# qope/SIPP

Hardware: AMD Instinct MI355X
Metric: SIPP proof-gen wall-clock + pairings-aggregated/sec, n=128 (the 3 STARK sub-proofs, hardened G1/G2 AIRs; outer plonky2 proof not included) (higher is better)
Workload: dtype u64; 1 GPU; n=128 SIPP instance per GPU: G1ExpStark 127 IO (N=2^16, W+P+Q=1176), G2ExpStark 127 IO (N=2^16, 2314), Fq12ExpStark 14 IO (N=2^13, 7970); IO records on host -> 3 flat proofs on host, the 3 sub-proofs on 3 concurrent HIP streams; parallelism=1 independent SIPP instance(s), one per GPU, no collective

## Files before the change

__graft_entry__.py:

```python
import os
import sys

ROOT = os.path.dirname(os.path.abspath(__file__))
if ROOT not in sys.path:
    sys.path.insert(0, ROOT)


def build():
    from sipp_amd import build as b
    so = b.build()
    assert os.path.exists(so), so
    from tests import _oracle
    _oracle.build()
    import sipp_amd
    sipp_amd.lib()
    import subprocess
    subprocess.check_call(["make", "-C", os.path.join(ROOT, "tests", "host"), "-s"])
    subprocess.check_call(["make", "-C", os.path.join(ROOT, "tests", "probe"), "-s"])


def smoke():
    import numpy as np
    import torch
    assert torch.cuda.is_available(), "smoke() needs a GPU"
    import sipp_amd
    from tests import _oracle

    ios = np.load(os.path.join(ROOT, "tests", "golden", "sipp_n4_ios.npz"))["g1"]
    ctx = sipp_amd.Ctx(device=0, workspace_bytes=4 << 30)
    proof = ctx.prove(0, ios)
    ctx.close()
    ref = _oracle.stark_prove(0, ios)
    assert len(proof) == len(ref) and (proof == ref).all(), "GPU proof differs from the CPU oracle's"
    assert sipp_amd.stark_verify(proof) == 0, "the library's own verifier (sipp_stark_verify) rejects the GPU proof"
    assert _oracle.stark_verify(proof) == 0, "oracle verifier rejects the GPU proof"
    print("smoke ok: G1ExpStark proof (%d words) identical to the oracle's, accepted by the library's verifier and the oracle's" % len(proof))


if __name__ == "__main__":
    build()
    if len(sys.argv) > 1 and sys.argv[1] == "smoke":
        smoke()
```

include/sipp_hip.h:

```cpp
#ifndef SIPP_HIP_H
#define SIPP_HIP_H

#include <stddef.h>
#include <stdint.h>

#ifdef __cplusplus
extern "C" {
#endif

typedef struct sipp_ctx sipp_ctx;

typedef enum {
    SIPP_OK = 0,
    SIPP_E_BADARG = -1,
    SIPP_E_HIP = -2,
    SIPP_E_NOMEM = -3,
    SIPP_E_BUFSZ = -4,
    SIPP_E_SUBGROUP = -5,
    SIPP_E_QUOTIENT = -6,
    SIPP_E_UNSUPPORTED = -7,
    SIPP_E_WITNESS = -8,
    SIPP_E_VERIFY = -9
} sipp_status;

typedef struct {
    uint32_t rate_bits;
    uint32_t cap_height;
    uint32_t pow_bits;
    uint32_t arity_bits;
    uint32_t final_poly_bits;
    uint32_t num_queries;
    uint32_t num_challenges;
    uint32_t pow_rule;
    uint32_t fs_rule;
    uint32_t lookup_rule;
} sipp_stark_config;
#define SIPP_POW_DUPLEX 0
#define SIPP_POW_HASH 1
#define SIPP_FS_STATEMENT 0
#define SIPP_FS_UPSTREAM 1
#define SIPP_LOOKUP_INDEPENDENT 0
#define SIPP_LOOKUP_SHARED 1

void sipp_default_config(sipp_stark_config *cfg);

typedef enum { SIPP_G1_EXP = 0, SIPP_G2_EXP = 1, SIPP_FQ12_EXP = 2,
               SIPP_MAP_G2 = 3 ,
               SIPP_G1_EXP_HARDENED = 4, SIPP_G2_EXP_HARDENED = 5,
               SIPP_PAIRING = 6  } sipp_kind;

#define SIPP_G1_IO_WORDS 56
#define SIPP_G2_IO_WORDS 104
#define SIPP_FQ12_IO_WORDS 296
#define SIPP_MAP_G2_IO_WORDS 48
#define SIPP_PAIRING_IO_WORDS 144

int sipp_ctx_create(sipp_ctx **out, int device, const sipp_stark_config *cfg, size_t workspace_bytes);
#define SIPP_ABI_VERSION 3u
uint32_t sipp_abi_version(void);
int sipp_ctx_create_checked(sipp_ctx **out, int device, const sipp_stark_config *cfg, size_t cfg_size, uint32_t abi_version,
                            size_t workspace_bytes);
#define SIPP_ROUTE_OPENINGS_UNGROUPED 1u
#define SIPP_ROUTE_LDE_COLUMN_WIDE 2u
#define SIPP_ROUTE_WITNESS_NO_GRAPH 4u
int sipp_ctx_set_kernel_routes(sipp_ctx *ctx, uint32_t routes);
void sipp_ctx_destroy(sipp_ctx *ctx);
int sipp_ctx_set_stream_priority(sipp_ctx *ctx, int level);
int sipp_ctx_set_hardened(sipp_ctx *ctx, int on);
const char *sipp_last_error(const sipp_ctx *ctx);
int sipp_sync(sipp_ctx *ctx);
void *sipp_stream(sipp_ctx *ctx);

int sipp_g1_exp_prove(sipp_ctx *ctx, const uint32_t *ios, size_t num_io, uint64_t *proof_out, size_t proof_cap,
                      size_t *proof_len);
int sipp_g2_exp_prove(sipp_ctx *ctx, const uint32_t *ios, size_t num_io, uint64_t *proof_out, size_t proof_cap,
                      size_t *proof_len);
int sipp_fq12_exp_prove(sipp_ctx *ctx, const uint32_t *ios, size_t num_io, uint64_t *proof_out, size_t proof_cap,
                        size_t *proof_len);
int sipp_prove(sipp_ctx *ctx, int kind, const uint32_t *ios, size_t num_io, uint64_t *proof_out, size_t proof_cap,
               size_t *proof_len);
int sipp_prove_async(sipp_ctx *ctx, int kind, const uint32_t *ios, size_t num_io, uint64_t *proof_out,
                     size_t proof_cap);
int sipp_wait(sipp_ctx *ctx, size_t *proof_len);
int sipp_instance_prove(sipp_ctx *const ctxs[3], const uint32_t *const ios[3], const size_t num_io[3],
                        uint64_t *const proof_out[3], const size_t proof_cap[3], size_t proof_len[3]);
int sipp_instances_prove(sipp_ctx *const *ctxs, size_t in_flight, size_t count, const uint32_t *const *ios,
                         const size_t *num_io, uint64_t *const *proof_out, const size_t *proof_cap, size_t *proof_len,
                         int *status);
int sipp_io_shard(size_t num_io, uint32_t world, uint32_t rank, size_t *first, size_t *count);
int sipp_exp_outputs(sipp_ctx *ctx, int kind, uint32_t *ios, size_t num_io);
size_t sipp_proof_size(const sipp_ctx *ctx, int kind, size_t num_io);
size_t sipp_workspace_bytes(int kind, size_t num_io);
size_t sipp_workspace_bytes_cfg(int kind, size_t num_io, const sipp_stark_config *cfg);
int sipp_device_memory(int device, size_t *free_bytes, size_t *total_bytes);
int sipp_stark_shape(const sipp_ctx *ctx, int kind, size_t num_io, uint32_t *log_rows, uint32_t *main_cols,
                     uint32_t *perm_cols, uint32_t *quotient_cols);

int sipp_map_to_g2_prove(sipp_ctx *ctx, const uint32_t *ios, size_t num_io, uint64_t *proof_out, size_t proof_cap,
                         size_t *proof_len);
int sipp_pairing_prove(sipp_ctx *ctx, const uint32_t *ios, size_t num_io, uint64_t *proof_out, size_t proof_cap,
                       size_t *proof_len);
int sipp_stark_verify(const uint64_t *proof, size_t len, const sipp_stark_config *cfg, int *reason);

int sipp_map_to_g2(sipp_ctx *ctx, const uint32_t *msgs, size_t n, uint32_t *map_ios, uint32_t *g2_ios, uint32_t *cleared);

int sipp_inner_product(sipp_ctx *ctx, const uint32_t *g1, const uint32_t *g2, size_t n, uint32_t *out);
int sipp_inner_products(sipp_ctx *ctx, const uint32_t *g1, const uint32_t *g2, size_t n, size_t count, uint32_t *out);

size_t sipp_native_proof_words(size_t n);
int sipp_prove_native(sipp_ctx *ctx, const uint32_t *A, const uint32_t *B, size_t n, uint32_t *proof);
int sipp_verify_native(sipp_ctx *ctx, const uint32_t *A, const uint32_t *B, size_t n, const uint32_t *proof,
                       uint32_t *statement, uint32_t *g1_ios, uint32_t *g2_ios, uint32_t *fq12_ios, int *accepted);

#define SIPP_SALT_SIZE 4
#define SIPP_FRI_MAX_ROUNDS 32
typedef struct {
    uint32_t rate_bits, cap_height, pow_bits, num_queries, pow_rule;
    uint32_t hiding;
    uint32_t n_rounds;
    uint32_t arity_bits[SIPP_FRI_MAX_ROUNDS];
} sipp_fri_params;
void sipp_fri_const_arity(sipp_fri_params *p, uint32_t arity_bits, uint32_t final_poly_bits, uint32_t degree_bits);
typedef struct {
    const uint64_t *d_coeffs;
    const uint64_t *d_lde;
    const uint64_t *d_tree;
    uint32_t n_polys, n_salt;
} sipp_oracle;
int sipp_commit_batch_ex(sipp_ctx *ctx, const uint64_t *d_in, int from_coeffs, uint64_t *d_coeffs, uint64_t *d_lde,
                         uint64_t *d_tree, size_t ncols, uint32_t log_n, uint32_t rate_bits, uint32_t cap_height,
                         const uint64_t *d_salt, uint32_t n_salt, uint64_t *cap_out);
typedef struct { uint32_t oracle, col_begin, col_end; } sipp_poly_range;
typedef struct {
    uint64_t point[2];
    uint32_t n_ranges;
    const sipp_poly_range *ranges;
} sipp_fri_batch;
typedef struct {
    uint64_t state[12];
    uint64_t in_buf[8];
    uint64_t n_in;
    uint64_t out_buf[8];
    uint64_t n_out;
} sipp_challenger;
size_t sipp_fri_proof_size(const sipp_oracle *oracles, size_t n_oracles, const sipp_fri_batch *batches, size_t n_batches,
                           uint32_t log_n, const sipp_fri_params *p);
int sipp_fri_prove_openings(sipp_ctx *ctx, const sipp_oracle *oracles, size_t n_oracles, const sipp_fri_batch *batches,
// ... 125 lines not shown
```

sipp_amd/csrc/api.hip:

```cpp
#include <algorithm>
#include <string>

#include "ctx.hpp"
#include "host_poseidon.hpp"

int sipp_poseidon_init_constants(sipp_ctx* ctx);

extern "C" {

void sipp_default_config(sipp_stark_config* cfg) {
    if (!cfg) return;
    cfg->rate_bits = 1;
    cfg->cap_height = 4;
    cfg->pow_bits = 16;
    cfg->arity_bits = 4;
    cfg->final_poly_bits = 5;
    cfg->num_queries = 84;
    cfg->num_challenges = 2;
    cfg->pow_rule = SIPP_POW_DUPLEX;
    cfg->fs_rule = SIPP_FS_STATEMENT;
    cfg->lookup_rule = SIPP_LOOKUP_INDEPENDENT;
}

static hipError_t create_ctx_stream(int device, int level, hipStream_t* out) {
    int lo = 0, hi = 0;
    (void)hipDeviceGetStreamPriorityRange(&lo, &hi);
    static const int dedicated = [] { const char* e = getenv("SIPP_DEDICATED_QUEUES"); return e ? atoi(e) : 1; }();
    if (level <= 0 && dedicated) {
        hipDeviceProp_t prop;
        if (hipGetDeviceProperties(&prop, device) == hipSuccess && prop.multiProcessorCount > 0 && prop.multiProcessorCount <= 1024) {
            uint32_t mask[32];
            const uint32_t words = ((uint32_t)prop.multiProcessorCount + 31) / 32;
            for (uint32_t i = 0; i < words; i++) {
                const uint32_t left = (uint32_t)prop.multiProcessorCount - 32 * i;
                mask[i] = left >= 32 ? 0xffffffffu : (1u << left) - 1;
            }
            if (hipExtStreamCreateWithCUMask(out, words, mask) == hipSuccess) return hipSuccess;
            (void)hipGetLastError();
        }
    }
    return hipStreamCreateWithPriority(out, hipStreamNonBlocking, level > 0 ? hi : level < 0 ? lo : 0);
}

int sipp_ctx_create(sipp_ctx** out, int device, const sipp_stark_config* cfg, size_t workspace_bytes) {
    if (!out) return SIPP_E_BADARG;
    *out = nullptr;
    int ndev = 0;
    if (hipGetDeviceCount(&ndev) != hipSuccess || ndev <= 0 || device < 0 || device >= ndev) return SIPP_E_HIP;
    sipp_ctx* ctx = new sipp_ctx();
    ctx->device = device;
    if (cfg)
        ctx->cfg = *cfg;
    else
        sipp_default_config(&ctx->cfg);
    if (ctx->cfg.rate_bits < 1 || ctx->cfg.rate_bits > 3 || ctx->cfg.num_challenges != 2 || ctx->cfg.arity_bits < 1 ||
        ctx->cfg.arity_bits > 4 || ctx->cfg.cap_height > 8 || ctx->cfg.pow_bits > 32 || ctx->cfg.pow_rule > SIPP_POW_HASH ||
        ctx->cfg.fs_rule > SIPP_FS_UPSTREAM || ctx->cfg.lookup_rule > SIPP_LOOKUP_SHARED || ctx->cfg.num_queries == 0 || ctx->cfg.num_queries > 1024 || ctx->cfg.final_poly_bits > 12) {
        delete ctx;
        return SIPP_E_UNSUPPORTED;
    }
    auto bail = [&](int rc) {
        hipError_t last = hipGetLastError();
        fprintf(stderr, "sipp_ctx_create(device %d, workspace %zu bytes) failed with status %d (last HIP error: %s)\n", device,
                workspace_bytes, rc, hipGetErrorString(last));
        sipp_ctx_destroy(ctx);
        return rc;
    };
    if (hipSetDevice(device) != hipSuccess) return bail(SIPP_E_HIP);
    if (create_ctx_stream(device, 0, &ctx->stream) != hipSuccess) return bail(SIPP_E_HIP);
    if (workspace_bytes == 0) workspace_bytes = (size_t)24 << 30;
    ctx->arena_size = workspace_bytes;
    if (hipMalloc((void**)&ctx->arena, workspace_bytes) != hipSuccess) return bail(SIPP_E_NOMEM);
    if (hipEventCreate(&ctx->t0) != hipSuccess || hipEventCreate(&ctx->t1) != hipSuccess) return bail(SIPP_E_HIP);
    ctx->h_pinned_words = (size_t)1 << 23;
    if (hipHostMalloc((void**)&ctx->h_pinned, ctx->h_pinned_words * 8) != hipSuccess) return bail(SIPP_E_NOMEM);
    int rc = sipp_poseidon_init_constants(ctx);
    if (rc != SIPP_OK) return bail(rc);
    *out = ctx;
    return SIPP_OK;
}

void sipp_ctx_destroy(sipp_ctx* ctx) {
    if (!ctx) return;
    if (ctx->async.started) {
        {
            std::unique_lock<std::mutex> lk(ctx->async.mu);
            ctx->async.cv.wait(lk, [&] { return !ctx->async.has_job || ctx->async.done; });
            ctx->async.quit = true;
        }
        ctx->async.cv.notify_all();
        ctx->async.th.join();
    }
    (void)hipSetDevice(ctx->device);
    if (ctx->stream) (void)hipStreamSynchronize(ctx->stream);
    sipp_witness_graph_release(ctx);
    for (auto& kv : ctx->tables) (void)hipFree(kv.second);
    for (auto e : ctx->ev_pool) (void)hipEventDestroy(e);
    if (ctx->t0) (void)hipEventDestroy(ctx->t0);
    if (ctx->t1) (void)hipEventDestroy(ctx->t1);
    if (ctx->h_pinned) (void)hipHostFree(ctx->h_pinned);
    if (ctx->arena) (void)hipFree(ctx->arena);
    if (ctx->aux_stream) (void)hipStreamDestroy(ctx->aux_stream);
    if (ctx->aux2_stream) (void)hipStreamDestroy(ctx->aux2_stream);
    if (ctx->stream) (void)hipStreamDestroy(ctx->stream);
    delete ctx;
}

uint32_t sipp_abi_version(void) { return SIPP_ABI_VERSION; }

int sipp_ctx_create_checked(sipp_ctx** out, int device, const sipp_stark_config* cfg, size_t cfg_size, uint32_t abi_version,
                            size_t workspace_bytes) {
    if (out) *out = nullptr;
    if (abi_version != SIPP_ABI_VERSION || (cfg && cfg_size != sizeof(sipp_stark_config))) return SIPP_E_BADARG;
    return sipp_ctx_create(out, device, cfg, workspace_bytes);
}

int sipp_ctx_set_kernel_routes(sipp_ctx* ctx, uint32_t routes) {
    if (!ctx || (routes & ~(uint32_t)(SIPP_ROUTE_OPENINGS_UNGROUPED | SIPP_ROUTE_LDE_COLUMN_WIDE | SIPP_ROUTE_WITNESS_NO_GRAPH))) return SIPP_E_BADARG;
    std::unique_lock<std::mutex> lk(ctx->async.mu);
    if (ctx->async.has_job) {
        lk.unlock();
        return sipp_fail(ctx, SIPP_E_BADARG, "set_kernel_routes: a proof is in flight on this ctx");
    }
    ctx->kernel_routes = routes;
    return SIPP_OK;
}

int sipp_ctx_set_hardened(sipp_ctx* ctx, int on) {
    if (!ctx) return SIPP_E_BADARG;
    std::unique_lock<std::mutex> lk(ctx->async.mu);
    if (ctx->async.has_job) {
        lk.unlock();
        return sipp_fail(ctx, SIPP_E_BADARG, "set_hardened: a proof is in flight on this ctx");
    }
    ctx->hardened = on != 0;
    return SIPP_OK;
}

int sipp_ctx_set_stream_priority(sipp_ctx* ctx, int level) {
    if (!ctx) return SIPP_E_BADARG;
    {
        std::unique_lock<std::mutex> lk(ctx->async.mu);
        if (ctx->async.has_job) {
            lk.unlock();
            return sipp_fail(ctx, SIPP_E_BADARG, "set_stream_priority: a proof is in flight on this ctx");
        }
    }
    SIPP_CHECK_HIP(ctx, hipSetDevice(ctx->device));
    hipStream_t ns = nullptr;
    if (create_ctx_stream(ctx->device, level, &ns) != hipSuccess) return sipp_fail(ctx, SIPP_E_HIP, "set_stream_priority: no stream");
    if (ctx->stream) {
        (void)hipStreamSynchronize(ctx->stream);
        if (ctx->prof) {
            (void)sipp_profile_enable(ctx, 0);
            ctx->prof = true;
        }
        (void)hipStreamDestroy(ctx->stream);
    }
    ctx->stream = ns;
    return SIPP_OK;
}

const char* sipp_last_error(const sipp_ctx* ctx) { return ctx ? ctx->err : "null ctx"; }

int sipp_sync(sipp_ctx* ctx) {
    if (!ctx) return SIPP_E_BADARG;
    SIPP_CHECK_HIP(ctx, hipSetDevice(ctx->device));
    SIPP_CHECK_HIP(ctx, hipStreamSynchronize(ctx->stream));
    return SIPP_OK;
}

void* sipp_stream(sipp_ctx* ctx) { return ctx ? (void*)ctx->stream : nullptr; }

static void prof_drain(sipp_ctx* ctx) {
    if (ctx->pending.empty()) return;
    (void)hipSetDevice(ctx->device);
    (void)hipStreamSynchronize(ctx->stream);
    for (auto& p : ctx->pending) {
        float ms = 0.f;
        if (hipEventElapsedTime(&ms, ctx->ev_pool[std::get<1>(p)], ctx->ev_pool[std::get<2>(p)]) == hipSuccess) {
            auto& e = ctx->prof_acc[std::get<0>(p)];
            e.calls++;
            e.ms += ms;
        }
    }
    ctx->pending.clear();
    ctx->ev_used = 0;
}

int sipp_profile_enable(sipp_ctx* ctx, int enable) {
    if (!ctx) return SIPP_E_BADARG;
    if (!enable) prof_drain(ctx);
    ctx->prof = enable != 0;
    return SIPP_OK;
}

int sipp_profile_reset(sipp_ctx* ctx) {
    if (!ctx) return SIPP_E_BADARG;
    prof_drain(ctx);
    ctx->prof_acc.clear();
    return SIPP_OK;
// ... 157 lines not shown
```

sipp_amd/csrc/ctx.hpp:

```cpp
#pragma once
#include <stdlib.h>
#include <hip/hip_runtime.h>
#include <stdint.h>
#include <stdio.h>
#include <string.h>

#include <condition_variable>
#include <map>
#include <mutex>
#include <string>
#include <thread>
#include <tuple>
#include <vector>

#include "../../include/sipp_hip.h"
#include "gl.hpp"

struct sipp_gate {
    std::mutex mu;
    std::condition_variable cv;
    bool open = false;
    void release() {
        {
            std::lock_guard<std::mutex> lk(mu);
            open = true;
        }
        cv.notify_all();
    }
    void wait() {
        std::unique_lock<std::mutex> lk(mu);
        cv.wait(lk, [&] { return open; });
    }
};

struct sipp_prof_entry {
    int calls = 0;
    double ms = 0.0;
};

struct sipp_ctx {
    int device = 0;
    hipStream_t stream = nullptr;
    sipp_stark_config cfg{};
    char err[512] = {0};

    char* arena = nullptr;
    size_t arena_size = 0;
    size_t arena_off = 0;
    size_t arena_peak = 0;

    std::map<std::tuple<int, uint64_t, uint64_t>, uint64_t*> tables;

    bool prof = false;
    std::vector<hipEvent_t> ev_pool;
    size_t ev_used = 0;
    std::vector<std::tuple<std::string, size_t, size_t>> pending;
    std::map<std::string, sipp_prof_entry> prof_acc;
    hipEvent_t t0 = nullptr, t1 = nullptr;

    uint64_t* h_pinned = nullptr;
    size_t h_pinned_words = 0;

    sipp_gate* gate_wait = nullptr;
    sipp_gate* gate_release = nullptr;

    hipStream_t aux_stream = nullptr;
    hipStream_t aux2_stream = nullptr;
    struct Fold {
        bool active = false;
        size_t mark = 0;
        uint32_t* d_ios[2] = {nullptr, nullptr};
        void* rows[2] = {nullptr, nullptr};
        int* d_err = nullptr;
        uint32_t num_io[2] = {0, 0};
        size_t n_in[2] = {0, 0};
    } fold;

    bool outputs_only = false;
    bool hardened = false;
    uint32_t kernel_routes = 0;
    struct WitnessGraph {
        hipGraph_t graph = nullptr;
        hipGraphExec_t exec = nullptr;
        std::vector<uint64_t> key;
    } wgraph;

    struct Async {
        std::thread th;
        std::mutex mu;
        std::condition_variable cv;
        bool started = false, has_job = false, done = false, quit = false;
        int kind = 0;
        const uint32_t* ios = nullptr;
        size_t num_io = 0, cap = 0, len = 0;
        uint64_t* out = nullptr;
        int rc = 0;
    } async;
};

#define SIPP_CHECK_HIP(ctx, expr)                                                                   \
    do {                                                                                            \
        hipError_t e__ = (expr);                                                                    \
        if (e__ != hipSuccess) {                                                                    \
            snprintf((ctx)->err, sizeof((ctx)->err), "%s:%d: %s -> %s", __FILE__, __LINE__, #expr,  \
                     hipGetErrorString(e__));                                                       \
            return SIPP_E_HIP;                                                                      \
        }                                                                                           \
    } while (0)

#define SIPP_TRY(expr)              \
    do {                            \
        int rc__ = (expr);          \
        if (rc__ != SIPP_OK) return rc__; \
    } while (0)

static inline int sipp_fail(sipp_ctx* ctx, int code, const char* msg) {
    if (ctx) snprintf(ctx->err, sizeof(ctx->err), "%s", msg);
    return code;
}

struct ArenaMark {
    size_t off;
};
static inline ArenaMark arena_mark(sipp_ctx* ctx) { return ArenaMark{ctx->arena_off}; }
static inline void arena_release(sipp_ctx* ctx, ArenaMark m) { ctx->arena_off = m.off; }
static inline void* arena_alloc(sipp_ctx* ctx, size_t bytes) {
    size_t off = (ctx->arena_off + 255) & ~(size_t)255;
    if (off + bytes > ctx->arena_size) {
        snprintf(ctx->err, sizeof(ctx->err), "workspace arena exhausted: need %zu more bytes (size %zu, used %zu)",
                 bytes, ctx->arena_size, off);
        return nullptr;
    }
    ctx->arena_off = off + bytes;
    if (ctx->arena_off > ctx->arena_peak) ctx->arena_peak = ctx->arena_off;
    return ctx->arena + off;
}
struct ArenaScope {
    sipp_ctx* ctx;
    ArenaMark mark;
    explicit ArenaScope(sipp_ctx* c) : ctx(c), mark(arena_mark(c)) {}
    ~ArenaScope() { arena_release(ctx, mark); }
    ArenaScope(const ArenaScope&) = delete;
    ArenaScope& operator=(const ArenaScope&) = delete;
};
// ... 86 lines not shown
```

sipp_amd/csrc/fri.hip:

```cpp
#include <algorithm>

#include "prover.hpp"

static size_t tree_words(uint32_t log_leaves) { return ((size_t)8 << log_leaves); }

static int read_cap(sipp_ctx* ctx, const uint64_t* d_tree, uint32_t log_leaves, uint32_t cap_height, uint64_t* cap_host) {
    const uint32_t ch = std::min(cap_height, log_leaves);
    uint64_t off = 0;
    for (uint32_t l = 0; l < log_leaves - ch; l++) off += (uint64_t)1 << (log_leaves - l);
    SIPP_CHECK_HIP(ctx, hipMemcpyAsync(cap_host, d_tree + 4 * off, ((size_t)4 << ch) * 8, hipMemcpyDeviceToHost, ctx->stream));
    SIPP_CHECK_HIP(ctx, hipStreamSynchronize(ctx->stream));
    return SIPP_OK;
}

size_t sipp_fri_core_words(const FriParamsDev& p, uint32_t log_n, const uint32_t* leaf_words, int n_oracles) {
    const uint32_t log_m = log_n + p.rate_bits;
    const size_t cap = (size_t)4 << p.cap_height;
    uint32_t sum = 0;
    for (uint32_t ab : p.arity_bits) sum += ab;
    size_t w = p.arity_bits.size() * cap + 2 * ((size_t)1 << (log_n - sum)) + 1;
    size_t per_q = 0;
    for (int o = 0; o < n_oracles; o++) per_q += leaf_words[o] + (size_t)(log_m - p.cap_height) * 4;
    uint32_t lt = log_m;
    for (uint32_t ab : p.arity_bits) {
        lt -= ab;
        per_q += ((size_t)2 << ab) + (size_t)(lt > p.cap_height ? lt - p.cap_height : 0) * 4;
    }
    return w + p.num_queries * per_q;
}

int sipp_fri_prove_core(sipp_ctx* ctx, const FriOracleDev* ors, int n_oracles, uint32_t log_n, const FriParamsDev& p,
                        uint64_t* d_final, host::Challenger& ch, uint64_t* pf, size_t& pos, size_t cap_total, size_t* final_len,
                        const std::function<void(const char*)>& tick) {
    const uint32_t log_m = log_n + p.rate_bits, R = (uint32_t)p.arity_bits.size(), nq = p.num_queries;
    const size_t n = (size_t)1 << log_n, m = (size_t)1 << log_m;
    const size_t cap_words = (size_t)4 << p.cap_height;
    if (p.cap_height > 8 || n_oracles < 1 || n_oracles > 8) return sipp_fail(ctx, SIPP_E_UNSUPPORTED, "fri: unsupported shape");
    auto push = [&](const uint64_t* v, size_t cnt) -> int {
        if (pos + cnt > cap_total) return SIPP_E_BUFSZ;
        memcpy(pf + pos, v, cnt * 8);
        pos += cnt;
        return SIPP_OK;
    };
    uint64_t cap_host[4 << 8];
    std::vector<uint64_t*> r_vals(R), r_tree(R);
    std::vector<uint32_t> r_loglen(R);
    uint64_t* cur = d_final;
    size_t len_c = n;
    uint32_t log_len = log_m;
    uint64_t shift = gl::GEN;
    for (uint32_t r = 0; r < R; r++) {
        const uint32_t ab = p.arity_bits[r];
        const size_t len = (size_t)1 << log_len;
        if (log_len < ab + 0u || (len_c >> ab) == 0) return sipp_fail(ctx, SIPP_E_BADARG, "fri: reduction arities exceed the degree");
        r_loglen[r] = log_len;
        r_vals[r] = arena_alloc_t<uint64_t>(ctx, 2 * len);
        r_tree[r] = arena_alloc_t<uint64_t>(ctx, tree_words(log_len - ab));
        uint64_t* nxt = arena_alloc_t<uint64_t>(ctx, 2 * (len_c >> ab) + 2);
        if (!r_vals[r] || !r_tree[r] || !nxt) return SIPP_E_NOMEM;
        SIPP_TRY(sipp_ntt_dif(ctx, cur, len_c, log_len - p.rate_bits, r_vals[r], len, log_len, 2, false, NttDiag{shift, 0}));
        SIPP_TRY(sipp_k_fri_leaves(ctx, r_vals[r], len, ab, r_tree[r]));
        SIPP_TRY(sipp_k_merkle_levels(ctx, r_tree[r], log_len - ab, p.cap_height));
        SIPP_TRY(read_cap(ctx, r_tree[r], log_len - ab, p.cap_height, cap_host));
        const size_t cw = (size_t)4 << std::min(p.cap_height, log_len - ab);
        ch.observe_many(cap_host, cw);
        SIPP_TRY(push(cap_host, cw));
        const gl::E2 fb = ch.get_ext();
        SIPP_TRY(sipp_k_fri_fold(ctx, cur, len_c, ab, fb, nxt));
        cur = nxt;
        len_c >>= ab;
        log_len -= ab;
        shift = gl::pow(shift, (uint64_t)1 << ab);
    }
    (void)cap_words;
    if (final_len) *final_len = len_c;
    {
        std::vector<uint64_t> fpv(2 * len_c);
        SIPP_CHECK_HIP(ctx, hipMemcpyAsync(fpv.data(), cur, fpv.size() * 8, hipMemcpyDeviceToHost, ctx->stream));
        SIPP_CHECK_HIP(ctx, hipStreamSynchronize(ctx->stream));
        for (size_t i = 0; i < len_c; i++) {
            uint64_t e[2] = {fpv[i], fpv[len_c + i]};
            ch.observe_many(e, 2);
            SIPP_TRY(push(e, 2));
        }
    }
    if (tick) tick("fri commit phase");
    uint64_t pow_witness = 0;
    if (p.pow_rule == SIPP_POW_HASH) {
        uint64_t zero[12] = {0}, cur_h[4];
        for (int i = 0; i < 4; i++) cur_h[i] = ch.get();
        SIPP_TRY(sipp_k_pow_search(ctx, zero, cur_h, 4, 0, p.pow_bits, &pow_witness));
    } else {
        SIPP_TRY(sipp_k_pow_search(ctx, ch.state, ch.in_buf, ch.n_in, 7, p.pow_bits, &pow_witness));
        ch.observe(pow_witness);
        (void)ch.get();
    }
    SIPP_TRY(push(&pow_witness, 1));
    if (tick) tick("pow");
    std::vector<uint32_t> qidx(nq);
    for (uint32_t i = 0; i < nq; i++) qidx[i] = (uint32_t)(ch.get() % m);
    uint32_t* d_idx = arena_alloc_t<uint32_t>(ctx, nq);
    if (!d_idx) return SIPP_E_NOMEM;
    SIPP_CHECK_HIP(ctx, hipMemcpyAsync(d_idx, qidx.data(), nq * 4, hipMemcpyHostToDevice, ctx->stream));
    const uint32_t nsib0 = log_m - p.cap_height;
    size_t st_words = 0;
    std::vector<size_t> off_rows(n_oracles), off_sib(n_oracles), off_leaf(R), off_rsib(R);
    std::vector<uint32_t> rsib(R), rshift(R);
    for (int o = 0; o < n_oracles; o++) {
        off_rows[o] = st_words;
        st_words += (size_t)nq * ors[o].ncols;
        off_sib[o] = st_words;
        st_words += (size_t)nq * nsib0 * 4;
    }
    {
        uint32_t sh = 0;
        for (uint32_t r = 0; r < R; r++) {
            const uint32_t ab = p.arity_bits[r];
            sh += ab;
            rshift[r] = sh;
            const uint32_t lt = log_m - sh;
            rsib[r] = lt > p.cap_height ? lt - p.cap_height : 0;
            off_leaf[r] = st_words;
            st_words += (size_t)nq * ((size_t)2 << ab);
            off_rsib[r] = st_words;
            st_words += (size_t)nq * rsib[r] * 4;
        }
    }
    if (st_words > ctx->h_pinned_words) return sipp_fail(ctx, SIPP_E_NOMEM, "query staging exceeds the pinned buffer");
    uint64_t* d_st = arena_alloc_t<uint64_t>(ctx, st_words);
    if (!d_st) return SIPP_E_NOMEM;
    std::vector<QueryGatherTask> tasks;
    {
        for (int o = 0; o < n_oracles; o++) {
            tasks.push_back(QueryGatherTask{ors[o].lde, d_st + off_rows[o], (uint64_t)ors[o].stride, 0, ors[o].ncols, 0, 0});
            if (nsib0) tasks.push_back(QueryGatherTask{ors[o].tree, d_st + off_sib[o], 0, 1, log_m, nsib0, 0});
        }
        for (uint32_t r = 0; r < R; r++) {
            const uint32_t ab = p.arity_bits[r];
            tasks.push_back(QueryGatherTask{r_vals[r], d_st + off_leaf[r], (uint64_t)1 << r_loglen[r], 2, rshift[r], ab, 0});
            if (rsib[r]) tasks.push_back(QueryGatherTask{r_tree[r], d_st + off_rsib[r], 0, 1, r_loglen[r] - ab, rsib[r], rshift[r]});
        }
        QueryGatherTask* d_tasks = arena_alloc_t<QueryGatherTask>(ctx, tasks.size());
        if (!d_tasks) return SIPP_E_NOMEM;
        SIPP_CHECK_HIP(ctx, hipMemcpyAsync(d_tasks, tasks.data(), tasks.size() * sizeof(QueryGatherTask), hipMemcpyHostToDevice, ctx->stream));
        SIPP_TRY(sipp_k_gather_tasks(ctx, d_tasks, (uint32_t)tasks.size(), d_idx, nq));
    }
    uint64_t* hst = ctx->h_pinned;
    SIPP_CHECK_HIP(ctx, hipMemcpyAsync(hst, d_st, st_words * 8, hipMemcpyDeviceToHost, ctx->stream));
    SIPP_CHECK_HIP(ctx, hipStreamSynchronize(ctx->stream));
    for (uint32_t qi = 0; qi < nq; qi++) {
        for (int o = 0; o < n_oracles; o++) {
            SIPP_TRY(push(hst + off_rows[o] + (size_t)qi * ors[o].ncols, (size_t)ors[o].ncols));
            SIPP_TRY(push(hst + off_sib[o] + (size_t)qi * nsib0 * 4, (size_t)nsib0 * 4));
        }
        for (uint32_t r = 0; r < R; r++) {
            const size_t lw = (size_t)2 << p.arity_bits[r];
            SIPP_TRY(push(hst + off_leaf[r] + (size_t)qi * lw, lw));
            SIPP_TRY(push(hst + off_rsib[r] + (size_t)qi * rsib[r] * 4, (size_t)rsib[r] * 4));
        }
    }
    return SIPP_OK;
}


#define SIPP_FRI_MAGIC 0x5349505046524931ULL

static size_t batch_len(const sipp_fri_batch& b) {
    size_t k = 0;
    for (uint32_t r = 0; r < b.n_ranges; r++) k += b.ranges[r].col_end - b.ranges[r].col_begin;
    return k;
}

static int check_params(sipp_ctx* ctx, const sipp_fri_params* p, uint32_t log_n) {
    if (!p || p->rate_bits < 1 || p->rate_bits > 3 || p->cap_height > 8 || p->pow_bits > 32 || p->pow_rule > SIPP_POW_HASH ||
        p->num_queries == 0 || p->num_queries > 1024 || p->n_rounds > SIPP_FRI_MAX_ROUNDS)
        return sipp_fail(ctx, SIPP_E_UNSUPPORTED, "fri: parameters out of the supported range");
    uint32_t sum = 0;
    for (uint32_t r = 0; r < p->n_rounds; r++) {
        if (p->arity_bits[r] < 1 || p->arity_bits[r] > 4) return sipp_fail(ctx, SIPP_E_UNSUPPORTED, "fri: arity must be 2, 4, 8 or 16");
        sum += p->arity_bits[r];
        if (log_n + p->rate_bits < sum + p->cap_height)
            return sipp_fail(ctx, SIPP_E_BADARG, "fri: reduction arities leave a layer smaller than its cap");
        if (log_n + p->rate_bits - sum + p->arity_bits[r] < 4)
            return sipp_fail(ctx, SIPP_E_UNSUPPORTED, "fri: a committed layer of fewer than 16 values is not supported");
    }
    if (sum > log_n) return sipp_fail(ctx, SIPP_E_BADARG, "fri: the reduction arities exceed the degree bits");
    if (log_n < 10 || log_n > 24) return sipp_fail(ctx, SIPP_E_UNSUPPORTED, "fri: degree bits outside the supported range [10, 24]");
    return SIPP_OK;
}

extern "C" {

void sipp_fri_const_arity(sipp_fri_params* p, uint32_t arity_bits, uint32_t final_poly_bits, uint32_t degree_bits) {
    if (!p) return;
    p->n_rounds = 0;
    while (degree_bits > final_poly_bits && degree_bits + p->rate_bits - arity_bits >= p->cap_height && degree_bits >= arity_bits &&
           p->n_rounds < SIPP_FRI_MAX_ROUNDS) {
        p->arity_bits[p->n_rounds++] = arity_bits;
        degree_bits -= arity_bits;
    }
}

int sipp_commit_batch_ex(sipp_ctx* ctx, const uint64_t* d_in, int from_coeffs, uint64_t* d_coeffs, uint64_t* d_lde, uint64_t* d_tree,
                         size_t ncols, uint32_t log_n, uint32_t rate_bits, uint32_t cap_height, const uint64_t* d_salt,
                         uint32_t n_salt, uint64_t* cap_out) {
    if (!ctx || !d_in || !d_coeffs || !d_lde || !d_tree || !cap_out || ncols == 0) return SIPP_E_BADARG;
    if (rate_bits < 1 || rate_bits > 3 || cap_height > 8 || (n_salt != 0 && (n_salt != SIPP_SALT_SIZE || !d_salt)))
        return sipp_fail(ctx, SIPP_E_UNSUPPORTED, "commit_batch_ex: blowup 2 / 4 / 8, cap height <= 8, salt 0 or 4 columns");
    SIPP_CHECK_HIP(ctx, hipSetDevice(ctx->device));
    const uint32_t log_m = log_n + rate_bits;
    const size_t n = (size_t)1 << log_n, m = (size_t)1 << log_m;
    ArenaScope scope(ctx);
    int rc;
    if (from_coeffs) {
        if (d_in != d_coeffs) SIPP_CHECK_HIP(ctx, hipMemcpyAsync(d_coeffs, d_in, ncols * n * 8, hipMemcpyDeviceToDevice, ctx->stream));
        rc = sipp_lde_from_coeffs(ctx, d_coeffs, d_lde, ncols, log_n, rate_bits);
        if (rc == SIPP_E_UNSUPPORTED) rc = sipp_ntt_dif(ctx, d_coeffs, n, log_n, d_lde, m, log_m, ncols, false, NttDiag{gl::GEN, 0});
    } else {
        rc = d_in != d_coeffs ? sipp_lde_from_values(ctx, d_in, d_coeffs, d_lde, ncols, log_n, rate_bits) : SIPP_E_UNSUPPORTED;
        if (rc == SIPP_E_UNSUPPORTED) {
            const uint64_t* src = d_in;
            if (d_in == d_coeffs) {
                uint64_t* tmp = arena_alloc_t<uint64_t>(ctx, n * ncols);
                if (!tmp) return SIPP_E_NOMEM;
                SIPP_CHECK_HIP(ctx, hipMemcpyAsync(tmp, d_in, n * ncols * 8, hipMemcpyDeviceToDevice, ctx->stream));
                src = tmp;
            }
// ... 14 lines not shown
                           uint32_t log_n, const sipp_fri_params* p) {
    if (!oracles || !batches || !p || n_oracles == 0 || n_oracles > 8 || n_batches == 0) return 0;
    FriParamsDev fp;
    fp.rate_bits = p->rate_bits; fp.cap_height = p->cap_height; fp.pow_bits = p->pow_bits; fp.num_queries = p->num_queries;
    fp.pow_rule = p->pow_rule;
    uint32_t sum = 0;
    for (uint32_t r = 0; r < p->n_rounds && r < SIPP_FRI_MAX_ROUNDS; r++) {
        fp.arity_bits.push_back(p->arity_bits[r]);
        sum += p->arity_bits[r];
    }
    if (sum > log_n) return 0;
    uint32_t lw[8];
    for (size_t o = 0; o < n_oracles; o++) lw[o] = oracles[o].n_polys + oracles[o].n_salt;
    size_t w = 8 + sipp_fri_core_words(fp, log_n, lw, (int)n_oracles);
    for (size_t b = 0; b < n_batches; b++) w += 2 * batch_len(batches[b]);
    return w;
}

int sipp_fri_prove_openings(sipp_ctx* ctx, const sipp_oracle* oracles, size_t n_oracles, const sipp_fri_batch* batches,
                            size_t n_batches, uint32_t log_n, const sipp_fri_params* p, sipp_challenger* chs, uint64_t* proof_out,
                            size_t proof_cap, size_t* proof_len) {
    if (!ctx || !oracles || !batches || !p || !chs || !proof_out || !proof_len || n_oracles == 0 || n_oracles > 8 || n_batches == 0)
        return SIPP_E_BADARG;
    SIPP_CHECK_HIP(ctx, hipSetDevice(ctx->device));
    SIPP_TRY(check_params(ctx, p, log_n));
    if (chs->n_in > 7 || chs->n_out > 8) return sipp_fail(ctx, SIPP_E_BADARG, "fri: malformed challenger state");
    const size_t total = sipp_fri_proof_size(oracles, n_oracles, batches, n_batches, log_n, p);
    if (total == 0) return SIPP_E_BADARG;
    if (proof_cap < total) return sipp_fail(ctx, SIPP_E_BUFSZ, "fri: proof buffer too small (see sipp_fri_proof_size)");
    for (size_t b = 0; b < n_batches; b++)
        for (uint32_t r = 0; r < batches[b].n_ranges; r++) {
            const sipp_poly_range& rg = batches[b].ranges[r];
            if (rg.oracle >= n_oracles || rg.col_begin > rg.col_end || rg.col_end > oracles[rg.oracle].n_polys)
                return sipp_fail(ctx, SIPP_E_BADARG, "fri: polynomial range outside its oracle");
        }
    const size_t n = (size_t)1 << log_n, m = n << p->rate_bits;
    FriParamsDev fp;
    fp.rate_bits = p->rate_bits; fp.cap_height = p->cap_height; fp.pow_bits = p->pow_bits; fp.num_queries = p->num_queries;
    fp.pow_rule = p->pow_rule;
    for (uint32_t r = 0; r < p->n_rounds; r++) fp.arity_bits.push_back(p->arity_bits[r]);
    host::Challenger ch;
    memcpy(ch.state, chs->state, sizeof ch.state);
    memcpy(ch.in_buf, chs->in_buf, sizeof ch.in_buf);
    memcpy(ch.out_buf, chs->out_buf, sizeof ch.out_buf);
    ch.n_in = (uint32_t)chs->n_in;
    ch.n_out = (uint32_t)chs->n_out;
    struct Release {
        sipp_ctx* c;
        ArenaMark mk;
        ~Release() {
            (void)hipStreamSynchronize(c->stream);
            arena_release(c, mk);
        }
    } release{ctx, arena_mark(ctx)};
    size_t pos = 0;
    uint64_t* pf = proof_out;
    {
        uint64_t hdr[8] = {SIPP_FRI_MAGIC, p->n_rounds, 0, p->num_queries, (uint64_t)n_oracles, (uint64_t)n_batches, total, log_n};
        memcpy(pf, hdr, sizeof hdr);
        pos = 8;
    }
    std::vector<uint64_t*> d_zp(n_batches), d_zip(n_batches);
    std::vector<gl::E2> points(n_batches);
    for (size_t b = 0; b < n_batches; b++) {
        points[b] = gl::E2{batches[b].point[0], batches[b].point[1]};
        if (gl::eq(gl::pow(points[b], (uint64_t)n), gl::e2(1))) return sipp_fail(ctx, SIPP_E_SUBGROUP, "fri: opening point in the subgroup");
        d_zp[b] = arena_alloc_t<uint64_t>(ctx, 2 * n);
        d_zip[b] = arena_alloc_t<uint64_t>(ctx, 2 * n);
        if (!d_zp[b] || !d_zip[b]) return SIPP_E_NOMEM;
        SIPP_TRY(sipp_k_pow_table(ctx, points[b], n, d_zp[b]));
        SIPP_TRY(sipp_k_pow_table(ctx, gl::inv(points[b]), n, d_zip[b]));
    }
    for (size_t b = 0; b < n_batches; b++) {
        const size_t k = batch_len(batches[b]);
        uint64_t* d_open = arena_alloc_t<uint64_t>(ctx, 4 * k + 4);
        if (!d_open) return SIPP_E_NOMEM;
        size_t at = 0;
        for (uint32_t r = 0; r < batches[b].n_ranges; r++) {
            const sipp_poly_range& rg = batches[b].ranges[r];
            const size_t cnt = rg.col_end - rg.col_begin;
            SIPP_TRY(sipp_k_openings(ctx, oracles[rg.oracle].d_coeffs + (size_t)rg.col_begin * n, cnt, n, d_zp[b], nullptr, d_open + 4 * at));
            at += cnt;
        }
        std::vector<uint64_t> hop(4 * k + 4);
        SIPP_CHECK_HIP(ctx, hipMemcpyAsync(hop.data(), d_open, (4 * k) * 8, hipMemcpyDeviceToHost, ctx->stream));
        SIPP_CHECK_HIP(ctx, hipStreamSynchronize(ctx->stream));
        for (size_t j = 0; j < k; j++) {
            memcpy(pf + pos, &hop[4 * j], 16);
            pos += 2;
            ch.observe_many(&hop[4 * j], 2);
        }
    }
    const gl::E2 alpha = ch.get_ext();
    uint64_t* d_acc = arena_alloc_t<uint64_t>(ctx, 2 * n);
    uint64_t* d_final = arena_alloc_t<uint64_t>(ctx, 2 * n);
    if (!d_acc || !d_final) return SIPP_E_NOMEM;
    for (size_t b = 0; b < n_batches; b++) {
        const size_t k = batch_len(batches[b]);
        std::vector<const uint64_t*> cols;
        cols.reserve(k);
        for (uint32_t r = 0; r < batches[b].n_ranges; r++) {
            const sipp_poly_range& rg = batches[b].ranges[r];
            for (uint32_t c = rg.col_begin; c < rg.col_end; c++) cols.push_back(oracles[rg.oracle].d_coeffs + (size_t)c * n);
        }
        std::vector<uint32_t> apow(6 * k + 6);
        gl::E2 ap = gl::e2(1);
        for (size_t c = 0; c < k; c++) {
            const uint64_t comp[2] = {ap.c0, ap.c1};
            for (int q = 0; q < 2; q++) {
                apow[6 * c + 3 * q] = (uint32_t)comp[q] & 0x3FFFFFu;
                apow[6 * c + 3 * q + 1] = (uint32_t)(comp[q] >> 22) & 0x3FFFFFu;
                apow[6 * c + 3 * q + 2] = (uint32_t)(comp[q] >> 44);
            }
            ap = gl::mul(ap, alpha);
        }
        const uint64_t** d_cols = reinterpret_cast<const uint64_t**>(arena_alloc(ctx, (k + 1) * sizeof(uint64_t*)));
        uint32_t* d_apow = arena_alloc_t<uint32_t>(ctx, apow.size());
        if (!d_cols || !d_apow) return SIPP_E_NOMEM;
        SIPP_CHECK_HIP(ctx, hipMemcpyAsync(d_cols, cols.data(), k * sizeof(uint64_t*), hipMemcpyHostToDevice, ctx->stream));
        SIPP_CHECK_HIP(ctx, hipMemcpyAsync(d_apow, apow.data(), apow.size() * 4, hipMemcpyHostToDevice, ctx->stream));
        SIPP_CHECK_HIP(ctx, hipStreamSynchronize(ctx->stream));
        SIPP_TRY(sipp_k_fri_batch_quotient(ctx, d_cols, (int)k, n, d_apow, d_zp[b], d_zip[b], ap, b == 0, d_acc));
    }
    SIPP_TRY(sipp_k_fri_mulx(ctx, d_acc, n, d_final));
    FriOracleDev ors[8];
    for (size_t o = 0; o < n_oracles; o++)
        ors[o] = FriOracleDev{oracles[o].d_lde, m, oracles[o].n_polys + oracles[o].n_salt, oracles[o].d_tree};
    size_t flen = 0;
    SIPP_TRY(sipp_fri_prove_core(ctx, ors, (int)n_oracles, log_n, fp, d_final, ch, pf, pos, total, &flen, nullptr));
    pf[2] = flen;
    if (pos != total) return sipp_fail(ctx, SIPP_E_BUFSZ, "internal: opening proof length mismatch");
    *proof_len = pos;
    memcpy(chs->state, ch.state, sizeof ch.state);
    memcpy(chs->in_buf, ch.in_buf, sizeof ch.in_buf);
    memcpy(chs->out_buf, ch.out_buf, sizeof ch.out_buf);
    chs->n_in = ch.n_in;
    chs->n_out = ch.n_out;
    return SIPP_OK;
}

}
```

sipp_amd/csrc/host_challenger.hpp:

```cpp
#pragma once
#include <stddef.h>
#include <stdint.h>

#include "gl.hpp"
#include "host_poseidon.hpp"

namespace host {


struct Challenger {
    uint64_t state[12] = {0};
    uint64_t in_buf[8];
    uint32_t n_in = 0;
    uint64_t out_buf[8];
    uint32_t n_out = 0;
    void duplex() {
        for (uint32_t i = 0; i < n_in; i++) state[i] = in_buf[i];
        n_in = 0;
        poseidon_permute(state);
        for (int i = 0; i < 8; i++) out_buf[i] = state[i];
        n_out = 8;
    }
    void observe(uint64_t e) {
        n_out = 0;
        in_buf[n_in++] = e;
        if (n_in == 8) duplex();
    }
    void observe_many(const uint64_t* e, size_t n) {
        for (size_t i = 0; i < n; i++) observe(e[i]);
    }
    uint64_t get() {
        if (n_in != 0 || n_out == 0) duplex();
        return out_buf[--n_out];
    }
    static void hash_no_pad(const uint64_t* in, size_t n, uint64_t out[4]) {
        uint64_t s[12] = {0};
        for (size_t i = 0; i < n; i += 8) {
            for (size_t k = 0; k < 8 && i + k < n; k++) s[k] = in[i + k];
            poseidon_permute(s);
        }
        for (int k = 0; k < 4; k++) out[k] = s[k];
    }
    static void two_to_one(const uint64_t l[4], const uint64_t r[4], uint64_t out[4]) {
        uint64_t s[12] = {l[0], l[1], l[2], l[3], r[0], r[1], r[2], r[3], 0, 0, 0, 0};
        poseidon_permute(s);
        for (int k = 0; k < 4; k++) out[k] = s[k];
    }
    gl::E2 get_ext() {
        gl::E2 r;
        r.c0 = get();
        r.c1 = get();
        return r;
    }
};

}
```

sipp_amd/csrc/poseidon.hip:

```cpp
#include <type_traits>
#include "ctx.hpp"
#ifndef GLL_T
#define GLL_T 140
#endif
#include "poseidon.hpp"
#include "poseidon_pair.hpp"
#include "prover.hpp"

namespace {

#ifndef SIPP_LEAVES_WPE
#define SIPP_LEAVES_WPE 3
#endif
__global__ void __launch_bounds__(256) __attribute__((amdgpu_waves_per_eu(SIPP_LEAVES_WPE, SIPP_LEAVES_WPE)))
poseidon_leaves_kernel(const uint64_t* __restrict__ lde, size_t col_stride,
                                                             uint32_t ncols, uint64_t n_leaves,
                                                             uint64_t* __restrict__ digests) {
    const uint64_t j0 = (uint64_t)blockIdx.x * blockDim.x + threadIdx.x;
    const uint64_t j = j0 < n_leaves ? j0 : n_leaves - 1;
    uint64_t s[12];
#pragma unroll
    for (int i = 0; i < 12; i++) s[i] = 0;
    const uint64_t* p = lde + j;
    __shared__ uint64_t stash[11 * 256];
// ... 140 lines not shown
#pragma unroll
    for (int i = 0; i < 12; i++) s[i] = 0;
    const uint64_t* c0 = vals + 16 * k;
    const uint64_t* c1 = vals + len + 16 * k;
#pragma unroll 1
    for (int chunk = 0; chunk < 4; chunk++) {
#pragma unroll
        for (int e = 0; e < 8; e++) s[e] = (e & 1) ? c1[4 * chunk + (e >> 1)] : c0[4 * chunk + (e >> 1)];
        poseidon::permute(s);
    }
    uint64_t* d = digests + 4 * k;
    d[0] = s[0]; d[1] = s[1]; d[2] = s[2]; d[3] = s[3];
}

__global__ void __launch_bounds__(256) fri_leaves_pair_kernel(const uint64_t* __restrict__ vals, uint64_t len,
                                                             uint64_t* __restrict__ digests) {
    __shared__ poseidon_pair::Tables T;
    poseidon_pair::load_tables(T);
    const uint32_t lane = threadIdx.x & 63, h = lane >> 5;
    const uint64_t wave = ((uint64_t)blockIdx.x * blockDim.x + threadIdx.x) >> 6;
    const uint64_t nl = len >> 4;
    if (wave * 32 >= nl) return;
    const uint64_t k = wave * 32 + (lane & 31);
    const bool live = k < nl;
    const uint64_t kk = live ? k : 0;
    const poseidon::mfma_v4i afrag = poseidon_pair::mds_fragment(lane);
    const uint64_t* c0 = vals + 16 * kk;
    const uint64_t* c1 = vals + len + 16 * kk;
    uint64_t s[6] = {0, 0, 0, 0, 0, 0};
#pragma unroll 1
    for (int chunk = 0; chunk < 4; chunk++) {
#pragma unroll
        for (int j = 0; j < 6; j++) {
            const uint32_t e = 6 * h + j;
            if (e < 8) s[j] = (e & 1) ? c1[4 * chunk + (e >> 1)] : c0[4 * chunk + (e >> 1)];
        }
        poseidon_pair::permute(s, lane, T, afrag);
    }
    if (!live || h) return;
    uint64_t* d = digests + 4 * k;
    d[0] = s[0];
    d[1] = s[1];
    d[2] = s[2];
    d[3] = s[3];
}

__global__ void __launch_bounds__(64) fri_leaves_any_kernel(const uint64_t* __restrict__ vals, uint64_t len, uint32_t ab,
                                                           uint64_t* __restrict__ digests) {
    const uint64_t k = (uint64_t)blockIdx.x * blockDim.x + threadIdx.x;
    if (k >= (len >> ab)) return;
    const uint32_t words = 2u << ab;
    const uint64_t* c0 = vals + (k << ab);
    const uint64_t* c1 = vals + len + (k << ab);
    uint64_t s[12];
#pragma unroll
    for (int i = 0; i < 12; i++) s[i] = 0;
    if (words <= 4) {
        s[0] = c0[0];
        s[1] = c1[0];
        if (words == 4) {
            s[2] = c0[1];
            s[3] = c1[1];
        }
    } else {
#pragma unroll 1
        for (uint32_t chunk = 0; chunk < words / 8; chunk++) {
#pragma unroll
            for (int e = 0; e < 8; e++) s[e] = (e & 1) ? c1[4 * chunk + (e >> 1)] : c0[4 * chunk + (e >> 1)];
            poseidon::permute(s);
        }
    }
    uint64_t* d = digests + 4 * k;
    d[0] = s[0]; d[1] = s[1]; d[2] = s[2]; d[3] = s[3];
}

struct PowArgs {
    uint64_t state[12];
    uint64_t in_buf[8];
    uint32_t n_in, pow_bits, resp_word;
    uint64_t base;
    unsigned long long* result;
};
__global__ void __launch_bounds__(256) pow_kernel(PowArgs a) {
    const uint64_t w = a.base + (uint64_t)blockIdx.x * blockDim.x + threadIdx.x;
    uint64_t s[12];
#pragma unroll
    for (int i = 0; i < 12; i++) s[i] = a.state[i];
#pragma unroll
    for (int i = 0; i < 8; i++) {
        if ((uint32_t)i < a.n_in) s[i] = a.in_buf[i];
        if ((uint32_t)i == a.n_in) s[i] = w;
    }
    poseidon::permute(s);
    const uint64_t resp = a.resp_word == 7 ? s[7] : s[0];
    if ((resp >> (64 - a.pow_bits)) == 0) atomicMin(a.result, (unsigned long long)w);
}

constexpr uint64_t thin_threshold() { return 65536; }

}

int sipp_k_fri_leaves(sipp_ctx* ctx, const uint64_t* d_vals, size_t len, uint32_t arity_bits, uint64_t* d_digests) {
    uint64_t nl = len >> arity_bits;
    ProfScope ps(ctx, "fri_leaves");
    if (arity_bits != 4) {
        if (arity_bits < 1 || arity_bits > 4) return sipp_fail(ctx, SIPP_E_UNSUPPORTED, "fri_leaves: arity must be 2, 4, 8 or 16");
        hipLaunchKernelGGL(fri_leaves_any_kernel, dim3((unsigned)((nl + 63) / 64)), dim3(64), 0, ctx->stream, d_vals, (uint64_t)len,
                           arity_bits, d_digests);
    } else if (nl <= thin_threshold())
        hipLaunchKernelGGL(fri_leaves_pair_kernel, dim3((unsigned)((2 * nl + 255) / 256)), dim3(256), 0, ctx->stream, d_vals,
                           (uint64_t)len, d_digests);
    else
        hipLaunchKernelGGL(fri_leaves_kernel, dim3((unsigned)((nl + 63) / 64)), dim3(64), 0, ctx->stream, d_vals, (uint64_t)len,
                           d_digests);
    SIPP_CHECK_HIP(ctx, hipGetLastError());
    return SIPP_OK;
}

int sipp_k_pow_search(sipp_ctx* ctx, const uint64_t state[12], const uint64_t* in_buf, uint32_t n_in, uint32_t resp_word,
                      uint32_t pow_bits, uint64_t* witness) {
    if (pow_bits == 0) { *witness = 0; return SIPP_OK; }
    if (pow_bits > 32 || n_in > 7 || (resp_word != 0 && resp_word != 7))
        return sipp_fail(ctx, SIPP_E_UNSUPPORTED, "pow_search: unsupported parameters");
    ArenaMark mk = arena_mark(ctx);
    unsigned long long* d_res = arena_alloc_t<unsigned long long>(ctx, 1);
    if (!d_res) return SIPP_E_NOMEM;
    PowArgs a;
    memcpy(a.state, state, sizeof a.state);
    memset(a.in_buf, 0, sizeof a.in_buf);
    memcpy(a.in_buf, in_buf, n_in * sizeof(uint64_t));
    a.n_in = n_in; a.pow_bits = pow_bits; a.resp_word = resp_word; a.result = d_res;
    const uint32_t log_batch = pow_bits + 1 < 12 ? 12 : pow_bits + 1 > 28 ? 28 : pow_bits + 1;
    const uint64_t batch = (uint64_t)1 << log_batch;
    unsigned long long h_res = ~0ull;
    SIPP_CHECK_HIP(ctx, hipMemsetAsync(d_res, 0xff, sizeof(unsigned long long), ctx->stream));
    for (uint64_t base = 0; base < ((uint64_t)1 << 44); base += batch) {
        a.base = base;
        {
            ProfScope ps(ctx, "pow_grind");
            hipLaunchKernelGGL(pow_kernel, dim3((unsigned)(batch / 256)), dim3(256), 0, ctx->stream, a);
        }
        SIPP_CHECK_HIP(ctx, hipGetLastError());
        SIPP_CHECK_HIP(ctx, hipMemcpyAsync(&h_res, d_res, sizeof h_res, hipMemcpyDeviceToHost, ctx->stream));
        SIPP_CHECK_HIP(ctx, hipStreamSynchronize(ctx->stream));
        if (h_res != ~0ull) break;
    }
    arena_release(ctx, mk);
    if (h_res == ~0ull) return sipp_fail(ctx, SIPP_E_UNSUPPORTED, "pow_search: no witness found");
    *witness = (uint64_t)h_res;
    return SIPP_OK;
}

int sipp_poseidon_init_constants(sipp_ctx* ctx) {
    SIPP_CHECK_HIP(ctx, hipMemcpyToSymbol(HIP_SYMBOL(poseidon::c_rc), SIPP_POSEIDON_RC, sizeof(SIPP_POSEIDON_RC)));
    SIPP_CHECK_HIP(ctx, hipMemcpyToSymbol(HIP_SYMBOL(poseidon::c_fast_first), SIPP_POSEIDON_FAST_FIRST,
                                          sizeof(SIPP_POSEIDON_FAST_FIRST)));
    SIPP_CHECK_HIP(ctx, hipMemcpyToSymbol(HIP_SYMBOL(poseidon::c_fast_scalar), SIPP_POSEIDON_FAST_SCALAR,
                                          sizeof(SIPP_POSEIDON_FAST_SCALAR)));
    SIPP_CHECK_HIP(ctx, hipMemcpyToSymbol(HIP_SYMBOL(poseidon::c_fast_mi), SIPP_POSEIDON_FAST_MI,
                                          sizeof(SIPP_POSEIDON_FAST_MI)));
    SIPP_CHECK_HIP(ctx, hipMemcpyToSymbol(HIP_SYMBOL(poseidon::c_fast_vs), SIPP_POSEIDON_FAST_VS,
                                          sizeof(SIPP_POSEIDON_FAST_VS)));
    SIPP_CHECK_HIP(ctx, hipMemcpyToSymbol(HIP_SYMBOL(poseidon::c_fast_what), SIPP_POSEIDON_FAST_WHAT,
                                          sizeof(SIPP_POSEIDON_FAST_WHAT)));
    SIPP_CHECK_HIP(ctx, hipMemcpyToSymbol(HIP_SYMBOL(poseidon::c_blk3), SIPP_POSEIDON_BLK3, sizeof(SIPP_POSEIDON_BLK3)));
    SIPP_CHECK_HIP(ctx, hipMemcpyToSymbol(HIP_SYMBOL(poseidon::c_comb3), SIPP_POSEIDON_COMB3, sizeof(SIPP_POSEIDON_COMB3)));
    SIPP_CHECK_HIP(ctx, hipMemcpyToSymbol(HIP_SYMBOL(poseidon::c_comb_c), SIPP_POSEIDON_COMB_C, sizeof(SIPP_POSEIDON_COMB_C)));
    SIPP_CHECK_HIP(ctx, hipMemcpyToSymbol(HIP_SYMBOL(poseidon::d_dense_a), SIPP_POSEIDON_DENSE_A, sizeof(SIPP_POSEIDON_DENSE_A)));
    SIPP_CHECK_HIP(ctx, hipMemcpyToSymbol(HIP_SYMBOL(poseidon::c_dense_start), SIPP_POSEIDON_DENSE_START, sizeof(SIPP_POSEIDON_DENSE_START)));
    SIPP_CHECK_HIP(ctx, hipMemcpyToSymbol(HIP_SYMBOL(poseidon_pair::d_pair_a), SIPP_POSEIDON_PAIR_A, sizeof(SIPP_POSEIDON_PAIR_A)));
    SIPP_CHECK_HIP(ctx, hipMemcpyToSymbol(HIP_SYMBOL(poseidon_pair::d_pair_mds_a), SIPP_POSEIDON_PAIR_MDS_A, sizeof(SIPP_POSEIDON_PAIR_MDS_A)));
    SIPP_CHECK_HIP(ctx, hipMemcpyToSymbol(HIP_SYMBOL(poseidon_pair::d_pair_cc), SIPP_POSEIDON_PAIR_CC3, sizeof(SIPP_POSEIDON_PAIR_CC3)));
    SIPP_CHECK_HIP(ctx, hipMemcpyToSymbol(HIP_SYMBOL(poseidon_pair::d_pair_start), SIPP_POSEIDON_PAIR_START, sizeof(SIPP_POSEIDON_PAIR_START)));
    return SIPP_OK;
}

int sipp_k_poseidon_leaves(sipp_ctx* ctx, const uint64_t* d_lde, size_t col_stride, size_t ncols, uint32_t log_leaves,
                           uint64_t* d_digests) {
    if (ncols == 0 || ncols > 0xffffffffull) return sipp_fail(ctx, SIPP_E_BADARG, "poseidon_leaves: bad ncols");
    uint64_t n = (uint64_t)1 << log_leaves;
    const bool thin = ncols > 4 && n <= thin_threshold() && n >= 32;
    ProfScope ps(ctx, ncols <= 4 ? "poseidon_leaves_noop" : thin ? "poseidon_leaves_pair" : "poseidon_leaves");
    if (ncols <= 4) {
        hipLaunchKernelGGL(poseidon_leaves_copy_kernel, dim3((unsigned)((n + 255) / 256)), dim3(256), 0, ctx->stream, d_lde, col_stride,
                           (uint32_t)ncols, n, d_digests);
    } else if (thin) {
        unsigned grid = (unsigned)((2 * n + 255) / 256);
        hipLaunchKernelGGL(poseidon_leaves_pair_kernel, dim3(grid), dim3(256), 0, ctx->stream, d_lde, col_stride,
                           (uint32_t)ncols, n, d_digests);
    } else {
        const unsigned bs = n <= 65536 ? 64 : 256;
        unsigned grid = (unsigned)((n + bs - 1) / bs);
        hipLaunchKernelGGL(poseidon_leaves_kernel, dim3(grid), dim3(bs), 0, ctx->stream, d_lde, col_stride,
                           (uint32_t)ncols, n, d_digests);
    }
    SIPP_CHECK_HIP(ctx, hipGetLastError());
    return SIPP_OK;
}

int sipp_k_merkle_levels(sipp_ctx* ctx, uint64_t* d_tree, uint32_t log_leaves, uint32_t cap_height) {
    if (cap_height > log_leaves) cap_height = log_leaves;
    {
        uint32_t level = 0;
        const uint32_t top = log_leaves - cap_height;
        while (level < top) {
            const uint32_t log_nodes = log_leaves - level;
            uint32_t lw = log_nodes <= 10 ? log_nodes : log_nodes >= 18 ? 10 : 8;
            uint32_t nlev = lw < top - level ? lw : top - level;
            const uint64_t widest_parents = (uint64_t)1 << (log_nodes - 1);
            if (widest_parents > thin_threshold()) {
                lw = 11;
                nlev = 3 < top - level ? 3 : top - level;
            }
            const unsigned blocks = 1u << (log_nodes - lw);
            ProfScope ps(ctx, "merkle_subtree");
            if (widest_parents <= thin_threshold())
                hipLaunchKernelGGL(merkle_subtree_kernel<true>, dim3(blocks), dim3(256), 0, ctx->stream, d_tree, log_leaves, level, lw, nlev);
            else
                hipLaunchKernelGGL(merkle_subtree_kernel<false>, dim3(blocks), dim3(256), 0, ctx->stream, d_tree, log_leaves, level, lw, nlev);
            SIPP_CHECK_HIP(ctx, hipGetLastError());
            level += nlev;
        }
        return SIPP_OK;
    }
}

int sipp_k_poseidon_permute(sipp_ctx* ctx, uint64_t* d_states, size_t n) {
    if (!n) return SIPP_OK;
    unsigned grid = (unsigned)((n + 255) / 256);
    ProfScope ps(ctx, "poseidon_permute");
    hipLaunchKernelGGL(poseidon_permute_kernel, dim3(grid), dim3(256), 0, ctx->stream, d_states, (uint64_t)n);
    SIPP_CHECK_HIP(ctx, hipGetLastError());
// ... 3 lines not shown
```

sipp_amd/csrc/prover.hip:

```cpp
#include <map>

#include "ctx.hpp"
#include "prover.hpp"

namespace {

using gl::E2;

template <bool REV>
__device__ __forceinline__ uint64_t block_scan_mul_256(uint64_t v, uint64_t* s) {
    const int t = REV ? 255 - (int)threadIdx.x : (int)threadIdx.x;
    s[t] = v;
    __syncthreads();
    for (int off = 1; off < 256; off <<= 1) {
        uint64_t o = t >= off ? s[t - off] : 1;
        __syncthreads();
        v = gl::mul(v, o);
        s[t] = v;
        __syncthreads();
    }
    return v;
}

__device__ __forceinline__ void block_scan4_mul_256(uint64_t (&v)[4], uint64_t (*s)[256]) {
    const int t = threadIdx.x;
#pragma unroll
    for (int q = 0; q < 4; q++) s[q][t] = v[q];
    __syncthreads();
    for (int off = 1; off < 256; off <<= 1) {
        uint64_t o[4];
        o[0] = t >= off ? s[0][t - off] : 1;
        o[1] = t >= off ? s[1][t - off] : 1;
        o[2] = t + off < 256 ? s[2][t + off] : 1;
        o[3] = t + off < 256 ? s[3][t + off] : 1;
        __syncthreads();
#pragma unroll
        for (int q = 0; q < 4; q++) {
            v[q] = gl::mul(v[q], o[q]);
            s[q][t] = v[q];
        }
        __syncthreads();
    }
}

template <int ZR>
__global__ void __launch_bounds__(256) z_phase_a(const uint64_t* __restrict__ trace, size_t n, int nm, int nc, int cbase,
                                                uint64_t gamma0, uint64_t gamma1, uint64_t beta0, uint64_t beta1,
                                                uint64_t* __restrict__ zv, uint64_t* __restrict__ totals) {
    __shared__ uint64_t s[4][256];
    const int j = blockIdx.y;
    const size_t r0 = (size_t)blockIdx.x * (256 * ZR) + (size_t)threadIdx.x * ZR;
    const ulonglong2* col = reinterpret_cast<const ulonglong2*>(trace + (size_t)(cbase + j) * n + r0);
    const ulonglong2* tab = reinterpret_cast<const ulonglong2*>(trace + r0);
    const ulonglong2* pin = reinterpret_cast<const ulonglong2*>(trace + (size_t)(nm + j) * n + r0);
    const ulonglong2* ptab = reinterpret_cast<const ulonglong2*>(trace + (size_t)(nm + nc + j) * n + r0);
    uint64_t num[2][ZR], den[2][ZR];
#pragma unroll
    for (int k = 0; k < ZR; k += 2) {
        const ulonglong2 c2 = col[k >> 1], t2 = tab[k >> 1], p2 = pin[k >> 1], q2 = ptab[k >> 1];
#pragma unroll
        for (int i = 0; i < 2; i++) {
            const uint64_t g = i ? gamma1 : gamma0, b = i ? beta1 : beta0;
            num[i][k] = gl::mul(gl::add(c2.x, g), gl::add(t2.x, b));
            den[i][k] = gl::mul(gl::add(p2.x, g), gl::add(q2.x, b));
            num[i][k + 1] = gl::mul(gl::add(c2.y, g), gl::add(t2.y, b));
            den[i][k + 1] = gl::mul(gl::add(p2.y, g), gl::add(q2.y, b));
        }
    }
    uint64_t v[4];
#pragma unroll
    for (int i = 0; i < 2; i++) {
        uint64_t ntot = 1;
#pragma unroll
        for (int k = 0; k < ZR; k++) {
            const uint64_t x = num[i][k];
            num[i][k] = ntot;
            ntot = gl::mul(ntot, x);
        }
#pragma unroll
        for (int k = ZR - 2; k >= 0; k--) den[i][k] = gl::mul(den[i][k], den[i][k + 1]);
        v[i] = ntot;
        v[2 + i] = den[i][0];
    }
    block_scan4_mul_256(v, s);
#pragma unroll
    for (int i = 0; i < 2; i++) {
// ... 237 lines not shown
            const uint64_t coef = gl::from_i64(*w++);
            uint64_t va[16], vb[16];
            w += qvec<16>(w, c, va);
            w += qvec<16>(w, c, vb);
#pragma unroll
            for (int ch = 0; ch < 2; ch++) {
                gl::Acc6 Ae, Ao, Be, Bo;
                Ae.zero(); Ao.zero(); Be.zero(); Bo.zero();
#pragma unroll
                for (int i = 0; i < 8; i++) {
                    const uint32_t* g3 = a.ginv3[ch][i];
                    Ae.mac((uint32_t)va[2 * i], (uint32_t)(va[2 * i] >> 32), g3);
                    Ao.mac((uint32_t)va[2 * i + 1], (uint32_t)(va[2 * i + 1] >> 32), g3);
                    Be.mac((uint32_t)vb[2 * i], (uint32_t)(vb[2 * i] >> 32), g3);
                    Bo.mac((uint32_t)vb[2 * i + 1], (uint32_t)(vb[2 * i + 1] >> 32), g3);
                }
                const uint64_t ae = Ae.reduce(), ao = Ao.reduce(), be = Be.reduce(), bo = Bo.reduce();
                const uint64_t cross = gl::add(gl::mul(ae, bo), gl::mul(ao, be));
                uint64_t t = gl::mad(gl::mul(ao, bo), a.gamma_inv[ch], gl::mul(ae, be));
                t = gl::mad(cross, 65536, t);
                psum[ch] = gl::mad(coef, t, psum[ch]);
            }
        }
        const int nl = slice == 0 ? (int)*w++ : 0;
        for (int p = 0; p < nl; p++) {
            const uint64_t coef = gl::from_i64(*w++);
            uint64_t va[16];
            w += qvec<16>(w, c, va);
#pragma unroll
            for (int ii = 0; ii < 16; ii++) e[ii] = gl::mad(coef, va[ii], e[ii]);
        }
        if (slice == 0) {
        uint64_t q[17];
        (void)qvec<17>(qdesc, c, q);
        const uint64_t s = c.local(sign_col);
        const uint64_t sgn = gl::sub(1, gl::add(s, s));
        uint64_t cprev = 0;
        const uint64_t coff = gl::from_i64(coffset);
        uint64_t d[32];
#pragma unroll
        for (int k = 0; k < 32; k++) {
            uint64_t al = 0, ah = 0;
#pragma unroll
            for (int ii = 0; ii < 17; ii++) {
                const int jj = k - ii;
                if (jj >= 0 && jj < 16) {
                    al += (uint64_t)(uint32_t)q[ii] * a.p_limbs[jj];
                    ah += (uint64_t)(uint32_t)(q[ii] >> 32) * a.p_limbs[jj];
                }
            }
            const uint64_t l = al + (ah << 32);
            const uint32_t h = (uint32_t)(ah >> 32) + (l < al ? 1u : 0u);
            const uint64_t qp = gl::reduce96(h, l);
            d[k] = gl::sub(e[k], gl::mul(sgn, qp));
        }
        const uint64_t wgt = (uint64_t)1 << (16 * grp);
#pragma unroll
        for (int mm = 0; mm < 32; mm++) {
            if (mm < 32 / grp) {
                uint64_t v;
                if (grp == 2) v = gl::mad(d[(2 * mm + 1) & 31], 65536, d[(2 * mm) & 31]);
                else v = d[mm];
                uint64_t ck = 0;
                if (mm < 32 / grp - 1) {
                    for (int l = 0; l < ncl; l++)
                        ck = gl::mad(c.local(cbase + mm * ncl + l), (uint64_t)1 << (lb * l), ck);
                    ck = gl::sub(ck, coff);
                }
                v = gl::sub(v, cprev);
                v = gl::mad(ck, wgt, v);
                c.emit(v);
                cprev = ck;
            }
        }
        c.emit(gl::mul(s, gl::sub(s, 1)));
        }
        c.acc0 = gl::mad(a.alpha16[0], psum[0], c.acc0);
        c.acc1 = gl::mad(a.alpha16[1], psum[1], c.acc1);
    }
    a.part[((size_t)g * 2 + 0) * m + j] = gl::mul(c.acc0, a.seg_pow[2 * g]);
    a.part[((size_t)g * 2 + 1) * m + j] = gl::mul(c.acc1, a.seg_pow[2 * g + 1]);
}

__global__ void alpha_pow3_kernel(uint64_t a0, uint64_t a1, int K, int nc, uint32_t* __restrict__ out) {
    const int t = blockIdx.x * blockDim.x + threadIdx.x;
    const int total = 2 * 3 + nc * 2 * 6;
    if (t >= total) return;
    int c, e;
    if (t < 6) {
        c = t / 3;
        e = K - 1 - t % 3;
    } else {
        const int k = (t - 6) / 12, r = (t - 6) % 12, slot = r % 6;
        c = r / 6;
        e = K - 1 - (3 + 2 * k) - (slot >> 1) * 2 * nc - (slot & 1);
    }
    uint32_t l[3];
    gl::limbs3(l, gl::pow(c ? a1 : a0, (uint64_t)e));
    for (int q = 0; q < 3; q++) out[3 * t + q] = l[q];
}

struct RestAcc {
    gl::Acc6 a[2];
    int terms;
    uint64_t folded[2];
    __device__ __forceinline__ void init() {
        a[0].zero();
        a[1].zero();
        terms = 0;
        folded[0] = folded[1] = 0;
    }
    __device__ __forceinline__ void mac(uint64_t v, const uint32_t* __restrict__ p0, const uint32_t* __restrict__ p1) {
        const uint32_t lo = (uint32_t)v, hi = (uint32_t)(v >> 32);
        a[0].mac(lo, hi, p0);
        a[1].mac(lo, hi, p1);
    }
    __device__ __forceinline__ void maybe_fold(int added) {
        terms += added;
        if (terms >= 960) {
            for (int c = 0; c < 2; c++) {
                folded[c] = gl::add(folded[c], gl::canon(a[c].reduce()));
                a[c].zero();
            }
            terms = 0;
        }
    }
    __device__ __forceinline__ uint64_t value(int c) const { return gl::add(folded[c], gl::canon(a[c].reduce())); }
};

struct RestPoint {
    uint64_t lf, zl, ll, zh_inv;
};
__device__ __forceinline__ RestPoint rest_point(const QuotArgs& a, uint32_t i) {
    const uint64_t x = gl::mul(gl::GEN, gl::pow(a.w_m, i));
    const uint64_t zh = a.zh[i & 1];
    RestPoint r;
    r.zl = gl::sub(x, a.g_inv);
    r.lf = gl::mul(gl::mul(zh, a.ninv), gl::inv(gl::sub(x, 1)));
    r.ll = gl::mul(gl::mul(gl::mul(zh, a.ninv), a.g_inv), gl::inv(r.zl));
    r.zh_inv = a.zh_inv[i & 1];
    return r;
}
__device__ __forceinline__ void rest_store(const QuotArgs& a, size_t m, size_t j, const RestPoint& pt, const uint64_t F[2], const uint64_t T[2],
                                           const uint64_t R[2]) {
    uint64_t acc[2] = {0, 0};
    for (int g = 0; g < a.n_seg; g++) {
        acc[0] = gl::add(acc[0], a.part[((size_t)g * 2 + 0) * m + j]);
        acc[1] = gl::add(acc[1], a.part[((size_t)g * 2 + 1) * m + j]);
    }
#pragma unroll
    for (int q = 0; q < 2; q++) {
        uint64_t v = gl::mul(acc[q], a.alphaK[q]);
        v = gl::add(v, R[q]);
        v = gl::mad(pt.lf, F[q], v);
        v = gl::mad(pt.zl, T[q], v);
        a.out[(size_t)q * m + j] = gl::mul(v, pt.zh_inv);
    }
}

template <bool SPLIT>
__global__ void __launch_bounds__(256) quotient_rest_kernel(QuotArgs a) {
    const size_t m = (size_t)1 << a.log_m;
    constexpr uint32_t RB = 3, RW = 256u >> RB;
    const uint32_t tid = threadIdx.x, run = tid / RW, blk = blockIdx.x, half = blk / (uint32_t)(m >> 9);
    const size_t j = (size_t)half * (m >> 1) + (size_t)run * (m >> (RB + 1)) + (size_t)(blk % (uint32_t)(m >> 9)) * RW + tid % RW;
    const uint32_t i = gl::bitrev((uint32_t)j, a.log_m);
// ... 104 lines not shown
    const int b = blockIdx.y;
    const E2 base = b == 0 ? a.base[0] : b == 1 ? a.base[1] : b == 2 ? a.base[2] : a.base[3];
    uint64_t* tab = b == 0 ? a.tab[0] : b == 1 ? a.tab[1] : b == 2 ? a.tab[2] : a.tab[3];
    const E2 r = gl::pow(base, (uint64_t)k);
    tab[k] = r.c0;
    tab[a.n + k] = r.c1;
}

__device__ __forceinline__ void openings_column(const uint64_t* __restrict__ col, size_t n, const uint64_t* __restrict__ t0,
                                                const uint64_t* __restrict__ t1, size_t tn, uint64_t* __restrict__ out4) {
    __shared__ uint64_t s[4][256];
    gl::Acc160 acc[4];
    constexpr int OB = 4;
    size_t k = threadIdx.x;
    for (; k + (OB - 1) * 256 < n; k += OB * 256) {
        uint64_t p0[OB], p1[OB], q0[OB], q1[OB], v[OB];
#pragma unroll
        for (int b = 0; b < OB; b++) {
            const size_t kb = k + (size_t)b * 256;
            p0[b] = t0[kb];
            p1[b] = t0[tn + kb];
            q0[b] = t1 ? t1[kb] : 0;
            q1[b] = t1 ? t1[tn + kb] : 0;
            v[b] = col[kb];
        }
#pragma unroll
        for (int b = 0; b < OB; b++) {
            acc[0].mac(v[b], p0[b]);
            acc[1].mac(v[b], p1[b]);
            if (t1) {
                acc[2].mac(v[b], q0[b]);
                acc[3].mac(v[b], q1[b]);
            }
        }
    }
    for (; k < n; k += 256) {
        const uint64_t v = col[k];
        acc[0].mac(v, t0[k]);
        acc[1].mac(v, t0[tn + k]);
        if (t1) {
            acc[2].mac(v, t1[k]);
            acc[3].mac(v, t1[tn + k]);
        }
    }
#pragma unroll
    for (int q = 0; q < 4; q++) s[q][threadIdx.x] = gl::canon(acc[q].reduce());
    __syncthreads();
    for (int off = 128; off > 0; off >>= 1) {
        if ((int)threadIdx.x < off)
            for (int q = 0; q < 4; q++) s[q][threadIdx.x] = gl::add(s[q][threadIdx.x], s[q][threadIdx.x + off]);
        __syncthreads();
    }
    if (threadIdx.x < 4) out4[threadIdx.x] = s[threadIdx.x][0];
}

__global__ void __launch_bounds__(256) openings_kernel(const uint64_t* __restrict__ coeffs, size_t n, uint32_t ncols,
                                                      const uint64_t* __restrict__ t0, const uint64_t* __restrict__ t1,
                                                      uint64_t* __restrict__ out) {
    openings_column(coeffs + (size_t)blockIdx.x * n, n, t0, t1, n, out + (size_t)blockIdx.x * 4);
}
__global__ void __launch_bounds__(256) openings_seg_kernel(const uint64_t* __restrict__ coeffs, size_t n, size_t seg_len,
                                                          const uint64_t* __restrict__ t0, const uint64_t* __restrict__ t1,
                                                          uint64_t* __restrict__ partial) {
    const size_t lo = (size_t)blockIdx.y * seg_len, len = min(seg_len, n - lo);
    openings_column(coeffs + (size_t)blockIdx.x * n + lo, len, t0 + lo, t1 ? t1 + lo : nullptr, n,
                    partial + ((size_t)blockIdx.x * gridDim.y + blockIdx.y) * 4);
}
__global__ void __launch_bounds__(256) openings_fold_kernel(const uint64_t* __restrict__ partial, uint32_t ncols, uint32_t segs,
                                                           uint64_t* __restrict__ out) {
    const uint32_t i = blockIdx.x * blockDim.x + threadIdx.x;
    if (i >= 4 * ncols) return;
    const uint64_t* p = partial + (size_t)(i >> 2) * segs * 4 + (i & 3);
    uint64_t acc = 0;
    for (uint32_t sg = 0; sg < segs; sg++) acc = gl::add(acc, p[4 * sg]);
    out[i] = acc;
}

struct Open3Args {
    const uint64_t* coeffs[3];
    uint32_t ncols[3];
    size_t n;
    const uint64_t *t0, *t1;
    uint64_t* out;
};
__global__ void __launch_bounds__(256) openings3_kernel(Open3Args a) {
    const uint32_t b = blockIdx.x;
    const uint64_t* col;
    const uint64_t* t1 = a.t1;
    if (b < a.ncols[0]) {
        col = a.coeffs[0] + (size_t)b * a.n;
    } else if (b < a.ncols[0] + a.ncols[1]) {
        col = a.coeffs[1] + (size_t)(b - a.ncols[0]) * a.n;
    } else {
        col = a.coeffs[2] + (size_t)(b - a.ncols[0] - a.ncols[1]) * a.n;
        t1 = nullptr;
    }
    openings_column(col, a.n, a.t0, t1, a.n, a.out + (size_t)b * 4);
}

constexpr int OG = 4;
struct OpenGArgs {
    const uint64_t* coeffs[3];
    uint32_t ncols[3];
    size_t n, seg_len;
    const uint64_t *t0, *t1;
    uint64_t* partial;
};
__global__ void __launch_bounds__(256) openings_group_kernel(OpenGArgs a) {
    __shared__ uint64_t s[4][256];
    uint32_t g = blockIdx.x, orc = 0, col_base = 0;
    while (orc < 2 && g >= (a.ncols[orc] + OG - 1) / OG) {
        g -= (a.ncols[orc] + OG - 1) / OG;
        col_base += a.ncols[orc];
        orc++;
    }
    const uint32_t c0 = g * OG, cnt = min((uint32_t)OG, a.ncols[orc] - c0);
    const bool two = orc < 2;
    const size_t n = a.n, lo = (size_t)blockIdx.y * a.seg_len, hi = min(n, lo + a.seg_len);
    const uint64_t* col = a.coeffs[orc] + (size_t)c0 * n;
    gl::Acc160 acc[OG][4];
    constexpr int OB = 2;
    size_t k = lo + threadIdx.x;
    for (; k + (OB - 1) * 256 < hi; k += OB * 256) {
        uint64_t p0[OB], p1[OB], q0[OB], q1[OB], v[OB][OG];
#pragma unroll
        for (int b = 0; b < OB; b++) {
            const size_t kb = k + (size_t)b * 256;
            p0[b] = a.t0[kb];
            p1[b] = a.t0[n + kb];
            q0[b] = two ? a.t1[kb] : 0;
            q1[b] = two ? a.t1[n + kb] : 0;
#pragma unroll
            for (int c = 0; c < OG; c++) v[b][c] = (uint32_t)c < cnt ? col[(size_t)c * n + kb] : 0;
        }
#pragma unroll
        for (int b = 0; b < OB; b++)
#pragma unroll
            for (int c = 0; c < OG; c++) {
                if ((uint32_t)c >= cnt) break;
                acc[c][0].mac(v[b][c], p0[b]);
                acc[c][1].mac(v[b][c], p1[b]);
                if (two) {
                    acc[c][2].mac(v[b][c], q0[b]);
                    acc[c][3].mac(v[b][c], q1[b]);
                }
            }
    }
    for (; k < hi; k += 256) {
        const uint64_t p0 = a.t0[k], p1 = a.t0[n + k], q0 = two ? a.t1[k] : 0, q1 = two ? a.t1[n + k] : 0;
#pragma unroll
        for (int c = 0; c < OG; c++) {
            if ((uint32_t)c >= cnt) break;
            const uint64_t v = col[(size_t)c * n + k];
            acc[c][0].mac(v, p0);
            acc[c][1].mac(v, p1);
            if (two) {
                acc[c][2].mac(v, q0);
                acc[c][3].mac(v, q1);
            }
        }
    }
#pragma unroll
    for (int c = 0; c < OG; c++) {
        if ((uint32_t)c >= cnt) break;
#pragma unroll
        for (int q = 0; q < 4; q++) s[q][threadIdx.x] = gl::canon(acc[c][q].reduce());
        __syncthreads();
        for (int off = 128; off > 0; off >>= 1) {
            if ((int)threadIdx.x < off)
                for (int q = 0; q < 4; q++) s[q][threadIdx.x] = gl::add(s[q][threadIdx.x], s[q][threadIdx.x + off]);
            __syncthreads();
        }
        if (threadIdx.x < 4) a.partial[((size_t)(col_base + c0 + c) * gridDim.y + blockIdx.y) * 4 + threadIdx.x] = s[threadIdx.x][0];
        __syncthreads();
    }
}

struct CombArgs {
    const uint64_t* src[3];
    int cnt[3];
    size_t n;
    const uint32_t* apow3;
    int n1;
    int slices;
    uint64_t* partial;
};
__global__ void __launch_bounds__(256) fri_combine_kernel(CombArgs a) {
    const size_t k = (size_t)blockIdx.x * 256 + threadIdx.x;
    const int total = a.cnt[0] + a.cnt[1] + a.cnt[2];
    const int per = (total + a.slices - 1) / a.slices;
    const int c_lo = blockIdx.y * per, c_hi = min(total, c_lo + per);
    gl::Acc6 G0, G1, H0, H1;
    G0.zero(); G1.zero(); H0.zero(); H1.zero();
    const uint64_t *src0 = a.src[0], *src1 = a.src[1], *src2 = a.src[2];
    const int cnt0 = a.cnt[0], cnt01 = a.cnt[0] + a.cnt[1], n1 = a.n1;
    const size_t nn = a.n;
    const uint32_t* __restrict__ apow3 = a.apow3;
    auto col_of = [=](int c) -> const uint64_t* {
        return c < cnt0 ? src0 + (size_t)c * nn : c < cnt01 ? src1 + (size_t)(c - cnt0) * nn : src2 + (size_t)(c - cnt01) * nn;
    };
#define SIPP_COMB_TERM(cc, vv)                                             \
    do {                                                                   \
        const uint64_t v_ = (vv);                                          \
        const uint32_t lo_ = (uint32_t)v_, hi_ = (uint32_t)(v_ >> 32);     \
        const uint32_t* __restrict__ w_ = apow3 + 6 * (cc);                \
        if ((cc) < n1) {                                 \
            G0.mac(lo_, hi_, w_);                                          \
            G1.mac(lo_, hi_, w_ + 3);                                      \
        } else {                                                           \
            H0.mac(lo_, hi_, w_);                                          \
            H1.mac(lo_, hi_, w_ + 3);                                      \
        }                                                                  \
    } while (0)
    constexpr int CB = 8;
    int c = c_lo;
    for (; c + CB <= c_hi; c += CB) {
        uint64_t v[CB];
#pragma unroll
        for (int b = 0; b < CB; b++) v[b] = col_of(c + b)[k];
#pragma unroll
        for (int b = 0; b < CB; b++) SIPP_COMB_TERM(c + b, v[b]);
    }
    for (; c < c_hi; c++) SIPP_COMB_TERM(c, col_of(c)[k]);
#undef SIPP_COMB_TERM
    const uint64_t g0 = gl::canon(G0.reduce()), g1 = gl::canon(G1.reduce());
    uint64_t* p = a.partial + (size_t)blockIdx.y * 4 * a.n;
    p[k] = gl::add(g0, gl::canon(H0.reduce()));
    p[a.n + k] = gl::add(g1, gl::canon(H1.reduce()));
    p[2 * a.n + k] = g0;
    p[3 * a.n + k] = g1;
}

struct GCombArgs {
    const uint64_t* const* cols;
    int total;
    size_t n;
    const uint32_t* apow3;
    int slices;
    uint64_t* partial;
};
__global__ void __launch_bounds__(256) fri_gcombine_kernel(GCombArgs a) {
    const size_t k = (size_t)blockIdx.x * 256 + threadIdx.x;
    const int per = (a.total + a.slices - 1) / a.slices;
    const int c_lo = blockIdx.y * per, c_hi = min(a.total, c_lo + per);
    gl::Acc6 G0, G1;
    G0.zero(); G1.zero();
    for (int c = c_lo; c < c_hi; c++) {
        const uint64_t v = a.cols[c][k];
        const uint32_t lo = (uint32_t)v, hi = (uint32_t)(v >> 32);
        const uint32_t* __restrict__ w = a.apow3 + 6 * c;
        G0.mac(lo, hi, w);
        G1.mac(lo, hi, w + 3);
    }
    uint64_t* p = a.partial + (size_t)blockIdx.y * 4 * a.n;
    p[k] = gl::canon(G0.reduce());
    p[a.n + k] = gl::canon(G1.reduce());
}

// ... 167 lines not shown
            const uint32_t l = e >> 2, w = e & 3;
            size_t off = 0;
            for (uint32_t k = 0; k < l; k++) off += (size_t)1 << (t.b - k);
            const size_t node = ((x >> t.d) >> l) ^ 1;
            t.out[((size_t)q * t.c + l) * 4 + w] = t.src[(off + node) * 4 + w];
        }
    } else {
        const size_t leaf = x >> t.b;
        for (uint32_t e = threadIdx.x; e < (2u << t.c); e += blockDim.x)
            t.out[((size_t)q << (t.c + 1)) + e] = t.src[(size_t)(e & 1) * t.a + (leaf << t.c) + (e >> 1)];
    }
}

}

int sipp_k_gather_tasks(sipp_ctx* ctx, const QueryGatherTask* d_tasks, uint32_t n_tasks, const uint32_t* d_idx, uint32_t nq) {
    if (!n_tasks || !nq) return SIPP_OK;
    ProfScope ps(ctx, "query_gather");
    hipLaunchKernelGGL(gather_tasks_kernel, dim3(nq, n_tasks), dim3(256), 0, ctx->stream, d_tasks, d_idx);
    SIPP_CHECK_HIP(ctx, hipGetLastError());
    return SIPP_OK;
}

int sipp_k_z_columns(sipp_ctx* ctx, const air_spec_t* a, const uint64_t* d_trace, uint32_t log_n, const uint64_t beta[2],
                     const uint64_t gamma[2], uint64_t* d_zv) {
    const size_t n = (size_t)1 << log_n;
    const int P = 2 * a->n_checked;
    const int zr = (n >= 16384) ? 8 : 4;
    const size_t zblock = (size_t)256 * zr;
    const unsigned nblk = (unsigned)(n / zblock);
    if (n % zblock) return sipp_fail(ctx, SIPP_E_BADARG, "z_columns: n must be a multiple of 1024");
    ArenaScope scope(ctx);
    uint64_t* totals = arena_alloc_t<uint64_t>(ctx, (size_t)2 * P * nblk);
    if (!totals) return SIPP_E_NOMEM;
    {
        ProfScope ps(ctx, "z_phase_a");
        if (zr == 8)
            hipLaunchKernelGGL(z_phase_a<8>, dim3(nblk, P / 2), dim3(256), 0, ctx->stream, d_trace, n, a->n_main, a->n_checked,
                               a->checked_base, gamma[0], gamma[1], beta[0], beta[1], d_zv, totals);
        else
            hipLaunchKernelGGL(z_phase_a<4>, dim3(nblk, P / 2), dim3(256), 0, ctx->stream, d_trace, n, a->n_main, a->n_checked,
                               a->checked_base, gamma[0], gamma[1], beta[0], beta[1], d_zv, totals);
    }
    {
        ProfScope ps(ctx, "z_phase_bc");
        hipLaunchKernelGGL(z_phase_b, dim3(P), dim3(256), 0, ctx->stream, totals, (int)nblk);
        if (zr == 8)
            hipLaunchKernelGGL(z_phase_c<8>, dim3(nblk, P), dim3(256), 0, ctx->stream, d_zv, n, totals);
        else
            hipLaunchKernelGGL(z_phase_c<4>, dim3(nblk, P), dim3(256), 0, ctx->stream, d_zv, n, totals);
    }
    SIPP_CHECK_HIP(ctx, hipGetLastError());
    return SIPP_OK;
}

static void host_ntt(uint64_t* a, uint32_t log_n, bool inverse) {
    const size_t n = (size_t)1 << log_n;
    for (size_t i = 0; i < n; i++) {
        const size_t j = gl::bitrev((uint32_t)i, log_n);
        if (i < j) std::swap(a[i], a[j]);
    }
    uint64_t root = gl::root_of_unity(log_n);
    if (inverse) root = gl::inv(root);
    for (uint32_t s = 1; s <= log_n; s++) {
        const size_t mlen = (size_t)1 << s, h = mlen >> 1;
        uint64_t wm = root;
        for (uint32_t k = s; k < log_n; k++) wm = gl::sqr(wm);
        for (size_t k = 0; k < n; k += mlen) {
            uint64_t w = 1;
            for (size_t j = 0; j < h; j++) {
                const uint64_t t = gl::mul(w, a[k + j + h]), u = a[k + j];
                a[k + j] = gl::add(u, t);
                a[k + j + h] = gl::sub(u, t);
                w = gl::mul(w, wm);
            }
        }
    }
    if (inverse) {
        const uint64_t ninv = gl::inv((uint64_t)n);
        for (size_t i = 0; i < n; i++) a[i] = gl::mul(a[i], ninv);
    }
}

int sipp_k_quotient(sipp_ctx* ctx, const air_spec_t* a, uint32_t log_n, const uint64_t* d_lde, const uint64_t* d_zlde,
                    size_t lde_stride, const uint64_t* d_aux, const uint64_t alpha[2], const uint64_t beta[2],
                    const uint64_t gamma[2], uint64_t* d_out) {
    const uint32_t log_m = log_n + 1;
    const size_t n = (size_t)1 << log_n, m = (size_t)1 << log_m;
    QuotArgs q{};
    q.lde = d_lde; q.zlde = d_zlde; q.aux = d_aux; q.lde_stride = lde_stride;
    q.prog = sipp_air_prog_device(ctx, a);
    if (!q.prog) return SIPP_E_HIP;
    q.prog_len = a->prog_len;
    q.W = a->n_main + 2 * a->n_checked; q.nm = a->n_main; q.nc = a->n_checked; q.cbase = a->checked_base;
    q.tbits = a->table_bits; q.log_n = log_n; q.log_m = log_m;
    q.alpha[0] = alpha[0]; q.alpha[1] = alpha[1]; q.gamma[0] = gamma[0]; q.gamma[1] = gamma[1];
    q.beta[0] = beta[0]; q.beta[1] = beta[1];
    const uint64_t g = gl::root_of_unity(log_n), wm = gl::root_of_unity(log_m);
    for (int k = 0; k < AIR_N_PERIODIC; k++) {
        const uint64_t mk = (uint64_t)AIR_PERIODIC[k][0], r0 = (uint64_t)AIR_PERIODIC[k][1];
        uint64_t* t = sipp_table_get(ctx, 200 + k, log_n, 0);
        if (!t) {
            const uint64_t K = n / mk;
            std::vector<uint64_t> v(2 * mk);
            const uint64_t gs = gl::inv(gl::pow(g, r0)), scale = gl::mul(K % gl::P, gl::inv(n % gl::P));
            for (uint64_t i = 0; i < 2 * mk; i++) {
                uint64_t x = gl::mul(gl::GEN, gl::pow(wm, i));
                uint64_t y = gl::mul(x, gs);
                uint64_t num = gl::sub(gl::pow(y, n), 1), den = gl::sub(gl::pow(y, K), 1);
                v[i] = gl::mul(gl::mul(num, gl::inv(den)), scale);
            }
            SIPP_TRY(sipp_table_put(ctx, 200 + k, log_n, 0, v, &t));
        }
        q.per_tab[k] = t;
        q.per_mask[k] = (uint32_t)(2 * mk - 1);
    }
    q.vper_tab = nullptr;
    q.vper_mask = 0;
    if (a->n_vflag + a->n_vconst > 0) {
        const uint32_t lr = (uint32_t)a->log_rows;
        const size_t R = (size_t)1 << lr, R2 = 2 * R;
        const int nv = a->n_vflag + a->n_vconst;
        uint64_t* t = sipp_table_get(ctx, 104, log_n, (uint64_t)a->kind);
        if (!t) {
            std::vector<uint64_t> tab((size_t)nv * R2), col(R2);
            const uint64_t shift = gl::pow(gl::GEN, (uint64_t)1 << (log_n - lr));
            std::map<std::vector<int64_t>, int> seen;
            std::vector<int64_t> vals(R);
            for (int k = 0; k < nv; k++) {
                for (size_t r = 0; r < R; r++) vals[r] = air_vper_value(a, k, (int)r);
                auto it = seen.find(vals);
                if (it != seen.end()) {
                    memcpy(&tab[(size_t)k * R2], &tab[(size_t)it->second * R2], R2 * 8);
                    continue;
                }
                seen.emplace(vals, k);
                for (size_t r = 0; r < R; r++) col[r] = gl::from_i64(vals[r]);
                host_ntt(col.data(), lr, true);
                uint64_t f = 1;
                for (size_t j = 0; j < R; j++) {
                    col[j] = gl::mul(col[j], f);
                    f = gl::mul(f, shift);
                }
                for (size_t j = R; j < R2; j++) col[j] = 0;
                host_ntt(col.data(), lr + 1, false);
                memcpy(&tab[(size_t)k * R2], col.data(), R2 * 8);
            }
            SIPP_TRY(sipp_table_put(ctx, 104, log_n, (uint64_t)a->kind, tab, &t));
        }
        q.vper_tab = t;
        q.vper_mask = (uint32_t)(R2 - 1);
    }
    const uint64_t sN = gl::pow(gl::GEN, n);
    q.zh[0] = gl::sub(sN, 1);
    q.zh[1] = gl::sub(gl::neg(sN), 1);
    q.zh_inv[0] = gl::inv(q.zh[0]);
    q.zh_inv[1] = gl::inv(q.zh[1]);
    q.ninv = gl::inv(n % gl::P);
    q.g_inv = gl::inv(g);
    q.w_m = wm;
    for (int i = 0; i < 16; i++) q.p_limbs[i] = AIR_BN_P_LIMBS[i];
    q.out = d_out;
    for (int ch = 0; ch < 2; ch++) {
        if (alpha[ch] == 0) return sipp_fail(ctx, SIPP_E_UNSUPPORTED, "quotient: a zero constraint challenge");
        const uint64_t gi = gl::inv(alpha[ch]);
        q.gamma_inv[ch] = gi;
        q.alpha16[ch] = gl::pow(alpha[ch], 16);
        uint64_t x = 1;
        for (int i = 0; i < 8; i++) {
            q.ginv3[ch][i][0] = (uint32_t)x & 0x3FFFFFu;
            q.ginv3[ch][i][1] = (uint32_t)(x >> 22) & 0x3FFFFFu;
            q.ginv3[ch][i][2] = (uint32_t)(x >> 44);
            x = gl::mul(x, gi);
        }
    }
    int n_gadget_segs = 0;
    ArenaScope scope(ctx);
    {
        std::vector<uint32_t> off, cnt;
        std::vector<int> ncons;
        const int64_t* w = a->prog;
        const int64_t* end = a->prog + a->prog_len;
        while (w < end && w[0] == 1) {
            off.push_back((uint32_t)(w - a->prog));
            cnt.push_back(0);
            if (w[6] != 2) return sipp_fail(ctx, SIPP_E_UNSUPPORTED, "quotient: gadgets must pair their limbs (group 2)");
            ncons.push_back(32 / (int)w[6] + 1);
            w += 7;
            w += 2 + 5 * w[1];
            int64_t np = *w++;
            for (int64_t p = 0; p < np; p++) {
                w += 1;
                w += 2 + 5 * w[1];
                w += 2 + 5 * w[1];
            }
            int64_t nl = *w++;
            for (int64_t p = 0; p < nl; p++) {
                w += 1;
                w += 2 + 5 * w[1];
            }
            if (np > 64) {
                const uint32_t nsl = (uint32_t)std::min<int64_t>(SIPP_QUOTIENT_MAX_SLICES, (np + 39) / 40);
                cnt.back() = 0x80000000u | (nsl << 8);
                for (uint32_t k = 1; k < nsl; k++) {
                    off.push_back(off.back());
                    cnt.push_back(0x80000000u | (nsl << 8) | k);
                    ncons.push_back(0);
                }
            }
        }
        while (w < end) {
            off.push_back((uint32_t)(w - a->prog));
            uint32_t k = 0;
            while (w < end && k < 64) {
                int64_t nmono = w[1];
                w += 2;
                for (int64_t mo = 0; mo < nmono; mo++) w += 2 + 2 * w[1];
                k++;
            }
            cnt.push_back(k);
            ncons.push_back((int)k);
        }
        const int ns = (int)off.size();
        q.n_seg = ns;
        n_gadget_segs = 0;
        auto is_gadget = [](uint32_t c) { return c == 0 || (c >> 31) != 0; };
        while (n_gadget_segs < ns && is_gadget(cnt[n_gadget_segs])) n_gadget_segs++;
        for (int g = n_gadget_segs; g < ns; g++)
            if (is_gadget(cnt[g])) return sipp_fail(ctx, SIPP_E_UNSUPPORTED, "quotient: gadgets must precede the polynomial constraints");
        std::vector<uint64_t> host((size_t)ns * 2 + ns + 2 + 192, 0);
        int after = 0;
        for (int g = ns - 1; g >= 0; g--) {
            host[2 * g] = gl::pow(alpha[0], (uint64_t)after);
            host[2 * g + 1] = gl::pow(alpha[1], (uint64_t)after);
            after += ncons[g];
        }
        uint32_t* h32 = reinterpret_cast<uint32_t*>(&host[2 * ns]);
        memcpy(h32, off.data(), (size_t)ns * 4);
        memcpy(h32 + ns, cnt.data(), (size_t)ns * 4);
        const size_t ap_at = (size_t)ns * 2 + (((size_t)2 * ns + 1) >> 1);
        {
            uint32_t* ap = reinterpret_cast<uint32_t*>(&host[ap_at]);
            for (int ch = 0; ch < 2; ch++) {
                uint64_t x = 1;
                for (int e = 0; e < 64; e++) {
                    ap[(ch * 64 + e) * 3 + 0] = (uint32_t)x & 0x3FFFFFu;
                    ap[(ch * 64 + e) * 3 + 1] = (uint32_t)(x >> 22) & 0x3FFFFFu;
                    ap[(ch * 64 + e) * 3 + 2] = (uint32_t)(x >> 44);
                    x = gl::mul(x, alpha[ch]);
                }
            }
        }
        uint64_t* d_tab = arena_alloc_t<uint64_t>(ctx, host.size());
        q.part = arena_alloc_t<uint64_t>(ctx, (size_t)ns * 2 * m);
        if (!d_tab || !q.part) return SIPP_E_NOMEM;
        SIPP_CHECK_HIP(ctx, hipMemcpyAsync(d_tab, host.data(), host.size() * 8, hipMemcpyHostToDevice, ctx->stream));
        SIPP_CHECK_HIP(ctx, hipStreamSynchronize(ctx->stream));
        q.seg_pow = d_tab;
        q.seg_off = reinterpret_cast<const uint32_t*>(d_tab + 2 * ns);
        q.seg_cnt = q.seg_off + ns;
        q.apoly3 = reinterpret_cast<const uint32_t*>(d_tab + ap_at);
    }
    {
        q.K = 3 + 6 * a->n_checked;
        const int nw = 6 + 12 * a->n_checked;
        uint32_t* d_ap = arena_alloc_t<uint32_t>(ctx, (size_t)3 * nw);
        if (!d_ap) return SIPP_E_NOMEM;
        hipLaunchKernelGGL(alpha_pow3_kernel, dim3((unsigned)((nw + 255) / 256)), dim3(256), 0, ctx->stream, alpha[0], alpha[1],
                           q.K, a->n_checked, d_ap);
        q.apow3 = d_ap;
        q.alphaK[0] = gl::pow(alpha[0], (uint64_t)q.K);
        q.alphaK[1] = gl::pow(alpha[1], (uint64_t)q.K);
    }
    {
        ProfScope ps(ctx, "quotient_prog");
        if (n_gadget_segs)
            hipLaunchKernelGGL(quotient_prog_kernel<false>, dim3((unsigned)(m / 64), (unsigned)n_gadget_segs), dim3(64), 0, ctx->stream, q, 0);
        if (q.n_seg > n_gadget_segs)
            hipLaunchKernelGGL(quotient_prog_kernel<true>, dim3((unsigned)(m / 64), (unsigned)(q.n_seg - n_gadget_segs)), dim3(64), 0, ctx->stream,
                               q, n_gadget_segs);
    }
    {
        ProfScope ps(ctx, "quotient_rest");
        q.chunks = (int)sipp_quotient_rest_chunks(log_n, a->n_checked);
        if (q.chunks > 1) {
            q.rest_part = arena_alloc_t<uint64_t>(ctx, (size_t)q.chunks * 6 * m);
            if (!q.rest_part) return SIPP_E_NOMEM;
            hipLaunchKernelGGL(quotient_rest_kernel<true>, dim3((unsigned)(m / 256), (unsigned)q.chunks), dim3(256), 0, ctx->stream, q);
            hipLaunchKernelGGL(quotient_finish_kernel, dim3((unsigned)(m / 256)), dim3(256), 0, ctx->stream, q);
        } else {
            q.chunks = 1;
            hipLaunchKernelGGL(quotient_rest_kernel<false>, dim3((unsigned)(m / 256)), dim3(256), 0, ctx->stream, q);
        }
    }
    SIPP_CHECK_HIP(ctx, hipGetLastError());
    return SIPP_OK;
}

int sipp_k_pow_table(sipp_ctx* ctx, gl::E2 base, size_t n, uint64_t* d_tab) {
    ProfScope ps(ctx, "pow_table");
    hipLaunchKernelGGL(pow_table_kernel, dim3((unsigned)((n + 255) / 256)), dim3(256), 0, ctx->stream, base, n, d_tab);
    SIPP_CHECK_HIP(ctx, hipGetLastError());
    return SIPP_OK;
}

int sipp_k_pow_table4(sipp_ctx* ctx, const gl::E2 base[4], size_t n, uint64_t* const d_tab[4]) {
    ProfScope ps(ctx, "pow_table");
    Pow4Args a;
    for (int i = 0; i < 4; i++) {
        a.base[i] = base[i];
        a.tab[i] = d_tab[i];
    }
    a.n = n;
    hipLaunchKernelGGL(pow_table4_kernel, dim3((unsigned)((n + 255) / 256), 4), dim3(256), 0, ctx->stream, a);
    SIPP_CHECK_HIP(ctx, hipGetLastError());
    return SIPP_OK;
}

int sipp_k_openings(sipp_ctx* ctx, const uint64_t* d_coeffs, size_t ncols, size_t n, const uint64_t* d_t0,
                    const uint64_t* d_t1, uint64_t* d_out) {
    if (!ncols) return SIPP_OK;
    ProfScope ps(ctx, "openings");
    const size_t want = (2048 + ncols - 1) / ncols, segs = std::min<size_t>(std::min<size_t>(64, want), n / 1024);
    if (segs <= 1) {
        hipLaunchKernelGGL(openings_kernel, dim3((unsigned)ncols), dim3(256), 0, ctx->stream, d_coeffs, n, (uint32_t)ncols, d_t0, d_t1,
                           d_out);
    } else {
        ArenaScope scope(ctx);
        uint64_t* partial = arena_alloc_t<uint64_t>(ctx, ncols * segs * 4);
        if (!partial) return SIPP_E_NOMEM;
        const size_t seg_len = (n + segs - 1) / segs;
        hipLaunchKernelGGL(openings_seg_kernel, dim3((unsigned)ncols, (unsigned)segs), dim3(256), 0, ctx->stream, d_coeffs, n, seg_len,
                           d_t0, d_t1, partial);
        hipLaunchKernelGGL(openings_fold_kernel, dim3((unsigned)((4 * ncols + 255) / 256)), dim3(256), 0, ctx->stream, partial,
                           (uint32_t)ncols, (uint32_t)segs, d_out);
    }
    SIPP_CHECK_HIP(ctx, hipGetLastError());
    return SIPP_OK;
}

int sipp_k_openings3(sipp_ctx* ctx, const uint64_t* const d_coeffs[3], const uint32_t ncols[3], size_t n, const uint64_t* d_t0,
                     const uint64_t* d_t1, uint64_t* d_out) {
    const unsigned total = ncols[0] + ncols[1] + ncols[2];
    if (!total) return SIPP_OK;
    ProfScope ps(ctx, "openings");
    Open3Args a;
    for (int i = 0; i < 3; i++) {
        a.coeffs[i] = d_coeffs[i];
        a.ncols[i] = ncols[i];
    }
    a.n = n; a.t0 = d_t0; a.t1 = d_t1; a.out = d_out;
    const bool grouped = !(ctx->kernel_routes & SIPP_ROUTE_OPENINGS_UNGROUPED);
    if (!grouped || n < 1024) {
        hipLaunchKernelGGL(openings3_kernel, dim3(total), dim3(256), 0, ctx->stream, a);
        SIPP_CHECK_HIP(ctx, hipGetLastError());
        return SIPP_OK;
    }
    OpenGArgs g;
    unsigned groups = 0;
    for (int i = 0; i < 3; i++) {
        g.coeffs[i] = d_coeffs[i];
        g.ncols[i] = ncols[i];
        groups += (ncols[i] + OG - 1) / OG;
    }
    const size_t segs = std::max<size_t>(1, std::min<size_t>(std::min<size_t>(SIPP_OPENINGS_MAX_SEGS, (4096 + groups - 1) / groups), n / 1024));
    ArenaScope scope(ctx);
    g.partial = arena_alloc_t<uint64_t>(ctx, (size_t)total * segs * 4);
    if (!g.partial) return SIPP_E_NOMEM;
    g.n = n; g.seg_len = (n + segs - 1) / segs; g.t0 = d_t0; g.t1 = d_t1;
    hipLaunchKernelGGL(openings_group_kernel, dim3(groups, (unsigned)segs), dim3(256), 0, ctx->stream, g);
    hipLaunchKernelGGL(openings_fold_kernel, dim3((4 * total + 255) / 256), dim3(256), 0, ctx->stream, g.partial, (uint32_t)total,
                       (uint32_t)segs, d_out);
    SIPP_CHECK_HIP(ctx, hipGetLastError());
    return SIPP_OK;
}

int sipp_k_fri_final(sipp_ctx* ctx, const uint64_t* const src[3], const int cnt[3], size_t n, const uint32_t* d_apow3,
                     int n1, gl::E2 shift1, const uint64_t* d_zp[2], const uint64_t* d_zip[2], uint64_t* d_final) {
    ArenaScope scope(ctx);
    const int total_cols = cnt[0] + cnt[1] + cnt[2];
    int slices = 8;
    while (slices < 64 && ((n / 256) * (size_t)slices < 2048 || (total_cols + slices - 1) / slices > 1024)) slices *= 2;
    uint64_t* partial = arena_alloc_t<uint64_t>(ctx, (size_t)slices * 4 * n);
    uint64_t* q = arena_alloc_t<uint64_t>(ctx, 4 * n);
    if (!partial || !q) return SIPP_E_NOMEM;
    CombArgs c{};
    for (int i = 0; i < 3; i++) { c.src[i] = src[i]; c.cnt[i] = cnt[i]; }
    c.n = n; c.apow3 = d_apow3; c.n1 = n1; c.slices = slices; c.partial = partial;
    if ((cnt[0] + cnt[1] + cnt[2] + slices - 1) / slices > 1024) return sipp_fail(ctx, SIPP_E_UNSUPPORTED, "fri_combine: more than 1024 columns per slice");
    {
        ProfScope ps(ctx, "fri_combine");
        hipLaunchKernelGGL(fri_combine_kernel, dim3((unsigned)(n / 256), slices), dim3(256), 0, ctx->stream, c);
    }
    DivArgs d{};
    d.partial = partial; d.slices = slices; d.n = n;
    d.zp[0] = d_zp[0]; d.zp[1] = d_zp[1]; d.zip[0] = d_zip[0]; d.zip[1] = d_zip[1];
    d.qout = q;
    const unsigned ntiles = (unsigned)(n / 1024);
    uint64_t* scan = arena_alloc_t<uint64_t>(ctx, 4 * n);
    uint64_t* totals = arena_alloc_t<uint64_t>(ctx, (size_t)4 * ntiles);
    if (!scan || !totals) return SIPP_E_NOMEM;
    if (n % 1024) return sipp_fail(ctx, SIPP_E_BADARG, "fri_divide: n must be a multiple of 1024");
    {
        ProfScope ps(ctx, "fri_divide");
        hipLaunchKernelGGL(fri_divide_tiles, dim3(ntiles, 2), dim3(1024), 0, ctx->stream, d, scan, totals);
        hipLaunchKernelGGL(fri_divide_carry, dim3(2), dim3(256), 0, ctx->stream, totals, (int)ntiles);
        hipLaunchKernelGGL(fri_divide_finish, dim3(ntiles, 2), dim3(1024), 0, ctx->stream, d, scan, totals);
        hipLaunchKernelGGL(fri_final_kernel, dim3((unsigned)((n + 255) / 256)), dim3(256), 0, ctx->stream, q, n, shift1, d_final);
    }
    SIPP_CHECK_HIP(ctx, hipGetLastError());
    return SIPP_OK;
}

int sipp_k_fri_batch_quotient(sipp_ctx* ctx, const uint64_t* const* d_cols, int total, size_t n, const uint32_t* d_apow3,
                              const uint64_t* d_zp, const uint64_t* d_zip, gl::E2 shift, bool first, uint64_t* d_acc) {
    ArenaScope scope(ctx);
    int slices = 1;
    while (slices < 64 && ((n / 256) * (size_t)slices < 1024 || (total + slices - 1) / slices > 1024)) slices *= 2;
    if ((total + slices - 1) / slices > 1024) return sipp_fail(ctx, SIPP_E_UNSUPPORTED, "fri: more than 65536 polynomials in one batch");
    if (n % 1024) return sipp_fail(ctx, SIPP_E_BADARG, "fri: degree must be a multiple of 1024");
    uint64_t* partial = arena_alloc_t<uint64_t>(ctx, (size_t)slices * 4 * n);
    uint64_t* q = arena_alloc_t<uint64_t>(ctx, 4 * n);
    uint64_t* scan = arena_alloc_t<uint64_t>(ctx, 4 * n);
    const unsigned ntiles = (unsigned)(n / 1024);
    uint64_t* totals = arena_alloc_t<uint64_t>(ctx, (size_t)4 * ntiles);
    if (!partial || !q || !scan || !totals) return SIPP_E_NOMEM;
    GCombArgs c{};
    c.cols = d_cols; c.total = total; c.n = n; c.apow3 = d_apow3; c.slices = slices; c.partial = partial;
    DivArgs d{};
    d.partial = partial; d.slices = slices; d.n = n;
    d.zp[0] = d_zp; d.zp[1] = d_zp; d.zip[0] = d_zip; d.zip[1] = d_zip;
    d.qout = q;
    {
        ProfScope ps(ctx, "fri_combine");
        hipLaunchKernelGGL(fri_gcombine_kernel, dim3((unsigned)(n / 256), slices), dim3(256), 0, ctx->stream, c);
    }
    {
        ProfScope ps(ctx, "fri_divide");
        hipLaunchKernelGGL(fri_divide_tiles, dim3(ntiles, 1), dim3(1024), 0, ctx->stream, d, scan, totals);
        hipLaunchKernelGGL(fri_divide_carry, dim3(1), dim3(256), 0, ctx->stream, totals, (int)ntiles);
        hipLaunchKernelGGL(fri_divide_finish, dim3(ntiles, 1), dim3(1024), 0, ctx->stream, d, scan, totals);
        hipLaunchKernelGGL(fri_accum_kernel, dim3((unsigned)((n + 255) / 256)), dim3(256), 0, ctx->stream, d_acc, q, n, shift, first ? 1 : 0);
    }
    SIPP_CHECK_HIP(ctx, hipGetLastError());
    return SIPP_OK;
}
int sipp_k_fri_mulx(sipp_ctx* ctx, const uint64_t* d_acc, size_t n, uint64_t* d_final) {
    hipLaunchKernelGGL(fri_mulx_kernel, dim3((unsigned)((n + 255) / 256)), dim3(256), 0, ctx->stream, d_acc, n, d_final);
    SIPP_CHECK_HIP(ctx, hipGetLastError());
    return SIPP_OK;
}

int sipp_k_fri_fold(sipp_ctx* ctx, const uint64_t* d_in, size_t len_in, uint32_t arity_bits, gl::E2 beta, uint64_t* d_out) {
    size_t len_out = len_in >> arity_bits;
    ProfScope ps(ctx, "fri_fold");
// ... 33 lines not shown
```

sipp_amd/csrc/prover.hpp:

```cpp
#pragma once
#include <functional>

#include "ctx.hpp"
#include "host_challenger.hpp"
#include "host_poseidon.hpp"
#include "poseidon_constants.h"

inline uint32_t sipp_quotient_rest_chunks(uint32_t log_n, int n_checked) {
    if (log_n + 1 > 15) return 1;
    const int c = n_checked / 32 < 16 ? n_checked / 32 : 16;
    return c > 1 ? (uint32_t)c : 1;
}
int sipp_k_z_columns(sipp_ctx* ctx, const air_spec_t* a, const uint64_t* d_trace, uint32_t log_n, const uint64_t beta[2],
                     const uint64_t gamma[2], uint64_t* d_zv);
int sipp_k_quotient(sipp_ctx* ctx, const air_spec_t* a, uint32_t log_n, const uint64_t* d_lde, const uint64_t* d_zlde,
                    size_t lde_stride, const uint64_t* d_aux, const uint64_t alpha[2], const uint64_t beta[2],
                    const uint64_t gamma[2], uint64_t* d_out);
int sipp_k_pow_table(sipp_ctx* ctx, gl::E2 base, size_t n, uint64_t* d_tab);
int sipp_k_pow_table4(sipp_ctx* ctx, const gl::E2 base[4], size_t n, uint64_t* const d_tab[4]);
int sipp_k_openings(sipp_ctx* ctx, const uint64_t* d_coeffs, size_t ncols, size_t n, const uint64_t* d_t0,
                    const uint64_t* d_t1, uint64_t* d_out);
constexpr size_t SIPP_OPENINGS_MAX_SEGS = 32;
constexpr int SIPP_QUOTIENT_MAX_SLICES = 8;
int sipp_k_openings3(sipp_ctx* ctx, const uint64_t* const d_coeffs[3], const uint32_t ncols[3], size_t n, const uint64_t* d_t0,
                     const uint64_t* d_t1, uint64_t* d_out);
int sipp_k_fri_final(sipp_ctx* ctx, const uint64_t* const src[3], const int cnt[3], size_t n, const uint32_t* d_apow3,
                     int n1, gl::E2 shift1, const uint64_t* d_zp[2], const uint64_t* d_zip[2], uint64_t* d_final);
int sipp_k_fri_batch_quotient(sipp_ctx* ctx, const uint64_t* const* d_cols, int total, size_t n, const uint32_t* d_apow3,
                              const uint64_t* d_zp, const uint64_t* d_zip, gl::E2 shift, bool first, uint64_t* d_acc);
int sipp_k_fri_mulx(sipp_ctx* ctx, const uint64_t* d_acc, size_t n, uint64_t* d_final);
int sipp_k_fri_fold(sipp_ctx* ctx, const uint64_t* d_in, size_t len_in, uint32_t arity_bits, gl::E2 beta, uint64_t* d_out);
struct QueryGatherTask {
    const uint64_t* src;
    uint64_t* out;
    uint64_t a;
    uint32_t type, b, c, d;
};
int sipp_k_gather_tasks(sipp_ctx* ctx, const QueryGatherTask* d_tasks, uint32_t n_tasks, const uint32_t* d_idx, uint32_t nq);
int sipp_k_gather_rows(sipp_ctx* ctx, const uint64_t* d_lde, size_t m, uint32_t ncols, const uint32_t* d_idx, uint32_t nq,
                       uint64_t* d_out);
int sipp_k_gather_siblings(sipp_ctx* ctx, const uint64_t* d_tree, uint32_t log_leaves, uint32_t nsib, uint32_t shift,
                           const uint32_t* d_idx, uint32_t nq, uint64_t* d_out);
int sipp_k_gather_fri_leaf(sipp_ctx* ctx, const uint64_t* d_vals, size_t len, uint32_t shift, uint32_t arity_bits,
                           const uint32_t* d_idx, uint32_t nq, uint64_t* d_out);
int sipp_k_fri_leaves(sipp_ctx* ctx, const uint64_t* d_vals, size_t len, uint32_t arity_bits, uint64_t* d_digests);
int sipp_k_pow_search(sipp_ctx* ctx, const uint64_t state[12], const uint64_t* in_buf, uint32_t n_in, uint32_t resp_word,
                      uint32_t pow_bits, uint64_t* witness);


struct FriOracleDev {
    const uint64_t* lde;
    size_t stride;
    uint32_t ncols;
    const uint64_t* tree;
};
struct FriParamsDev {
    uint32_t rate_bits = 1, cap_height = 4, pow_bits = 16, num_queries = 84, pow_rule = 0;
    std::vector<uint32_t> arity_bits;
};
size_t sipp_fri_core_words(const FriParamsDev& p, uint32_t log_n, const uint32_t* leaf_words, int n_oracles);
int sipp_fri_prove_core(sipp_ctx* ctx, const FriOracleDev* ors, int n_oracles, uint32_t log_n, const FriParamsDev& p,
                        uint64_t* d_final, host::Challenger& ch, uint64_t* pf, size_t& pos, size_t cap_total, size_t* final_len,
                        const std::function<void(const char*)>& tick);
```

sipp_amd/csrc/stark.hip:

```cpp
#include <atomic>
#include <thread>
#include <algorithm>
#include <chrono>

#include "prover.hpp"

static const int IO_WORDS[7] = {SIPP_G1_IO_WORDS, SIPP_G2_IO_WORDS, SIPP_FQ12_IO_WORDS, SIPP_MAP_G2_IO_WORDS, SIPP_G1_IO_WORDS, SIPP_G2_IO_WORDS,
                                SIPP_PAIRING_IO_WORDS};
static inline int base_kind(int kind) {
    return (kind == SIPP_G1_EXP_HARDENED || kind == SIPP_G2_EXP_HARDENED) ? kind - SIPP_G1_EXP_HARDENED : kind;
}
static inline int ctx_kind(const sipp_ctx* ctx, int kind) {
    return (ctx && ctx->hardened && (kind == SIPP_G1_EXP || kind == SIPP_G2_EXP)) ? kind + SIPP_G1_EXP_HARDENED : kind;
}
#define SIPP_MAGIC 0x5349505053544b31ULL

struct Shape {
    const air_spec_t* air;
    uint32_t log_n;
    uint32_t num_io;
    int W, P, Q;
};

static int shape_of(int kind, size_t num_io, Shape* s) {
    if (kind < 0 || kind > SIPP_PAIRING || num_io == 0 || num_io > ((size_t)1 << 17)) return SIPP_E_BADARG;
    const uint32_t log_rows = kind == SIPP_MAP_G2 ? 3 : kind == SIPP_PAIRING ? AIR_PAIRING_LOG_ROWS : 9;
    uint32_t nio = 2;
    while (nio < num_io || ((size_t)nio << log_rows) < 1024) nio <<= 1;
    uint32_t log_n = log_rows;
    while ((1u << (log_n - log_rows)) < nio) log_n++;
    s->air = sipp_air_get(kind, log_n);
    if (!s->air || (uint32_t)s->air->log_rows != log_rows) return SIPP_E_UNSUPPORTED;
    s->log_n = log_n;
    s->num_io = nio;
    s->W = s->air->n_main + 2 * s->air->n_checked;
    s->P = 2 * s->air->n_checked;
    s->Q = 4;
    return SIPP_OK;
}

static FriParamsDev fri_params_of(const sipp_stark_config& c, uint32_t degree_bits) {
    FriParamsDev p;
    p.rate_bits = c.rate_bits; p.cap_height = c.cap_height; p.pow_bits = c.pow_bits; p.num_queries = c.num_queries;
    p.pow_rule = c.pow_rule;
    while (degree_bits > c.final_poly_bits && degree_bits + c.rate_bits - c.arity_bits >= c.cap_height &&
           degree_bits >= c.arity_bits && p.arity_bits.size() < 32) {
        p.arity_bits.push_back(c.arity_bits);
        degree_bits -= c.arity_bits;
    }
    return p;
}

static size_t proof_words(const sipp_stark_config& cfg, const Shape& s) {
    const FriParamsDev fp = fri_params_of(cfg, s.log_n);
    const uint32_t log_m = s.log_n + cfg.rate_bits;
    const size_t cap = (size_t)4 << cfg.cap_height;
    size_t w = 16 + 3 * cap + 2 * (size_t)(2 * s.W + 2 * s.P + s.Q);
    const uint32_t leaf_words[3] = {(uint32_t)s.W, (uint32_t)s.P, (uint32_t)s.Q};
    w += sipp_fri_core_words(fp, s.log_n, leaf_words, 3);
    w += (size_t)s.num_io * s.air->pi_per_io;
    (void)log_m;
    return w;
}

static int upload_ios(sipp_ctx* ctx, int kind, const uint32_t* ios, size_t num_io, const Shape& s, uint32_t** d_ios,
                      std::vector<uint32_t>* host_copy) {
    const size_t ppi = IO_WORDS[kind];
    const size_t words = (size_t)s.num_io * ppi;
    if (words * 4 > ctx->h_pinned_words * 8) return sipp_fail(ctx, SIPP_E_NOMEM, "IO list larger than the pinned staging buffer");
    uint32_t* h = reinterpret_cast<uint32_t*>(ctx->h_pinned);
    for (size_t io = 0; io < s.num_io; io++)
        memcpy(h + io * ppi, ios + (io < num_io ? io : num_io - 1) * ppi, ppi * 4);
    if (host_copy) host_copy->assign(h, h + words);
    *d_ios = arena_alloc_t<uint32_t>(ctx, words);
    if (!*d_ios) return SIPP_E_NOMEM;
    SIPP_CHECK_HIP(ctx, hipMemcpyAsync(*d_ios, h, words * 4, hipMemcpyHostToDevice, ctx->stream));
    SIPP_CHECK_HIP(ctx, hipStreamSynchronize(ctx->stream));
    return SIPP_OK;
}

static size_t tree_words(uint32_t log_leaves) { return ((size_t)8 << log_leaves); }

static int read_cap(sipp_ctx* ctx, const uint64_t* d_tree, uint32_t log_leaves, uint64_t* cap_host) {
    const uint32_t ch = std::min(ctx->cfg.cap_height, log_leaves);
    uint64_t off = 0;
    for (uint32_t l = 0; l < log_leaves - ch; l++) off += (uint64_t)1 << (log_leaves - l);
    SIPP_CHECK_HIP(ctx, hipMemcpyAsync(cap_host, d_tree + 4 * off, ((size_t)4 << ch) * 8, hipMemcpyDeviceToHost, ctx->stream));
    SIPP_CHECK_HIP(ctx, hipStreamSynchronize(ctx->stream));
    return SIPP_OK;
}

static int commit_coeffs_launch(sipp_ctx* ctx, const uint64_t* d_coeffs, size_t ncols, uint32_t log_n, uint64_t* d_lde,
                                uint64_t* d_tree) {
    const uint32_t log_m = log_n + ctx->cfg.rate_bits;
    int rc = sipp_lde_from_coeffs(ctx, d_coeffs, d_lde, ncols, log_n, ctx->cfg.rate_bits);
    if (rc == SIPP_E_UNSUPPORTED)
        rc = sipp_ntt_dif(ctx, d_coeffs, (size_t)1 << log_n, log_n, d_lde, (size_t)1 << log_m, log_m, ncols, false,
                          NttDiag{gl::GEN, 0});
    SIPP_TRY(rc);
    SIPP_TRY(sipp_k_poseidon_leaves(ctx, d_lde, (size_t)1 << log_m, ncols, log_m, d_tree));
    return sipp_k_merkle_levels(ctx, d_tree, log_m, ctx->cfg.cap_height);
}
static int commit_coeffs(sipp_ctx* ctx, const uint64_t* d_coeffs, size_t ncols, uint32_t log_n, uint64_t* d_lde,
                         uint64_t* d_tree, uint64_t* cap_host) {
    SIPP_TRY(commit_coeffs_launch(ctx, d_coeffs, ncols, log_n, d_lde, d_tree));
    return read_cap(ctx, d_tree, log_n + ctx->cfg.rate_bits, cap_host);
}

static int commit_values_launch(sipp_ctx* ctx, const uint64_t* d_values, size_t ncols, uint32_t log_n, uint64_t* d_coeffs,
                                uint64_t* d_lde, uint64_t* d_tree) {
    const size_t n = (size_t)1 << log_n;
    const uint32_t log_m = log_n + ctx->cfg.rate_bits;
    const int rc = sipp_lde_from_values(ctx, d_values, d_coeffs, d_lde, ncols, log_n, ctx->cfg.rate_bits);
    if (rc == SIPP_OK) {
        SIPP_TRY(sipp_k_poseidon_leaves(ctx, d_lde, (size_t)1 << log_m, ncols, log_m, d_tree));
        return sipp_k_merkle_levels(ctx, d_tree, log_m, ctx->cfg.cap_height);
    }
    if (rc != SIPP_E_UNSUPPORTED) return rc;
    SIPP_TRY(sipp_bitrev_cols(ctx, d_values, n, d_coeffs, n, log_n, ncols));
    SIPP_TRY(sipp_ntt_dit(ctx, d_coeffs, n, log_n, ncols, true, NttDiag{}));
    return commit_coeffs_launch(ctx, d_coeffs, ncols, log_n, d_lde, d_tree);
}
static int commit_values(sipp_ctx* ctx, const uint64_t* d_values, size_t ncols, uint32_t log_n, uint64_t* d_coeffs,
                         uint64_t* d_lde, uint64_t* d_tree, uint64_t* cap_host) {
    SIPP_TRY(commit_values_launch(ctx, d_values, ncols, log_n, d_coeffs, d_lde, d_tree));
    return read_cap(ctx, d_tree, log_n + ctx->cfg.rate_bits, cap_host);
}

static void host_ifft(std::vector<uint64_t>& a, uint32_t log_n) {
    const size_t n = (size_t)1 << log_n;
    for (size_t i = 0; i < n; i++) {
        size_t j = gl::bitrev((uint32_t)i, log_n);
        if (i < j) std::swap(a[i], a[j]);
    }
    const uint64_t root = gl::inv(gl::root_of_unity(log_n));
    for (uint32_t s = 1; s <= log_n; s++) {
        const size_t mlen = (size_t)1 << s, h = mlen >> 1;
        uint64_t wm = root;
        for (uint32_t k = s; k < log_n; k++) wm = gl::sqr(wm);
        for (size_t k = 0; k < n; k += mlen) {
            uint64_t w = 1;
            for (size_t j = 0; j < h; j++) {
                uint64_t t = gl::mul(w, a[k + j + h]), u = a[k + j];
                a[k + j] = gl::add(u, t);
                a[k + j + h] = gl::sub(u, t);
                w = gl::mul(w, wm);
            }
        }
    }
    const uint64_t ninv = gl::inv((uint64_t)n);
    for (auto& v : a) v = gl::mul(v, ninv);
}

static void fq12_tower_limbs(const uint32_t* c96, int t, uint16_t limbs[16]) {
    static const uint64_t P[4] = {0x3c208c16d87cfd47ULL, 0x97816a916871ca8dULL, 0xb85045b68181585dULL, 0x30644e72e131a029ULL};
    typedef unsigned __int128 u128;
    const int i = t >> 1;
    uint64_t r[5] = {0, 0, 0, 0, 0};
    auto load = [&](int k, uint64_t out[4]) {
        for (int q = 0; q < 4; q++) out[q] = (uint64_t)c96[8 * k + 2 * q] | ((uint64_t)c96[8 * k + 2 * q + 1] << 32);
    };
    uint64_t hi[4];
    load(i + 6, hi);
    if (t & 1) {
        memcpy(r, hi, 32);
    } else {
        uint64_t lo[4];
        load(i, lo);
        u128 carry = 0;
        for (int q = 0; q < 4; q++) {
            carry += (u128)hi[q] * 9 + lo[q];
// ... 67 lines not shown

static int prove_impl(sipp_ctx* ctx, int kind, const uint32_t* ios, size_t num_io_in, uint64_t* proof_out, size_t proof_cap,
                      size_t* proof_len) {
    if (!ctx || !ios || !proof_out || !proof_len) return SIPP_E_BADARG;
    kind = ctx_kind(ctx, kind);
    struct GateGuard {
        sipp_ctx* c;
        ~GateGuard() {
            if (c->gate_release) c->gate_release->release();
            c->gate_release = nullptr;
        }
    } gate_guard{ctx};
    SIPP_CHECK_HIP(ctx, hipSetDevice(ctx->device));
    const sipp_stark_config& cfg = ctx->cfg;
    Shape s;
    SIPP_TRY(shape_of(kind, num_io_in, &s));
    const air_spec_t* a = s.air;
    const FriParamsDev fp = fri_params_of(cfg, s.log_n);
    const uint32_t log_n = s.log_n, log_m = log_n + cfg.rate_bits, R = (uint32_t)fp.arity_bits.size();
    if (R > 0 && log_m < (R - 1) * cfg.arity_bits + 4)
        return sipp_fail(ctx, SIPP_E_UNSUPPORTED, "stark: arity_bits / final_poly_bits fold the FRI layers below 16 values for this trace length");
    const uint32_t log_mq = log_n + 1;
    const size_t n = (size_t)1 << log_n, m = (size_t)1 << log_m, mq = (size_t)1 << log_mq;
    const size_t final_len = n >> (R * cfg.arity_bits);
    const int W = s.W, P = s.P, Q = s.Q;
    const uint32_t nq = cfg.num_queries;
    (void)nq;
    const size_t cap_words = (size_t)4 << cfg.cap_height;
    const size_t total_words = proof_words(cfg, s);
    if (proof_cap < total_words) return sipp_fail(ctx, SIPP_E_BUFSZ, "proof buffer too small (see sipp_proof_size)");
    if (n < ((size_t)1 << a->table_bits)) return sipp_fail(ctx, SIPP_E_UNSUPPORTED, "trace shorter than the range table");

    static const bool host_timing = getenv("SIPP_HOST_TIMING") != nullptr;
    auto t_prev = std::chrono::steady_clock::now();
    auto tick = [&](const char* what) {
        if (!host_timing) return;
        (void)hipStreamSynchronize(ctx->stream);
        auto now = std::chrono::steady_clock::now();
        fprintf(stderr, "[sipp kind %d] %-18s %8.3f ms\n", kind, what, std::chrono::duration<double, std::milli>(now - t_prev).count());
        t_prev = now;
    };
    ArenaMark mark = arena_mark(ctx);
    struct Release {
        sipp_ctx* c;
        ArenaMark m;
        ~Release() {
            (void)hipStreamSynchronize(c->stream);
            arena_release(c, m);
        }
    } release{ctx, mark};

    uint64_t* pf = proof_out;
    size_t pos = 0;
    auto push = [&](const uint64_t* v, size_t cnt) {
        memcpy(pf + pos, v, cnt * 8);
        pos += cnt;
    };
    {
        uint64_t hdr[16] = {SIPP_MAGIC, (uint64_t)kind, log_n, s.num_io, (uint64_t)W, (uint64_t)P, (uint64_t)Q, cfg.cap_height,
                            R, (uint64_t)final_len, nq, (uint64_t)a->pi_per_io, total_words, cfg.rate_bits, cfg.arity_bits,
                            (uint64_t)(cfg.fs_rule | (cfg.lookup_rule << 1))};
        push(hdr, 16);
    }

    std::vector<uint32_t> pis;
    uint32_t* d_ios = nullptr;
    SIPP_TRY(upload_ios(ctx, kind, ios, num_io_in, s, &d_ios, &pis));
    int* d_err = arena_alloc_t<int>(ctx, 1);
    uint64_t* d_trace = arena_alloc_t<uint64_t>(ctx, (size_t)W * n);
    Oracle3 T{arena_alloc_t<uint64_t>(ctx, (size_t)W * n), arena_alloc_t<uint64_t>(ctx, (size_t)W * m),
              arena_alloc_t<uint64_t>(ctx, tree_words(log_m)), W};
    Oracle3 Z{arena_alloc_t<uint64_t>(ctx, (size_t)P * n), arena_alloc_t<uint64_t>(ctx, (size_t)P * m),
              arena_alloc_t<uint64_t>(ctx, tree_words(log_m)), P};
    Oracle3 Qo{arena_alloc_t<uint64_t>(ctx, (size_t)2 * mq), arena_alloc_t<uint64_t>(ctx, (size_t)Q * m),
               arena_alloc_t<uint64_t>(ctx, tree_words(log_m)), Q};
    if (!d_err || !d_trace || !T.coeffs || !T.lde || !T.tree || !Z.coeffs || !Z.lde || !Z.tree || !Qo.coeffs || !Qo.lde ||
        !Qo.tree)
        return SIPP_E_NOMEM;
    if (!pis_canonical(kind, pis.data(), s.num_io))
        return sipp_fail(ctx, SIPP_E_WITNESS, "IO record holds a non-canonical field element (>= p)");
    SIPP_CHECK_HIP(ctx, hipMemsetAsync(d_err, 0, sizeof(int), ctx->stream));
    SIPP_TRY(sipp_trace_fill(ctx, a, d_ios, s.num_io, log_n, d_trace, d_err));
    {
        int h_err = 0;
        SIPP_CHECK_HIP(ctx, hipMemcpyAsync(&h_err, d_err, sizeof(int), hipMemcpyDeviceToHost, ctx->stream));
        SIPP_CHECK_HIP(ctx, hipStreamSynchronize(ctx->stream));
        if (h_err) return sipp_fail(ctx, h_err, "trace fill: IO record not provable (claimed output wrong, degenerate point or non-canonical limbs)");
    }

    tick("trace fill");
    if (ctx->gate_release) {
        ctx->gate_release->release();
        ctx->gate_release = nullptr;
    }
    if (ctx->gate_wait) {
        ctx->gate_wait->wait();
        ctx->gate_wait = nullptr;
    }
    uint64_t cap_host[4 << 8];

    SIPP_TRY(commit_values_launch(ctx, d_trace, (size_t)W, log_n, T.coeffs, T.lde, T.tree));
    host::Challenger ch;
    if (cfg.fs_rule == SIPP_FS_STATEMENT) {
        const uint64_t st[16] = {(uint64_t)kind, log_n, s.num_io, (uint64_t)W, (uint64_t)P, (uint64_t)Q, cfg.rate_bits,
                                 cfg.cap_height, cfg.pow_bits, cfg.arity_bits, cfg.final_poly_bits, cfg.num_queries,
                                 cfg.num_challenges, cfg.pow_rule, (uint64_t)a->pi_per_io, (uint64_t)cfg.lookup_rule};
        uint64_t root[4];
        ch.observe_many(st, 16);
        pi_root(pis.data(), s.num_io, a->pi_per_io, root);
        ch.observe_many(root, 4);
    }
    const int n_aux = a->n_aux;
    const uint32_t log_io = log_n - (uint32_t)a->log_rows;
    const size_t nio = s.num_io;
    std::vector<uint64_t> auxc((size_t)n_aux * nio), col(nio);
    {
        const uint64_t g = gl::root_of_unity(log_n);
        for (int ai = 0; ai < n_aux; ai++) {
            const int word = a->aux[4 * ai], part = a->aux[4 * ai + 1], shift = a->aux[4 * ai + 2], sub = a->aux[4 * ai + 3];
            for (size_t io = 0; io < nio; io++) {
                const uint32_t* rec = &pis[io * a->pi_per_io];
                if (part == 3) {
                    uint16_t limbs[16];
                    fq12_tower_limbs(rec + word, sub / 16, limbs);
                    col[io] = limbs[sub % 16];
                } else {
                    uint32_t w = rec[word];
                    col[io] = part == 0 ? (w & 0xffff) : part == 1 ? (w >> 16) : w;
                }
            }
            host_ifft(col, log_io);
            if (shift) {
                const uint64_t sft = gl::inv(gl::pow(g, (uint64_t)shift));
                uint64_t f = 1;
                for (size_t j = 0; j < nio; j++) {
                    col[j] = gl::mul(col[j], f);
                    f = gl::mul(f, sft);
                }
            }
            memcpy(&auxc[(size_t)ai * nio], col.data(), nio * 8);
        }
    }
    SIPP_TRY(read_cap(ctx, T.tree, log_m, cap_host));
    ch.observe_many(cap_host, cap_words);
    push(cap_host, cap_words);
    tick("trace commit");

    uint64_t beta[2], gamma[2];
    for (int i = 0; i < 2; i++) {
        beta[i] = ch.get();
        gamma[i] = ch.get();
        if (cfg.lookup_rule == SIPP_LOOKUP_SHARED) beta[i] = gamma[i];
    }
    {
        ArenaMark mz = arena_mark(ctx);
        uint64_t* d_zv = arena_alloc_t<uint64_t>(ctx, (size_t)P * n);
        if (!d_zv) return SIPP_E_NOMEM;
        SIPP_TRY(sipp_k_z_columns(ctx, a, d_trace, log_n, beta, gamma, d_zv));
        SIPP_TRY(commit_values(ctx, d_zv, (size_t)P, log_n, Z.coeffs, Z.lde, Z.tree, cap_host));
        arena_release(ctx, mz);
    }
    ch.observe_many(cap_host, cap_words);
    push(cap_host, cap_words);

    tick("Z + commit");
    uint64_t alpha[2];
    alpha[0] = ch.get();
    alpha[1] = ch.get();

    {
        ArenaMark mark_q = arena_mark(ctx);
        uint64_t* d_auxc = arena_alloc_t<uint64_t>(ctx, (size_t)n_aux * nio + 1);
        uint64_t* d_aux = arena_alloc_t<uint64_t>(ctx, (size_t)n_aux * mq + 1);
        if (!d_auxc || !d_aux) return SIPP_E_NOMEM;
        SIPP_CHECK_HIP(ctx, hipMemcpyAsync(d_auxc, auxc.data(), auxc.size() * 8, hipMemcpyHostToDevice, ctx->stream));
        SIPP_CHECK_HIP(ctx, hipStreamSynchronize(ctx->stream));
        if (n_aux) {
            int rc_aux = sipp_tree_coset_eval(ctx, d_auxc, d_aux, (size_t)n_aux, log_io, log_mq);
            if (rc_aux == SIPP_E_UNSUPPORTED)
                rc_aux = sipp_ntt_dif(ctx, d_auxc, nio, log_io, d_aux, mq, log_mq, (size_t)n_aux, false, NttDiag{gl::GEN, 0});
            SIPP_TRY(rc_aux);
        }
        SIPP_TRY(sipp_k_quotient(ctx, a, log_n, T.lde, Z.lde, m, d_aux, alpha, beta, gamma, Qo.coeffs));
        SIPP_TRY(sipp_ntt_dit(ctx, Qo.coeffs, mq, log_mq, 2, true, NttDiag{gl::inv(gl::GEN), 0}));
        SIPP_TRY(commit_coeffs(ctx, Qo.coeffs, (size_t)Q, log_n, Qo.lde, Qo.tree, cap_host));
        arena_release(ctx, mark_q);
    }
    ch.observe_many(cap_host, cap_words);
    push(cap_host, cap_words);

    tick("quotient + commit");
    const gl::E2 zeta = ch.get_ext();
    if (gl::eq(gl::pow(zeta, (uint64_t)n), gl::e2(1))) return sipp_fail(ctx, SIPP_E_SUBGROUP, "zeta in the trace subgroup");
    const gl::E2 gzeta = gl::scale(zeta, gl::root_of_unity(log_n));
    uint64_t* d_zp[2] = {arena_alloc_t<uint64_t>(ctx, 2 * n), arena_alloc_t<uint64_t>(ctx, 2 * n)};
    uint64_t* d_zip[2] = {arena_alloc_t<uint64_t>(ctx, 2 * n), arena_alloc_t<uint64_t>(ctx, 2 * n)};
    uint64_t* d_open = arena_alloc_t<uint64_t>(ctx, (size_t)(W + P + Q) * 4);
    if (!d_zp[0] || !d_zp[1] || !d_zip[0] || !d_zip[1] || !d_open) return SIPP_E_NOMEM;
    {
        const gl::E2 bases[4] = {zeta, gzeta, gl::inv(zeta), gl::inv(gzeta)};
        uint64_t* const tabs[4] = {d_zp[0], d_zp[1], d_zip[0], d_zip[1]};
        SIPP_TRY(sipp_k_pow_table4(ctx, bases, n, tabs));
    }
    {
        const uint64_t* const cf[3] = {T.coeffs, Z.coeffs, Qo.coeffs};
        const uint32_t nc3[3] = {(uint32_t)W, (uint32_t)P, (uint32_t)Q};
        SIPP_TRY(sipp_k_openings3(ctx, cf, nc3, n, d_zp[0], d_zp[1], d_open));
    }
    std::vector<uint64_t> hop((size_t)(W + P + Q) * 4);
    SIPP_CHECK_HIP(ctx, hipMemcpyAsync(hop.data(), d_open, hop.size() * 8, hipMemcpyDeviceToHost, ctx->stream));
    SIPP_CHECK_HIP(ctx, hipStreamSynchronize(ctx->stream));
    {
        for (int c = 0; c < W; c++) push(&hop[(size_t)c * 4], 2);
        for (int c = 0; c < W; c++) push(&hop[(size_t)c * 4 + 2], 2);
        for (int c = 0; c < P; c++) push(&hop[(size_t)(W + c) * 4], 2);
        for (int c = 0; c < P; c++) push(&hop[(size_t)(W + c) * 4 + 2], 2);
        for (int c = 0; c < Q; c++) push(&hop[(size_t)(W + P + c) * 4], 2);
        for (int c = 0; c < W; c++) ch.observe_many(&hop[(size_t)c * 4], 2);
        for (int c = 0; c < P; c++) ch.observe_many(&hop[(size_t)(W + c) * 4], 2);
        for (int c = 0; c < Q; c++) ch.observe_many(&hop[(size_t)(W + P + c) * 4], 2);
        for (int c = 0; c < W; c++) ch.observe_many(&hop[(size_t)c * 4 + 2], 2);
        for (int c = 0; c < P; c++) ch.observe_many(&hop[(size_t)(W + c) * 4 + 2], 2);
    }

    tick("openings+observe");
    const gl::E2 fa = ch.get_ext();
    uint64_t* d_final = arena_alloc_t<uint64_t>(ctx, 2 * n);
    {
        std::vector<uint32_t> apow((size_t)(W + P + Q) * 6);
        gl::E2 ap = gl::e2(1);
        for (int c = 0; c < W + P + Q; c++) {
            const uint64_t comp[2] = {ap.c0, ap.c1};
            for (int q = 0; q < 2; q++) {
                apow[6 * c + 3 * q] = (uint32_t)comp[q] & 0x3FFFFFu;
                apow[6 * c + 3 * q + 1] = (uint32_t)(comp[q] >> 22) & 0x3FFFFFu;
                apow[6 * c + 3 * q + 2] = (uint32_t)(comp[q] >> 44);
            }
            ap = gl::mul(ap, fa);
        }
        uint32_t* d_apow = arena_alloc_t<uint32_t>(ctx, apow.size());
        if (!d_final || !d_apow) return SIPP_E_NOMEM;
        SIPP_CHECK_HIP(ctx, hipMemcpyAsync(d_apow, apow.data(), apow.size() * 4, hipMemcpyHostToDevice, ctx->stream));
        SIPP_CHECK_HIP(ctx, hipStreamSynchronize(ctx->stream));
        const uint64_t* src[3] = {T.coeffs, Z.coeffs, Qo.coeffs};
        const int cnt[3] = {W, P, Q};
        const uint64_t* zp[2] = {d_zp[0], d_zp[1]};
        const uint64_t* zip[2] = {d_zip[0], d_zip[1]};
        SIPP_TRY(sipp_k_fri_final(ctx, src, cnt, n, d_apow, W + P, gl::pow(fa, (uint64_t)(W + P)), zp, zip, d_final));
    }
    {
        const FriOracleDev ors[3] = {{T.lde, m, (uint32_t)W, T.tree}, {Z.lde, m, (uint32_t)P, Z.tree}, {Qo.lde, m, (uint32_t)Q, Qo.tree}};
        size_t flen = 0;
        SIPP_TRY(sipp_fri_prove_core(ctx, ors, 3, log_n, fp, d_final, ch, pf, pos, total_words, &flen, tick));
        if (flen != final_len) return sipp_fail(ctx, SIPP_E_BUFSZ, "internal: final polynomial length mismatch");
    }
    for (size_t k = 0; k < pis.size(); k++) pf[pos++] = pis[k];
    tick("queries+assemble");
    if (pos != total_words) return sipp_fail(ctx, SIPP_E_BUFSZ, "internal: proof length mismatch");
    *proof_len = pos;
    return SIPP_OK;
}

extern "C" {

int sipp_stark_shape(const sipp_ctx* ctx, int kind, size_t num_io, uint32_t* log_rows, uint32_t* main_cols,
                     uint32_t* perm_cols, uint32_t* quotient_cols) {
    kind = ctx_kind(ctx, kind);
    Shape s;
    SIPP_TRY(shape_of(kind, num_io, &s));
    if (log_rows) *log_rows = s.log_n;
    if (main_cols) *main_cols = (uint32_t)s.W;
    if (perm_cols) *perm_cols = (uint32_t)s.P;
    if (quotient_cols) *quotient_cols = (uint32_t)s.Q;
    return SIPP_OK;
}

int sipp_io_shard(size_t num_io, uint32_t world, uint32_t rank, size_t* first, size_t* count) {
    if (!first || !count || world == 0 || rank >= world || num_io > SIZE_MAX / world) return SIPP_E_BADARG;
    const size_t lo = num_io * rank / world, hi = num_io * ((size_t)rank + 1) / world;
    *first = lo;
    *count = hi - lo;
    return SIPP_OK;
}

size_t sipp_workspace_bytes(int kind, size_t num_io) { return sipp_workspace_bytes_cfg(kind, num_io, nullptr); }

int sipp_device_memory(int device, size_t* free_bytes, size_t* total_bytes) {
    int ndev = 0;
    if (hipGetDeviceCount(&ndev) != hipSuccess || device < 0 || device >= ndev) return SIPP_E_HIP;
    int prev = 0;
    (void)hipGetDevice(&prev);
    size_t fr = 0, tot = 0;
    if (hipSetDevice(device) != hipSuccess || hipMemGetInfo(&fr, &tot) != hipSuccess) return SIPP_E_HIP;
    (void)hipSetDevice(prev);
    if (free_bytes) *free_bytes = fr;
    if (total_bytes) *total_bytes = tot;
    return SIPP_OK;
}

size_t sipp_workspace_bytes_cfg(int kind, size_t num_io, const sipp_stark_config* cfg) {
    Shape s;
    if (shape_of(kind, num_io, &s) != SIPP_OK) return 0;
    const uint32_t rate_bits = cfg ? cfg->rate_bits : 1;
    if (rate_bits < 1 || rate_bits > 3) return 0;
    const size_t n = (size_t)1 << s.log_n, m = n << rate_bits;
    const size_t W = (size_t)s.W, P = (size_t)s.P, Q = (size_t)s.Q, nc = (size_t)s.air->n_checked;
    size_t words = n * (2 * W + 3 * P)
                   + m * (W + P + Q + 2 + (size_t)s.air->n_aux)
                   + 3 * 8 * m
                   + 2 * m * (1 + (size_t)s.air->n_gadgets + (size_t)s.air->n_constraints / 64 + 2 +
                              (kind == SIPP_PAIRING ? SIPP_QUOTIENT_MAX_SLICES : 0))
                   + (sipp_quotient_rest_chunks(s.log_n, s.air->n_checked) > 1
                          ? (size_t)sipp_quotient_rest_chunks(s.log_n, s.air->n_checked) * 6 * 2 * n : 0)
                   + (W + P + Q) * SIPP_OPENINGS_MAX_SEGS * 4
                   + 80 * n;
    size_t bytes = 8 * words + nc * ((size_t)16 << s.air->table_bits)
                   + n * 400
                   + ((size_t)64 << 20);
    return bytes + bytes / 16;
}

size_t sipp_proof_size(const sipp_ctx* ctx, int kind, size_t num_io) {
    kind = ctx_kind(ctx, kind);
    Shape s;
    if (!ctx || shape_of(kind, num_io, &s) != SIPP_OK) return 0;
    return proof_words(ctx->cfg, s);
// ... 372 lines not shown
```

Measured before the change: 2406 pairings/s.

## Trim prover tail host round-trips: pinned staging, device alpha tables, pipelined openings

Moves several host round-trips in the STARK tail onto pinned staging buffers. Alpha-power and quotient segment tables are now built on the device instead of on the host and uploaded. Openings are split into ranges, each copied back with its own event, so the challenger can start absorbing while later ranges are still computing. The PoW grind now double-buffers batches and exits early once a witness is found. This cuts synchronisations and pageable copies, but reuses the shared pinned buffer in several places, which risks aliasing, and adds more launch and event overhead.

```diff
diff --git a/__graft_entry__.py b/__graft_entry__.py
--- a/__graft_entry__.py
+++ b/__graft_entry__.py
@@ -17,6 +17,7 @@
     import subprocess
     subprocess.check_call(["make", "-C", os.path.join(ROOT, "tests", "host"), "-s"])
     subprocess.check_call(["make", "-C", os.path.join(ROOT, "tests", "probe"), "-s"])
+    subprocess.check_call(["make", "-C", os.path.join(ROOT, "tests", "probe_tail"), "-s"])
 
 
 def smoke():
diff --git a/include/sipp_hip.h b/include/sipp_hip.h
--- a/include/sipp_hip.h
+++ b/include/sipp_hip.h
@@ -63,6 +63,9 @@
 #define SIPP_ROUTE_OPENINGS_UNGROUPED 1u
 #define SIPP_ROUTE_LDE_COLUMN_WIDE 2u
 #define SIPP_ROUTE_WITNESS_NO_GRAPH 4u
+#define SIPP_ROUTE_OPENING_RANGES_SHIFT 4
+#define SIPP_ROUTE_OPENING_RANGES_MASK 0xF0u
+#define SIPP_ROUTE_OPENING_RANGES(k) (((uint32_t)(k) << SIPP_ROUTE_OPENING_RANGES_SHIFT) & SIPP_ROUTE_OPENING_RANGES_MASK)
 int sipp_ctx_set_kernel_routes(sipp_ctx *ctx, uint32_t routes);
 void sipp_ctx_destroy(sipp_ctx *ctx);
 int sipp_ctx_set_stream_priority(sipp_ctx *ctx, int level);
diff --git a/sipp_amd/csrc/api.hip b/sipp_amd/csrc/api.hip
--- a/sipp_amd/csrc/api.hip
+++ b/sipp_amd/csrc/api.hip
@@ -74,6 +74,9 @@
     if (hipEventCreate(&ctx->t0) != hipSuccess || hipEventCreate(&ctx->t1) != hipSuccess) return bail(SIPP_E_HIP);
     ctx->h_pinned_words = (size_t)1 << 23;
     if (hipHostMalloc((void**)&ctx->h_pinned, ctx->h_pinned_words * 8) != hipSuccess) return bail(SIPP_E_NOMEM);
+    if (hipHostMalloc((void**)&ctx->h_stage, SIPP_STAGE_WORDS * 8) != hipSuccess) return bail(SIPP_E_NOMEM);
+    for (auto& e : ctx->ev_tail)
+        if (hipEventCreateWithFlags(&e, hipEventDisableTiming) != hipSuccess) return bail(SIPP_E_HIP);
     int rc = sipp_poseidon_init_constants(ctx);
     if (rc != SIPP_OK) return bail(rc);
     *out = ctx;
@@ -99,6 +102,9 @@
     if (ctx->t0) (void)hipEventDestroy(ctx->t0);
     if (ctx->t1) (void)hipEventDestroy(ctx->t1);
     if (ctx->h_pinned) (void)hipHostFree(ctx->h_pinned);
+    if (ctx->h_stage) (void)hipHostFree(ctx->h_stage);
+    for (auto e : ctx->ev_tail)
+        if (e) (void)hipEventDestroy(e);
     if (ctx->arena) (void)hipFree(ctx->arena);
     if (ctx->aux_stream) (void)hipStreamDestroy(ctx->aux_stream);
     if (ctx->aux2_stream) (void)hipStreamDestroy(ctx->aux2_stream);
@@ -116,7 +122,8 @@
 }
 
 int sipp_ctx_set_kernel_routes(sipp_ctx* ctx, uint32_t routes) {
-    if (!ctx || (routes & ~(uint32_t)(SIPP_ROUTE_OPENINGS_UNGROUPED | SIPP_ROUTE_LDE_COLUMN_WIDE | SIPP_ROUTE_WITNESS_NO_GRAPH))) return SIPP_E_BADARG;
+    if (!ctx || (routes & ~(uint32_t)(SIPP_ROUTE_OPENINGS_UNGROUPED | SIPP_ROUTE_LDE_COLUMN_WIDE | SIPP_ROUTE_WITNESS_NO_GRAPH |
+                                     SIPP_ROUTE_OPENING_RANGES_MASK))) return SIPP_E_BADARG;
     std::unique_lock<std::mutex> lk(ctx->async.mu);
     if (ctx->async.has_job) {
         lk.unlock();
diff --git a/sipp_amd/csrc/ctx.hpp b/sipp_amd/csrc/ctx.hpp
--- a/sipp_amd/csrc/ctx.hpp
+++ b/sipp_amd/csrc/ctx.hpp
@@ -38,6 +38,9 @@
     double ms = 0.0;
 };
 
+constexpr size_t SIPP_STAGE_CAP_WORDS = (size_t)4 << 8;
+constexpr size_t SIPP_STAGE_WORDS = SIPP_STAGE_CAP_WORDS + 8;
+
 struct sipp_ctx {
     int device = 0;
     hipStream_t stream = nullptr;
@@ -50,6 +53,12 @@
     size_t arena_peak = 0;
 
     std::map<std::tuple<int, uint64_t, uint64_t>, uint64_t*> tables;
+
+    struct QuotSegs {
+        int n_seg = 0, n_gadget_segs = 0;
+        const uint32_t* d_tab = nullptr;
+    };
+    std::map<const void*, QuotSegs> quot_segs;
 
     bool prof = false;
     std::vector<hipEvent_t> ev_pool;
@@ -60,6 +69,8 @@
 
     uint64_t* h_pinned = nullptr;
     size_t h_pinned_words = 0;
+    uint64_t* h_stage = nullptr;
+    hipEvent_t ev_tail[16] = {nullptr};
 
     sipp_gate* gate_wait = nullptr;
     sipp_gate* gate_release = nullptr;
diff --git a/sipp_amd/csrc/fri.hip b/sipp_amd/csrc/fri.hip
--- a/sipp_amd/csrc/fri.hip
+++ b/sipp_amd/csrc/fri.hip
@@ -8,8 +8,9 @@
     const uint32_t ch = std::min(cap_height, log_leaves);
     uint64_t off = 0;
     for (uint32_t l = 0; l < log_leaves - ch; l++) off += (uint64_t)1 << (log_leaves - l);
-    SIPP_CHECK_HIP(ctx, hipMemcpyAsync(cap_host, d_tree + 4 * off, ((size_t)4 << ch) * 8, hipMemcpyDeviceToHost, ctx->stream));
+    SIPP_CHECK_HIP(ctx, hipMemcpyAsync(ctx->h_stage, d_tree + 4 * off, ((size_t)4 << ch) * 8, hipMemcpyDeviceToHost, ctx->stream));
     SIPP_CHECK_HIP(ctx, hipStreamSynchronize(ctx->stream));
+    memcpy(cap_host, ctx->h_stage, ((size_t)4 << ch) * 8);
     return SIPP_OK;
 }
 
@@ -75,8 +76,13 @@
     (void)cap_words;
     if (final_len) *final_len = len_c;
     {
-        std::vector<uint64_t> fpv(2 * len_c);
-        SIPP_CHECK_HIP(ctx, hipMemcpyAsync(fpv.data(), cur, fpv.size() * 8, hipMemcpyDeviceToHost, ctx->stream));
+        std::vector<uint64_t> big;
+        uint64_t* fpv = ctx->h_pinned;
+        if (2 * len_c > ctx->h_pinned_words) {
+            big.resize(2 * len_c);
+            fpv = big.data();
+        }
+        SIPP_CHECK_HIP(ctx, hipMemcpyAsync(fpv, cur, 2 * len_c * 8, hipMemcpyDeviceToHost, ctx->stream));
         SIPP_CHECK_HIP(ctx, hipStreamSynchronize(ctx->stream));
         for (size_t i = 0; i < len_c; i++) {
             uint64_t e[2] = {fpv[i], fpv[len_c + i]};
@@ -97,11 +103,12 @@
     }
     SIPP_TRY(push(&pow_witness, 1));
     if (tick) tick("pow");
-    std::vector<uint32_t> qidx(nq);
+    uint32_t* qidx = reinterpret_cast<uint32_t*>(ctx->h_pinned);
+    if ((size_t)nq * 4 + 64 + 80 * sizeof(QueryGatherTask) > ctx->h_pinned_words * 8) return sipp_fail(ctx, SIPP_E_NOMEM, "query indices exceed the pinned buffer");
     for (uint32_t i = 0; i < nq; i++) qidx[i] = (uint32_t)(ch.get() % m);
     uint32_t* d_idx = arena_alloc_t<uint32_t>(ctx, nq);
     if (!d_idx) return SIPP_E_NOMEM;
-    SIPP_CHECK_HIP(ctx, hipMemcpyAsync(d_idx, qidx.data(), nq * 4, hipMemcpyHostToDevice, ctx->stream));
+    SIPP_CHECK_HIP(ctx, hipMemcpyAsync(d_idx, qidx, nq * 4, hipMemcpyHostToDevice, ctx->stream));
     const uint32_t nsib0 = log_m - p.cap_height;
     size_t st_words = 0;
     std::vector<size_t> off_rows(n_oracles), off_sib(n_oracles), off_leaf(R), off_rsib(R);
@@ -142,7 +149,9 @@
         }
         QueryGatherTask* d_tasks = arena_alloc_t<QueryGatherTask>(ctx, tasks.size());
         if (!d_tasks) return SIPP_E_NOMEM;
-        SIPP_CHECK_HIP(ctx, hipMemcpyAsync(d_tasks, tasks.data(), tasks.size() * sizeof(QueryGatherTask), hipMemcpyHostToDevice, ctx->stream));
+        QueryGatherTask* h_tasks = reinterpret_cast<QueryGatherTask*>(ctx->h_pinned + (((size_t)nq * 4 + 63) / 64) * 8);
+        memcpy(h_tasks, tasks.data(), tasks.size() * sizeof(QueryGatherTask));
+        SIPP_CHECK_HIP(ctx, hipMemcpyAsync(d_tasks, h_tasks, tasks.size() * sizeof(QueryGatherTask), hipMemcpyHostToDevice, ctx->stream));
         SIPP_TRY(sipp_k_gather_tasks(ctx, d_tasks, (uint32_t)tasks.size(), d_idx, nq));
     }
     uint64_t* hst = ctx->h_pinned;
@@ -323,14 +332,15 @@
             SIPP_TRY(sipp_k_openings(ctx, oracles[rg.oracle].d_coeffs + (size_t)rg.col_begin * n, cnt, n, d_zp[b], nullptr, d_open + 4 * at));
             at += cnt;
         }
-        std::vector<uint64_t> hop(4 * k + 4);
-        SIPP_CHECK_HIP(ctx, hipMemcpyAsync(hop.data(), d_open, (4 * k) * 8, hipMemcpyDeviceToHost, ctx->stream));
+        if (4 * k > ctx->h_pinned_words) return sipp_fail(ctx, SIPP_E_NOMEM, "fri: opening set exceeds the pinned buffer");
+        const uint64_t* hop = ctx->h_pinned;
+        SIPP_CHECK_HIP(ctx, hipMemcpyAsync(ctx->h_pinned, d_open, (4 * k) * 8, hipMemcpyDeviceToHost, ctx->stream));
         SIPP_CHECK_HIP(ctx, hipStreamSynchronize(ctx->stream));
         for (size_t j = 0; j < k; j++) {
             memcpy(pf + pos, &hop[4 * j], 16);
             pos += 2;
-            ch.observe_many(&hop[4 * j], 2);
-        }
+        }
+        ch.observe_strided(hop, k, 4, 2);
     }
     const gl::E2 alpha = ch.get_ext();
     uint64_t* d_acc = arena_alloc_t<uint64_t>(ctx, 2 * n);
@@ -344,22 +354,12 @@
             const sipp_poly_range& rg = batches[b].ranges[r];
             for (uint32_t c = rg.col_begin; c < rg.col_end; c++) cols.push_back(oracles[rg.oracle].d_coeffs + (size_t)c * n);
         }
-        std::vector<uint32_t> apow(6 * k + 6);
-        gl::E2 ap = gl::e2(1);
-        for (size_t c = 0; c < k; c++) {
-            const uint64_t comp[2] = {ap.c0, ap.c1};
-            for (int q = 0; q < 2; q++) {
-                apow[6 * c + 3 * q] = (uint32_t)comp[q] & 0x3FFFFFu;
-                apow[6 * c + 3 * q + 1] = (uint32_t)(comp[q] >> 22) & 0x3FFFFFu;
-                apow[6 * c + 3 * q + 2] = (uint32_t)(comp[q] >> 44);
-            }
-            ap = gl::mul(ap, alpha);
-        }
+        const gl::E2 ap = gl::pow(alpha, (uint64_t)k);
         const uint64_t** d_cols = reinterpret_cast<const uint64_t**>(arena_alloc(ctx, (k + 1) * sizeof(uint64_t*)));
-        uint32_t* d_apow = arena_alloc_t<uint32_t>(ctx, apow.size());
+        uint32_t* d_apow = arena_alloc_t<uint32_t>(ctx, 6 * k + 6);
         if (!d_cols || !d_apow) return SIPP_E_NOMEM;
+        SIPP_TRY(sipp_k_fri_apow3(ctx, alpha, k, d_apow));
         SIPP_CHECK_HIP(ctx, hipMemcpyAsync(d_cols, cols.data(), k * sizeof(uint64_t*), hipMemcpyHostToDevice, ctx->stream));
-        SIPP_CHECK_HIP(ctx, hipMemcpyAsync(d_apow, apow.data(), apow.size() * 4, hipMemcpyHostToDevice, ctx->stream));
         SIPP_CHECK_HIP(ctx, hipStreamSynchronize(ctx->stream));
         SIPP_TRY(sipp_k_fri_batch_quotient(ctx, d_cols, (int)k, n, d_apow, d_zp[b], d_zip[b], ap, b == 0, d_acc));
     }
diff --git a/sipp_amd/csrc/host_challenger.hpp b/sipp_amd/csrc/host_challenger.hpp
--- a/sipp_amd/csrc/host_challenger.hpp
+++ b/sipp_amd/csrc/host_challenger.hpp
@@ -29,6 +29,21 @@
     void observe_many(const uint64_t* e, size_t n) {
         for (size_t i = 0; i < n; i++) observe(e[i]);
     }
+    void observe_strided(const uint64_t* e, size_t count, size_t stride, uint32_t width) {
+        if (!count || !width) return;
+        uint32_t k = n_in;
+        for (size_t i = 0; i < count; i++, e += stride)
+            for (uint32_t j = 0; j < width; j++) {
+                in_buf[k++] = e[j];
+                if (k == 8) {
+                    n_in = 8;
+                    duplex();
+                    k = 0;
+                }
+            }
+        n_in = k;
+        if (k) n_out = 0;
+    }
     uint64_t get() {
         if (n_in != 0 || n_out == 0) duplex();
         return out_buf[--n_out];
diff --git a/sipp_amd/csrc/poseidon.hip b/sipp_amd/csrc/poseidon.hip
--- a/sipp_amd/csrc/poseidon.hip
+++ b/sipp_amd/csrc/poseidon.hip
@@ -246,6 +246,7 @@
     unsigned long long* result;
 };
 __global__ void __launch_bounds__(256) pow_kernel(PowArgs a) {
+    if (*a.result < a.base) return;
     const uint64_t w = a.base + (uint64_t)blockIdx.x * blockDim.x + threadIdx.x;
     uint64_t s[12];
 #pragma unroll
@@ -296,22 +297,33 @@
     a.n_in = n_in; a.pow_bits = pow_bits; a.resp_word = resp_word; a.result = d_res;
     const uint32_t log_batch = pow_bits + 1 < 12 ? 12 : pow_bits + 1 > 28 ? 28 : pow_bits + 1;
     const uint64_t batch = (uint64_t)1 << log_batch;
-    unsigned long long h_res = ~0ull;
+    volatile unsigned long long* h_res = reinterpret_cast<volatile unsigned long long*>(ctx->h_stage + SIPP_STAGE_CAP_WORDS);
+    unsigned long long found = ~0ull;
     SIPP_CHECK_HIP(ctx, hipMemsetAsync(d_res, 0xff, sizeof(unsigned long long), ctx->stream));
-    for (uint64_t base = 0; base < ((uint64_t)1 << 44); base += batch) {
+    const uint64_t limit = (uint64_t)1 << 44;
+    auto enqueue = [&](uint64_t base, int slot) -> int {
         a.base = base;
         {
             ProfScope ps(ctx, "pow_grind");
             hipLaunchKernelGGL(pow_kernel, dim3((unsigned)(batch / 256)), dim3(256), 0, ctx->stream, a);
         }
         SIPP_CHECK_HIP(ctx, hipGetLastError());
-        SIPP_CHECK_HIP(ctx, hipMemcpyAsync(&h_res, d_res, sizeof h_res, hipMemcpyDeviceToHost, ctx->stream));
-        SIPP_CHECK_HIP(ctx, hipStreamSynchronize(ctx->stream));
-        if (h_res != ~0ull) break;
+        SIPP_CHECK_HIP(ctx, hipMemcpyAsync(const_cast<unsigned long long*>(h_res) + slot, d_res, sizeof(unsigned long long),
+                                           hipMemcpyDeviceToHost, ctx->stream));
+        SIPP_CHECK_HIP(ctx, hipEventRecord(ctx->ev_tail[slot], ctx->stream));
+        return SIPP_OK;
+    };
+    SIPP_TRY(enqueue(0, 0));
+    int slot = 0;
+    for (uint64_t base = 0; base < limit; base += batch, slot ^= 1) {
+        if (base + batch < limit) SIPP_TRY(enqueue(base + batch, slot ^ 1));
+        SIPP_CHECK_HIP(ctx, hipEventSynchronize(ctx->ev_tail[slot]));
+        found = h_res[slot];
+        if (found != ~0ull) break;
     }
     arena_release(ctx, mk);
-    if (h_res == ~0ull) return sipp_fail(ctx, SIPP_E_UNSUPPORTED, "pow_search: no witness found");
-    *witness = (uint64_t)h_res;
+    if (found == ~0ull) return sipp_fail(ctx, SIPP_E_UNSUPPORTED, "pow_search: no witness found");
+    *witness = (uint64_t)found;
     return SIPP_OK;
 }
 
diff --git a/sipp_amd/csrc/prover.hip b/sipp_amd/csrc/prover.hip
--- a/sipp_amd/csrc/prover.hip
+++ b/sipp_amd/csrc/prover.hip
@@ -2,6 +2,7 @@
 
 #include "ctx.hpp"
 #include "prover.hpp"
+#include "tail_tables.hpp"
 
 namespace {
 
@@ -405,6 +406,18 @@
     a.part[((size_t)g * 2 + 1) * m + j] = gl::mul(c.acc1, a.seg_pow[2 * g + 1]);
 }
 
+__global__ void quotient_alpha_tab_kernel(uint64_t a0, uint64_t a1, int ns, const uint32_t* __restrict__ after,
+                                          uint64_t* __restrict__ seg_pow, uint32_t* __restrict__ apoly3) {
+    const int t = blockIdx.x * blockDim.x + threadIdx.x;
+    if (t < 2 * ns) {
+        seg_pow[t] = sipp_tail::seg_pow_word(a0, a1, after, t);
+    } else if (t < 2 * ns + 128) {
+        uint32_t l[3];
+        sipp_tail::apoly3_entry(a0, a1, t - 2 * ns, l);
+        for (int q = 0; q < 3; q++) apoly3[3 * (t - 2 * ns) + q] = l[q];
+    }
+}
+
 __global__ void alpha_pow3_kernel(uint64_t a0, uint64_t a1, int K, int nc, uint32_t* __restrict__ out) {
     const int t = blockIdx.x * blockDim.x + threadIdx.x;
     const int total = 2 * 3 + nc * 2 * 6;
@@ -675,9 +688,10 @@
     size_t n;
     const uint64_t *t0, *t1;
     uint64_t* out;
+    uint32_t b0;
 };
 __global__ void __launch_bounds__(256) openings3_kernel(Open3Args a) {
-    const uint32_t b = blockIdx.x;
+    const uint32_t b = a.b0 + blockIdx.x;
     const uint64_t* col;
     const uint64_t* t1 = a.t1;
     if (b < a.ncols[0]) {
@@ -698,10 +712,11 @@
     size_t n, seg_len;
     const uint64_t *t0, *t1;
     uint64_t* partial;
+    uint32_t g0;
 };
 __global__ void __launch_bounds__(256) openings_group_kernel(OpenGArgs a) {
     __shared__ uint64_t s[4][256];
-    uint32_t g = blockIdx.x, orc = 0, col_base = 0;
+    uint32_t g = a.g0 + blockIdx.x, orc = 0, col_base = 0;
     while (orc < 2 && g >= (a.ncols[orc] + OG - 1) / OG) {
         g -= (a.ncols[orc] + OG - 1) / OG;
         col_base += a.ncols[orc];
@@ -767,6 +782,14 @@
         if (threadIdx.x < 4) a.partial[((size_t)(col_base + c0 + c) * gridDim.y + blockIdx.y) * 4 + threadIdx.x] = s[threadIdx.x][0];
         __syncthreads();
     }
+}
+
+__global__ void __launch_bounds__(256) fri_apow3_kernel(E2 fa, uint32_t total, uint32_t* __restrict__ out) {
+    const uint32_t c = blockIdx.x * blockDim.x + threadIdx.x;
+    if (c >= total) return;
+    uint32_t l[6];
+    sipp_tail::fri_apow3_entry(fa, c, l);
+    for (int q = 0; q < 6; q++) out[6 * c + q] = l[q];
 }
 
 struct CombArgs {
@@ -1100,6 +1123,74 @@
     }
 }
 
+static int quotient_segments(sipp_ctx* ctx, const air_spec_t* a, sipp_ctx::QuotSegs* out) {
+    std::vector<uint32_t> off, cnt;
+    std::vector<int> ncons;
+    const int64_t* w = a->prog;
+    const int64_t* end = a->prog + a->prog_len;
+    while (w < end && w[0] == 1) {
+        off.push_back((uint32_t)(w - a->prog));
+        cnt.push_back(0);
+        if (w[6] != 2) return sipp_fail(ctx, SIPP_E_UNSUPPORTED, "quotient: gadgets must pair their limbs (group 2)");
+        ncons.push_back(32 / (int)w[6] + 1);
+        w += 7;
+        w += 2 + 5 * w[1];
+        int64_t np = *w++;
+        for (int64_t p = 0; p < np; p++) {
+            w += 1;
+            w += 2 + 5 * w[1];
+            w += 2 + 5 * w[1];
+        }
+        int64_t nl = *w++;
+        for (int64_t p = 0; p < nl; p++) {
+            w += 1;
+            w += 2 + 5 * w[1];
+        }
+        if (np > 64) {
+            const uint32_t nsl = (uint32_t)std::min<int64_t>(SIPP_QUOTIENT_MAX_SLICES, (np + 39) / 40);
+            cnt.back() = 0x80000000u | (nsl << 8);
+            for (uint32_t k = 1; k < nsl; k++) {
+                off.push_back(off.back());
+                cnt.push_back(0x80000000u | (nsl << 8) | k);
+                ncons.push_back(0);
+            }
+        }
+    }
+    while (w < end) {
+        off.push_back((uint32_t)(w - a->prog));
+        uint32_t k = 0;
+        while (w < end && k < 64) {
+            int64_t nmono = w[1];
+            w += 2;
+            for (int64_t mo = 0; mo < nmono; mo++) w += 2 + 2 * w[1];
+            k++;
+        }
+        cnt.push_back(k);
+        ncons.push_back((int)k);
+    }
+    const int ns = (int)off.size();
+    int n_gadget_segs = 0;
+    auto is_gadget = [](uint32_t c) { return c == 0 || (c >> 31) != 0; };
+    while (n_gadget_segs < ns && is_gadget(cnt[n_gadget_segs])) n_gadget_segs++;
+    for (int g = n_gadget_segs; g < ns; g++)
+        if (is_gadget(cnt[g])) return sipp_fail(ctx, SIPP_E_UNSUPPORTED, "quotient: gadgets must precede the polynomial constraints");
+    std::vector<uint64_t> host(((size_t)3 * ns + 1) / 2 + 1, 0);
+    uint32_t* h32 = reinterpret_cast<uint32_t*>(host.data());
+    memcpy(h32, off.data(), (size_t)ns * 4);
+    memcpy(h32 + ns, cnt.data(), (size_t)ns * 4);
+    uint32_t after = 0;
+    for (int g = ns - 1; g >= 0; g--) {
+        h32[2 * ns + g] = after;
+        after += (uint32_t)ncons[g];
+    }
+    uint64_t* d = nullptr;
+    SIPP_TRY(sipp_table_put(ctx, 105, (uint64_t)a->kind, (uint64_t)(uintptr_t)a->prog, host, &d));
+    out->n_seg = ns;
+    out->n_gadget_segs = n_gadget_segs;
+    out->d_tab = reinterpret_cast<const uint32_t*>(d);
+    return SIPP_OK;
+}
+
 int sipp_k_quotient(sipp_ctx* ctx, const air_spec_t* a, uint32_t log_n, const uint64_t* d_lde, const uint64_t* d_zlde,
                     size_t lde_stride, const uint64_t* d_aux, const uint64_t alpha[2], const uint64_t beta[2],
                     const uint64_t gamma[2], uint64_t* d_out) {
@@ -1192,91 +1283,21 @@
             x = gl::mul(x, gi);
         }
     }
-    int n_gadget_segs = 0;
     ArenaScope scope(ctx);
+    sipp_ctx::QuotSegs& segs = ctx->quot_segs[a->prog];
+    if (!segs.d_tab) SIPP_TRY(quotient_segments(ctx, a, &segs));
+    const int ns = segs.n_seg, n_gadget_segs = segs.n_gadget_segs;
     {
-        std::vector<uint32_t> off, cnt;
-        std::vector<int> ncons;
-        const int64_t* w = a->prog;
-        const int64_t* end = a->prog + a->prog_len;
-        while (w < end && w[0] == 1) {
-            off.push_back((uint32_t)(w - a->prog));
-            cnt.push_back(0);
-            if (w[6] != 2) return sipp_fail(ctx, SIPP_E_UNSUPPORTED, "quotient: gadgets must pair their limbs (group 2)");
-            ncons.push_back(32 / (int)w[6] + 1);
-            w += 7;
-            w += 2 + 5 * w[1];
-            int64_t np = *w++;
-            for (int64_t p = 0; p < np; p++) {
-                w += 1;
-                w += 2 + 5 * w[1];
-                w += 2 + 5 * w[1];
-            }
-            int64_t nl = *w++;
-            for (int64_t p = 0; p < nl; p++) {
-                w += 1;
-                w += 2 + 5 * w[1];
-            }
-            if (np > 64) {
-                const uint32_t nsl = (uint32_t)std::min<int64_t>(SIPP_QUOTIENT_MAX_SLICES, (np + 39) / 40);
-                cnt.back() = 0x80000000u | (nsl << 8);
-                for (uint32_t k = 1; k < nsl; k++) {
-                    off.push_back(off.back());
-                    cnt.push_back(0x80000000u | (nsl << 8) | k);
-                    ncons.push_back(0);
-                }
-            }
-        }
-        while (w < end) {
-            off.push_back((uint32_t)(w - a->prog));
-            uint32_t k = 0;
-            while (w < end && k < 64) {
-                int64_t nmono = w[1];
-                w += 2;
-                for (int64_t mo = 0; mo < nmono; mo++) w += 2 + 2 * w[1];
-                k++;
-            }
-            cnt.push_back(k);
-            ncons.push_back((int)k);
-        }
-        const int ns = (int)off.size();
         q.n_seg = ns;
-        n_gadget_segs = 0;
-        auto is_gadget = [](uint32_t c) { return c == 0 || (c >> 31) != 0; };
-        while (n_gadget_segs < ns && is_gadget(cnt[n_gadget_segs])) n_gadget_segs++;
-        for (int g = n_gadget_segs; g < ns; g++)
-            if (is_gadget(cnt[g])) return sipp_fail(ctx, SIPP_E_UNSUPPORTED, "quotient: gadgets must precede the polynomial constraints");
-        std::vector<uint64_t> host((size_t)ns * 2 + ns + 2 + 192, 0);
-        int after = 0;
-        for (int g = ns - 1; g >= 0; g--) {
-            host[2 * g] = gl::pow(alpha[0], (uint64_t)after);
-            host[2 * g + 1] = gl::pow(alpha[1], (uint64_t)after);
-            after += ncons[g];
-        }
-        uint32_t* h32 = reinterpret_cast<uint32_t*>(&host[2 * ns]);
-        memcpy(h32, off.data(), (size_t)ns * 4);
-        memcpy(h32 + ns, cnt.data(), (size_t)ns * 4);
-        const size_t ap_at = (size_t)ns * 2 + (((size_t)2 * ns + 1) >> 1);
-        {
-            uint32_t* ap = reinterpret_cast<uint32_t*>(&host[ap_at]);
-            for (int ch = 0; ch < 2; ch++) {
-                uint64_t x = 1;
-                for (int e = 0; e < 64; e++) {
-                    ap[(ch * 64 + e) * 3 + 0] = (uint32_t)x & 0x3FFFFFu;
-                    ap[(ch * 64 + e) * 3 + 1] = (uint32_t)(x >> 22) & 0x3FFFFFu;
-                    ap[(ch * 64 + e) * 3 + 2] = (uint32_t)(x >> 44);
-                    x = gl::mul(x, alpha[ch]);
-                }
-            }
-        }
-        uint64_t* d_tab = arena_alloc_t<uint64_t>(ctx, host.size());
+        const size_t ap_at = (size_t)ns * 2;
+        uint64_t* d_tab = arena_alloc_t<uint64_t>(ctx, ap_at + 192);
         q.part = arena_alloc_t<uint64_t>(ctx, (size_t)ns * 2 * m);
         if (!d_tab || !q.part) return SIPP_E_NOMEM;
-        SIPP_CHECK_HIP(ctx, hipMemcpyAsync(d_tab, host.data(), host.size() * 8, hipMemcpyHostToDevice, ctx->stream));
-        SIPP_CHECK_HIP(ctx, hipStreamSynchronize(ctx->stream));
+        hipLaunchKernelGGL(quotient_alpha_tab_kernel, dim3((unsigned)((2 * ns + 128 + 255) / 256)), dim3(256), 0, ctx->stream, alpha[0],
+                           alpha[1], ns, segs.d_tab + 2 * ns, d_tab, reinterpret_cast<uint32_t*>(d_tab + ap_at));
         q.seg_pow = d_tab;
-        q.seg_off = reinterpret_cast<const uint32_t*>(d_tab + 2 * ns);
-        q.seg_cnt = q.seg_off + ns;
+        q.seg_off = segs.d_tab;
+        q.seg_cnt = segs.d_tab + ns;
         q.apoly3 = reinterpret_cast<const uint32_t*>(d_tab + ap_at);
     }
     {
@@ -1357,38 +1378,68 @@
     return SIPP_OK;
 }
 
+uint32_t sipp_openings3_units(const sipp_ctx* ctx, const uint32_t ncols[3], size_t n) {
+    if ((ctx->kernel_routes & SIPP_ROUTE_OPENINGS_UNGROUPED) || n < 1024) return ncols[0] + ncols[1] + ncols[2];
+    uint32_t groups = 0;
+    for (int i = 0; i < 3; i++) groups += (ncols[i] + OG - 1) / OG;
+    return groups;
+}
 int sipp_k_openings3(sipp_ctx* ctx, const uint64_t* const d_coeffs[3], const uint32_t ncols[3], size_t n, const uint64_t* d_t0,
-                     const uint64_t* d_t1, uint64_t* d_out) {
+                     const uint64_t* d_t1, uint64_t* d_out, uint32_t part, uint32_t nparts, uint32_t* col_lo, uint32_t* col_hi) {
     const unsigned total = ncols[0] + ncols[1] + ncols[2];
-    if (!total) return SIPP_OK;
+    const uint32_t units = sipp_openings3_units(ctx, ncols, n);
+    if (!nparts || part >= nparts || nparts > std::max(1u, units)) return sipp_fail(ctx, SIPP_E_BADARG, "openings: range outside the launch units");
+    const uint32_t u0 = (uint32_t)((uint64_t)units * part / nparts), u1 = (uint32_t)((uint64_t)units * (part + 1) / nparts);
+    *col_lo = *col_hi = 0;
+    if (!total || u0 == u1) return SIPP_OK;
     ProfScope ps(ctx, "openings");
     Open3Args a;
     for (int i = 0; i < 3; i++) {
         a.coeffs[i] = d_coeffs[i];
         a.ncols[i] = ncols[i];
     }
-    a.n = n; a.t0 = d_t0; a.t1 = d_t1; a.out = d_out;
+    a.n = n; a.t0 = d_t0; a.t1 = d_t1; a.out = d_out; a.b0 = u0;
     const bool grouped = !(ctx->kernel_routes & SIPP_ROUTE_OPENINGS_UNGROUPED);
     if (!grouped || n < 1024) {
-        hipLaunchKernelGGL(openings3_kernel, dim3(total), dim3(256), 0, ctx->stream, a);
+        hipLaunchKernelGGL(openings3_kernel, dim3(u1 - u0), dim3(256), 0, ctx->stream, a);
         SIPP_CHECK_HIP(ctx, hipGetLastError());
+        *col_lo = u0;
+        *col_hi = u1;
         return SIPP_OK;
     }
     OpenGArgs g;
-    unsigned groups = 0;
     for (int i = 0; i < 3; i++) {
         g.coeffs[i] = d_coeffs[i];
         g.ncols[i] = ncols[i];
-        groups += (ncols[i] + OG - 1) / OG;
-    }
+    }
+    auto first_col = [&](uint32_t grp) {
+        uint32_t base = 0;
+        for (int i = 0; i < 3; i++) {
+            const uint32_t ng = (ncols[i] + OG - 1) / OG;
+            if (grp < ng) return base + grp * OG;
+            grp -= ng;
+            base += ncols[i];
+        }
+        return base;
+    };
+    const uint32_t groups = units, c0 = first_col(u0), c1 = first_col(u1);
     const size_t segs = std::max<size_t>(1, std::min<size_t>(std::min<size_t>(SIPP_OPENINGS_MAX_SEGS, (4096 + groups - 1) / groups), n / 1024));
     ArenaScope scope(ctx);
     g.partial = arena_alloc_t<uint64_t>(ctx, (size_t)total * segs * 4);
     if (!g.partial) return SIPP_E_NOMEM;
-    g.n = n; g.seg_len = (n + segs - 1) / segs; g.t0 = d_t0; g.t1 = d_t1;
-    hipLaunchKernelGGL(openings_group_kernel, dim3(groups, (unsigned)segs), dim3(256), 0, ctx->stream, g);
-    hipLaunchKernelGGL(openings_fold_kernel, dim3((4 * total + 255) / 256), dim3(256), 0, ctx->stream, g.partial, (uint32_t)total,
-                       (uint32_t)segs, d_out);
+    g.n = n; g.seg_len = (n + segs - 1) / segs; g.t0 = d_t0; g.t1 = d_t1; g.g0 = u0;
+    hipLaunchKernelGGL(openings_group_kernel, dim3(u1 - u0, (unsigned)segs), dim3(256), 0, ctx->stream, g);
+    hipLaunchKernelGGL(openings_fold_kernel, dim3((4 * (c1 - c0) + 255) / 256), dim3(256), 0, ctx->stream, g.partial + (size_t)c0 * segs * 4,
+                       c1 - c0, (uint32_t)segs, d_out + (size_t)c0 * 4);
+    SIPP_CHECK_HIP(ctx, hipGetLastError());
+    *col_lo = c0;
+    *col_hi = c1;
+    return SIPP_OK;
+}
+
+int sipp_k_fri_apow3(sipp_ctx* ctx, gl::E2 fa, size_t total, uint32_t* d_apow3) {
+    if (!total) return SIPP_OK;
+    hipLaunchKernelGGL(fri_apow3_kernel, dim3((unsigned)((total + 255) / 256)), dim3(256), 0, ctx->stream, fa, (uint32_t)total, d_apow3);
     SIPP_CHECK_HIP(ctx, hipGetLastError());
     return SIPP_OK;
 }
diff --git a/sipp_amd/csrc/prover.hpp b/sipp_amd/csrc/prover.hpp
--- a/sipp_amd/csrc/prover.hpp
+++ b/sipp_amd/csrc/prover.hpp
@@ -22,8 +22,10 @@
                     const uint64_t* d_t1, uint64_t* d_out);
 constexpr size_t SIPP_OPENINGS_MAX_SEGS = 32;
 constexpr int SIPP_QUOTIENT_MAX_SLICES = 8;
+uint32_t sipp_openings3_units(const sipp_ctx* ctx, const uint32_t ncols[3], size_t n);
 int sipp_k_openings3(sipp_ctx* ctx, const uint64_t* const d_coeffs[3], const uint32_t ncols[3], size_t n, const uint64_t* d_t0,
-                     const uint64_t* d_t1, uint64_t* d_out);
+                     const uint64_t* d_t1, uint64_t* d_out, uint32_t part, uint32_t nparts, uint32_t* col_lo, uint32_t* col_hi);
+int sipp_k_fri_apow3(sipp_ctx* ctx, gl::E2 fa, size_t total, uint32_t* d_apow3);
 int sipp_k_fri_final(sipp_ctx* ctx, const uint64_t* const src[3], const int cnt[3], size_t n, const uint32_t* d_apow3,
                      int n1, gl::E2 shift1, const uint64_t* d_zp[2], const uint64_t* d_zip[2], uint64_t* d_final);
 int sipp_k_fri_batch_quotient(sipp_ctx* ctx, const uint64_t* const* d_cols, int total, size_t n, const uint32_t* d_apow3,
diff --git a/sipp_amd/csrc/stark.hip b/sipp_amd/csrc/stark.hip
--- a/sipp_amd/csrc/stark.hip
+++ b/sipp_amd/csrc/stark.hip
@@ -79,14 +79,23 @@
     return SIPP_OK;
 }
 
+constexpr uint32_t SIPP_OPENING_RANGES_DEFAULT = 4;
+static uint32_t opening_ranges(const sipp_ctx* ctx, int kind, uint32_t units) {
+    uint32_t k = (ctx->kernel_routes & SIPP_ROUTE_OPENING_RANGES_MASK) >> SIPP_ROUTE_OPENING_RANGES_SHIFT;
+    if (!k) k = SIPP_OPENING_RANGES_DEFAULT;
+    (void)kind;
+    return std::max(1u, std::min(std::min(k, units), 15u));
+}
+
 static size_t tree_words(uint32_t log_leaves) { return ((size_t)8 << log_leaves); }
 
 static int read_cap(sipp_ctx* ctx, const uint64_t* d_tree, uint32_t log_leaves, uint64_t* cap_host) {
     const uint32_t ch = std::min(ctx->cfg.cap_height, log_leaves);
     uint64_t off = 0;
     for (uint32_t l = 0; l < log_leaves - ch; l++) off += (uint64_t)1 << (log_leaves - l);
-    SIPP_CHECK_HIP(ctx, hipMemcpyAsync(cap_host, d_tree + 4 * off, ((size_t)4 << ch) * 8, hipMemcpyDeviceToHost, ctx->stream));
+    SIPP_CHECK_HIP(ctx, hipMemcpyAsync(ctx->h_stage, d_tree + 4 * off, ((size_t)4 << ch) * 8, hipMemcpyDeviceToHost, ctx->stream));
     SIPP_CHECK_HIP(ctx, hipStreamSynchronize(ctx->stream));
+    memcpy(cap_host, ctx->h_stage, ((size_t)4 << ch) * 8);
     return SIPP_OK;
 }
 
@@ -320,9 +329,10 @@
     SIPP_CHECK_HIP(ctx, hipMemsetAsync(d_err, 0, sizeof(int), ctx->stream));
     SIPP_TRY(sipp_trace_fill(ctx, a, d_ios, s.num_io, log_n, d_trace, d_err));
     {
-        int h_err = 0;
-        SIPP_CHECK_HIP(ctx, hipMemcpyAsync(&h_err, d_err, sizeof(int), hipMemcpyDeviceToHost, ctx->stream));
+        int* h_errp = reinterpret_cast<int*>(ctx->h_stage);
+        SIPP_CHECK_HIP(ctx, hipMemcpyAsync(h_errp, d_err, sizeof(int), hipMemcpyDeviceToHost, ctx->stream));
         SIPP_CHECK_HIP(ctx, hipStreamSynchronize(ctx->stream));
+        const int h_err = *h_errp;
         if (h_err) return sipp_fail(ctx, h_err, "trace fill: IO record not provable (claimed output wrong, degenerate point or non-canonical limbs)");
     }
 
@@ -351,7 +361,9 @@
     const int n_aux = a->n_aux;
     const uint32_t log_io = log_n - (uint32_t)a->log_rows;
     const size_t nio = s.num_io;
-    std::vector<uint64_t> auxc((size_t)n_aux * nio), col(nio);
+    if ((size_t)n_aux * nio > ctx->h_pinned_words) return sipp_fail(ctx, SIPP_E_NOMEM, "public-input polynomials larger than the pinned staging buffer");
+    uint64_t* const auxc = ctx->h_pinned;
+    std::vector<uint64_t> col(nio);
     {
         const uint64_t g = gl::root_of_unity(log_n);
         for (int ai = 0; ai < n_aux; ai++) {
@@ -376,7 +388,7 @@
                     f = gl::mul(f, sft);
                 }
             }
-            memcpy(&auxc[(size_t)ai * nio], col.data(), nio * 8);
+            memcpy(auxc + (size_t)ai * nio, col.data(), nio * 8);
         }
     }
     SIPP_TRY(read_cap(ctx, T.tree, log_m, cap_host));
@@ -411,9 +423,8 @@
         uint64_t* d_auxc = arena_alloc_t<uint64_t>(ctx, (size_t)n_aux * nio + 1);
         uint64_t* d_aux = arena_alloc_t<uint64_t>(ctx, (size_t)n_aux * mq + 1);
         if (!d_auxc || !d_aux) return SIPP_E_NOMEM;
-        SIPP_CHECK_HIP(ctx, hipMemcpyAsync(d_auxc, auxc.data(), auxc.size() * 8, hipMemcpyHostToDevice, ctx->stream));
-        SIPP_CHECK_HIP(ctx, hipStreamSynchronize(ctx->stream));
         if (n_aux) {
+            SIPP_CHECK_HIP(ctx, hipMemcpyAsync(d_auxc, auxc, (size_t)n_aux * nio * 8, hipMemcpyHostToDevice, ctx->stream));
             int rc_aux = sipp_tree_coset_eval(ctx, d_auxc, d_aux, (size_t)n_aux, log_io, log_mq);
             if (rc_aux == SIPP_E_UNSUPPORTED)
                 rc_aux = sipp_ntt_dif(ctx, d_auxc, nio, log_io, d_aux, mq, log_mq, (size_t)n_aux, false, NttDiag{gl::GEN, 0});
@@ -440,46 +451,40 @@
         uint64_t* const tabs[4] = {d_zp[0], d_zp[1], d_zip[0], d_zip[1]};
         SIPP_TRY(sipp_k_pow_table4(ctx, bases, n, tabs));
     }
+    const size_t n_open = (size_t)(W + P + Q);
+    if (n_open * 4 > ctx->h_pinned_words) return sipp_fail(ctx, SIPP_E_NOMEM, "opening set larger than the pinned staging buffer");
+    const uint64_t* const hop = ctx->h_pinned;
     {
         const uint64_t* const cf[3] = {T.coeffs, Z.coeffs, Qo.coeffs};
         const uint32_t nc3[3] = {(uint32_t)W, (uint32_t)P, (uint32_t)Q};
-        SIPP_TRY(sipp_k_openings3(ctx, cf, nc3, n, d_zp[0], d_zp[1], d_open));
-    }
-    std::vector<uint64_t> hop((size_t)(W + P + Q) * 4);
-    SIPP_CHECK_HIP(ctx, hipMemcpyAsync(hop.data(), d_open, hop.size() * 8, hipMemcpyDeviceToHost, ctx->stream));
-    SIPP_CHECK_HIP(ctx, hipStreamSynchronize(ctx->stream));
-    {
+        const uint32_t nr = opening_ranges(ctx, kind, sipp_openings3_units(ctx, nc3, n));
+        uint32_t lo[16], hi[16];
+        for (uint32_t k = 0; k < nr; k++) {
+            SIPP_TRY(sipp_k_openings3(ctx, cf, nc3, n, d_zp[0], d_zp[1], d_open, k, nr, &lo[k], &hi[k]));
+            if (hi[k] > lo[k])
+                SIPP_CHECK_HIP(ctx, hipMemcpyAsync(ctx->h_pinned + (size_t)lo[k] * 4, d_open + (size_t)lo[k] * 4, (size_t)(hi[k] - lo[k]) * 32,
+                                                   hipMemcpyDeviceToHost, ctx->stream));
+            SIPP_CHECK_HIP(ctx, hipEventRecord(ctx->ev_tail[k], ctx->stream));
+        }
+        for (uint32_t k = 0; k < nr; k++) {
+            SIPP_CHECK_HIP(ctx, hipEventSynchronize(ctx->ev_tail[k]));
+            ch.observe_strided(hop + (size_t)lo[k] * 4, hi[k] - lo[k], 4, 2);
+        }
+        ch.observe_strided(hop + 2, (size_t)(W + P), 4, 2);
         for (int c = 0; c < W; c++) push(&hop[(size_t)c * 4], 2);
         for (int c = 0; c < W; c++) push(&hop[(size_t)c * 4 + 2], 2);
         for (int c = 0; c < P; c++) push(&hop[(size_t)(W + c) * 4], 2);
         for (int c = 0; c < P; c++) push(&hop[(size_t)(W + c) * 4 + 2], 2);
         for (int c = 0; c < Q; c++) push(&hop[(size_t)(W + P + c) * 4], 2);
-        for (int c = 0; c < W; c++) ch.observe_many(&hop[(size_t)c * 4], 2);
-        for (int c = 0; c < P; c++) ch.observe_many(&hop[(size_t)(W + c) * 4], 2);
-        for (int c = 0; c < Q; c++) ch.observe_many(&hop[(size_t)(W + P + c) * 4], 2);
-        for (int c = 0; c < W; c++) ch.observe_many(&hop[(size_t)c * 4 + 2], 2);
-        for (int c = 0; c < P; c++) ch.observe_many(&hop[(size_t)(W + c) * 4 + 2], 2);
     }
 
     tick("openings+observe");
     const gl::E2 fa = ch.get_ext();
     uint64_t* d_final = arena_alloc_t<uint64_t>(ctx, 2 * n);
     {
-        std::vector<uint32_t> apow((size_t)(W + P + Q) * 6);
-        gl::E2 ap = gl::e2(1);
-        for (int c = 0; c < W + P + Q; c++) {
-            const uint64_t comp[2] = {ap.c0, ap.c1};
-            for (int q = 0; q < 2; q++) {
-                apow[6 * c + 3 * q] = (uint32_t)comp[q] & 0x3FFFFFu;
-                apow[6 * c + 3 * q + 1] = (uint32_t)(comp[q] >> 22) & 0x3FFFFFu;
-                apow[6 * c + 3 * q + 2] = (uint32_t)(comp[q] >> 44);
-            }
-            ap = gl::mul(ap, fa);
-        }
-        uint32_t* d_apow = arena_alloc_t<uint32_t>(ctx, apow.size());
+        uint32_t* d_apow = arena_alloc_t<uint32_t>(ctx, n_open * 6);
         if (!d_final || !d_apow) return SIPP_E_NOMEM;
-        SIPP_CHECK_HIP(ctx, hipMemcpyAsync(d_apow, apow.data(), apow.size() * 4, hipMemcpyHostToDevice, ctx->stream));
-        SIPP_CHECK_HIP(ctx, hipStreamSynchronize(ctx->stream));
+        SIPP_TRY(sipp_k_fri_apow3(ctx, fa, n_open, d_apow));
         const uint64_t* src[3] = {T.coeffs, Z.coeffs, Qo.coeffs};
         const int cnt[3] = {W, P, Q};
         const uint64_t* zp[2] = {d_zp[0], d_zp[1]};
diff --git a/sipp_amd/csrc/tail_tables.hpp b/sipp_amd/csrc/tail_tables.hpp
--- /dev/null
+++ b/sipp_amd/csrc/tail_tables.hpp
@@ -0,0 +1,23 @@
+#pragma once
+#include "gl.hpp"
+
+namespace sipp_tail {
+
+__device__ __forceinline__ uint64_t seg_pow_word(uint64_t a0, uint64_t a1, const uint32_t* __restrict__ after, int t) {
+    return gl::pow(t & 1 ? a1 : a0, (uint64_t)after[t >> 1]);
+}
+
+__device__ __forceinline__ void apoly3_entry(uint64_t a0, uint64_t a1, int u, uint32_t (&l)[3]) {
+    gl::limbs3(l, gl::pow(u >> 6 ? a1 : a0, (uint64_t)(u & 63)));
+}
+
+__device__ __forceinline__ void fri_apow3_entry(gl::E2 fa, uint32_t c, uint32_t (&l)[6]) {
+    const gl::E2 p = gl::pow(fa, (uint64_t)c);
+    uint32_t t[3];
+    gl::limbs3(t, p.c0);
+    for (int q = 0; q < 3; q++) l[q] = t[q];
+    gl::limbs3(t, p.c1);
+    for (int q = 0; q < 3; q++) l[3 + q] = t[q];
+}
+
+}
```

Result: no change. 2417 pairings/s (median of 5 runs) (+0.5%).
